# V-Sekai/godot-whisper

Measured on AMD Instinct MI355X. Metric: realtime-factor (audio-sec/wall-sec), base.en 30 s chunk, PCM->tokens, higher is better.
Workload: dtype f16; 1 GPU; base.en, single 30 s chunk per step per GPU (1x MI355X), greedy decode, host params (max_tokens=16, single_segment, token_timestamps), whisper_full with host PCM (H2D inside the timed region); weights=synthetic seed 1234 (f16 ggml, base.en shape)

## Files before the change

godot-whisper_amd/csrc/device.cpp:

```cpp

#include "wmi.h"
#include <atomic>
#include <thread>
#include <map>
#include <mutex>
#include "kernels.h"

#include <algorithm>
#include <cmath>
#include <cstdlib>
#include <cstring>

namespace wmi {

namespace {

template <typename T> bool dalloc(T *& p, size_t n_elems) {
    p = nullptr;
    return HIP_OK(hipMalloc((void **) &p, std::max<size_t>(n_elems, 1) * sizeof(T)));
}
template <typename T> void dfree(T *& p) { if (p) (void) hipFree(p); p = nullptr; }

}

static bool make_own_queue_stream(int device, hipStream_t * out) {
    uint32_t mask[16]; for (uint32_t & m : mask) m = 0xFFFFFFFFu;
    hipDeviceProp_t prop{};
    const int ncu = hipGetDeviceProperties(&prop, device) == hipSuccess ? prop.multiProcessorCount : 256;
    const uint32_t words = (uint32_t) std::min(16, (ncu + 31) / 32);
    if (hipExtStreamCreateWithCUMask(out, words, mask) == hipSuccess) return true;
    (void) hipGetLastError();
    return false;
}

static std::mutex g_oq_mu;
static std::map<int, std::vector<hipStream_t>> g_oq_pool;
static std::map<int, int> g_oq_made;
hipStream_t own_queue_stream_get(int device) {
    static const int cap = getenv("WMI_OWN_QUEUE_CAP") ? std::max(0, atoi(getenv("WMI_OWN_QUEUE_CAP"))) : 16;
    {
        std::lock_guard<std::mutex> lk(g_oq_mu);
        auto & v = g_oq_pool[device];
        if (!v.empty()) { hipStream_t s = v.back(); v.pop_back(); return s; }
        if (g_oq_made[device] >= cap) return nullptr;
        g_oq_made[device] += 1;
    }
    hipStream_t s = nullptr;
    if (make_own_queue_stream(device, &s)) return s;
    std::lock_guard<std::mutex> lk(g_oq_mu);
    g_oq_made[device] -= 1;
    return nullptr;
}
void own_queue_stream_put(int device, hipStream_t s) {
    if (!s) return;
    (void) hipStreamSynchronize(s);
    std::lock_guard<std::mutex> lk(g_oq_mu);
    g_oq_pool[device].push_back(s);
}

static thread_local StateInstall * t_state_install = nullptr;
State * StateSlot::get() const {
    for (const StateInstall * p = t_state_install; p; p = p->prev) if (p->slot == this) return p->st;
    return own;
}
StateInstall::StateInstall(const StateSlot & sl, State * s) : slot(&sl), st(s), prev(t_state_install) { t_state_install = this; }
StateInstall::~StateInstall() { t_state_install = prev; }
StateInstall * state_installs_top() { return t_state_install; }
void state_installs_set(StateInstall * top) { t_state_install = top; }

static bool init_state_into(whisper_context & ctx, State * st, bool replica_state, hipStream_t adopt);
bool init_state(whisper_context & ctx, bool replica_state, hipStream_t adopt) {
    State * st = new State();
    ctx.state = st;
    return init_state_into(ctx, st, replica_state, adopt);
}
static bool init_state_into(whisper_context & ctx, State * st, bool replica_state, hipStream_t adopt) {
    const HParams & hp = ctx.model.hp;
    st->device = ctx.device;
    DeviceState & d = st->dev;
    if (!HIP_OK(hipSetDevice(ctx.device))) return false;
    static const bool pooled = getenv("WMI_POOLED_MAIN_STREAM") != nullptr;
    if (adopt) { d.stream = adopt; d.stream_own_queue = true; }
    else if (!pooled && (d.stream = own_queue_stream_get(ctx.device))) d.stream_own_queue = true;
    else HIP_TRY(hipStreamCreateWithFlags(&d.stream, hipStreamNonBlocking));
    if (!replica_state) {
        static const int spares = getenv("WMI_SPARE_QUEUES") ? atoi(getenv("WMI_SPARE_QUEUES"))
                                : getenv("WMI_BATCH_REPLICAS") ? std::max(0, std::min(15, atoi(getenv("WMI_BATCH_REPLICAS")))) : 3;
        for (int i = 0; i < spares; ++i) { hipStream_t sp = own_queue_stream_get(ctx.device); if (sp) ctx.spare_streams.push_back(sp); }
    }

    const size_t S = hp.n_audio_state, T = hp.n_audio_ctx, Lt = hp.n_text_layer, H = hp.n_audio_head;
    const size_t n_self = 3 * (size_t) hp.n_text_ctx;
    st->kv_self.size = (uint32_t) n_self; st->kv_self.cells.assign(n_self, KVCell());
    bool ok = true;
    ok = ok && dalloc(st->kv_self.k, Lt * n_self * S) && dalloc(st->kv_self.v, Lt * n_self * S);
    ok = ok && dalloc(d.kvc_k, Lt * T * S) && dalloc(d.kvc_v, Lt * T * S);
    d.Tpad = (int) ((T + 63) / 64 * 64);
    const size_t mel_rows = 2 * T + 8;
    ok = ok && dalloc(d.mel_t, mel_rows * hp.n_mels + 1024) && dalloc(d.conv1, (2 * T + 4) * S)
            && dalloc(d.x, T * S) && dalloc(d.embd_conv, T * S) && dalloc(d.xn, T * S)
            && dalloc(d.q, T * S) && dalloc(d.k, T * S) && dalloc(d.vt, S * d.Tpad) && dalloc(d.att, T * S)
            && dalloc(d.h, T * 4 * S) && dalloc(d.rowmax, H * T) && dalloc(d.enc_out, T * S) && dalloc(d.enc_out_h, T * S)
            && dalloc(d.mel_max, 4);
    const size_t n = hp.n_text_ctx;
    if (ctx.model.quantised) {
        const size_t rows = std::max<size_t>(T, n);
        d.aq_rows = (int) rows;
        ok = ok && dalloc(d.aq, rows * 4 * S) && dalloc(d.ads, 2 * rows * (4 * S / 32)) && dalloc(d.att32, T * S) && dalloc(d.datt32, n * S);
        d.wq16_elems = 8 * S * S;
        ok = ok && dalloc(d.aq16, rows * 4 * S) && dalloc(d.wq16, d.wq16_elems);
    }
    d.logits_rows_cap = 8;
    ok = ok && dalloc(d.d_tokens, 3 * n + n * n_self);
    if (ok) { d.d_pos = d.d_tokens + n; d.d_rows = d.d_pos + n; d.d_mask = (float *) (d.d_rows + n); }
    ok = ok
            && dalloc(d.dx, n * S) && dalloc(d.dxn, n * S) && dalloc(d.dq, n * S) && dalloc(d.datt, n * S)
            && dalloc(d.dh, n * 4 * S) && dalloc(d.logits, (size_t) d.logits_rows_cap * hp.n_vocab)
            && dalloc(d.xattn, k::attn_cross_scratch_floats((int) n, (int) H, (int) T));
    d.pinned_bytes = std::max<size_t>((size_t) d.logits_rows_cap * hp.n_vocab * 4, n * n_self * 4 + 3 * n * 4 + 4096);
    ok = ok && HIP_OK(hipHostMalloc(&d.pinned, d.pinned_bytes, hipHostMallocDefault));
    {
        unsigned char * hand = nullptr;
        ok = ok && dalloc(hand, (size_t) 32 * S + 64 + 40960);
        if (ok) { d.mlp_hand = hand; d.mlp_arrive = (unsigned long long *) (hand + (size_t) 16 * S); k::fill_zero(hand, (size_t) 32 * S + 64 + 40960, d.stream); }
    }
    if (!ok) { WMI_ERR("%s: device allocation failed\n", __func__); return false; }
    k::fill_zero(d.vt, S * d.Tpad * sizeof(__half), d.stream);
    k::fill_zero(d.conv1, (2 * T + 4) * S * sizeof(__half), d.stream);
    k::fill_zero(d.mel_t, (mel_rows * hp.n_mels + 1024) * sizeof(__half), d.stream);
    k::fill_zero(st->kv_self.k, Lt * n_self * S * sizeof(__half), d.stream);
    k::fill_zero(st->kv_self.v, Lt * n_self * S * sizeof(__half), d.stream);
    k::fill_zero(d.kvc_k, Lt * T * S * sizeof(__half), d.stream);
    k::fill_zero(d.kvc_v, Lt * T * S * sizeof(__half), d.stream);
    HIP_TRY(hipStreamSynchronize(d.stream));

    st->batch.token.resize(n); st->batch.pos.resize(n); st->batch.seq_id.resize(n); st->batch.logits.resize(n);
    st->logits.reserve((size_t) hp.n_vocab * 8);
    for (auto & dec : st->decoders) dec.rng = std::mt19937(0);
    WMI_INFO("%s: kv self size = %.2f MB, kv cross size = %.2f MB\n", __func__,
             2.0 * Lt * n_self * S * 2 / 1e6, 2.0 * Lt * T * S * 2 / 1e6);
    return true;
}

State * create_state(whisper_context & ctx) {
    State * st = new State();
    if (init_state_into(ctx, st, true, nullptr)) return st;
    destroy_state(st);
    return nullptr;
}

void free_state(whisper_context & ctx) {
    destroy_state(ctx.state);
    ctx.state = nullptr;
}

void destroy_state(State * st) {
    if (!st) return;
    (void) hipSetDevice(st->device);
    DeviceState & d = st->dev;
    if (d.stream) (void) hipStreamSynchronize(d.stream);
    dfree(st->kv_self.k); dfree(st->kv_self.v); dfree(d.kvc_k); dfree(d.kvc_v);
    if (d.copy_stream) { (void) hipStreamSynchronize(d.copy_stream); (void) hipStreamDestroy(d.copy_stream); }
    if (d.energy_ev) (void) hipEventDestroy(d.energy_ev);
    for (hipEvent_t & e : d.ph_ev) { if (e) (void) hipEventDestroy(e); e = nullptr; }
    if (d.mel_ev) { (void) hipEventDestroy(d.mel_ev); d.mel_ev = nullptr; }
    dfree(d.energy); if (d.energy_host) (void) hipHostFree(d.energy_host);
    if (d.ts_host) (void) hipHostFree(d.ts_host);
    dfree(d.pcm); dfree(d.mel); dfree(d.mel_max); dfree(d.mel_t); dfree(d.conv1); dfree(d.x); dfree(d.embd_conv);
    dfree(d.xn); dfree(d.q); dfree(d.k); dfree(d.vt); dfree(d.att); dfree(d.h); dfree(d.rowmax); dfree(d.enc_out);
    dfree(d.enc_out_h); dfree(d.d_tokens); d.d_pos = nullptr; d.d_mask = nullptr; d.d_rows = nullptr; dfree(d.dx); dfree(d.dxn);
    dfree(d.dq); dfree(d.datt); dfree(d.dh); dfree(d.logits); dfree(d.xattn); dfree(d.ban_dev);
    if (d.mlp_hand) { (void) hipFree(d.mlp_hand); d.mlp_hand = nullptr; d.mlp_arrive = nullptr; }
    dfree(d.aq); dfree(d.ads); dfree(d.aq16); dfree(d.wq16); dfree(d.att32); dfree(d.datt32);
    for (auto & sg : d.step_graphs) { if (sg.exec) (void) hipGraphExecDestroy(sg.exec); if (sg.graph) (void) hipGraphDestroy(sg.graph); sg = DeviceState::StepGraph{}; }
    if (d.step_dev) (void) hipFree(d.step_dev);
    if (d.sample_dev) (void) hipFree(d.sample_dev);
    if (d.filter_scratch) (void) hipFree(d.filter_scratch);
    if (d.draw_scratch) (void) hipFree(d.draw_scratch);
    if (d.draw_host) (void) hipHostFree(d.draw_host);
    if (d.step_host) (void) hipHostFree(d.step_host);
    if (d.sample_host) (void) hipHostFree(d.sample_host);
    if (d.pinned) (void) hipHostFree(d.pinned);
    if (d.stream && d.stream_own_queue) own_queue_stream_put(st->device, d.stream);
    else if (d.stream) (void) hipStreamDestroy(d.stream);
    delete st;
}

static bool ensure_mel_capacity(DeviceState & d, size_t n_pad, size_t n_mel_elems) {
    if (n_pad > d.pcm_cap) { dfree(d.pcm); if (!dalloc(d.pcm, n_pad + 1024)) return false; d.pcm_cap = n_pad + 1024; }
    if (n_mel_elems > d.mel_cap) { dfree(d.mel); if (!dalloc(d.mel, n_mel_elems)) return false; d.mel_cap = n_mel_elems; }
    return true;
}

static bool phase_events(DeviceState & d) {
    for (hipEvent_t & e : d.ph_ev) if (!e && !HIP_OK(hipEventCreate(&e))) return false;
    return true;
}
int64_t phase_settle(State & st, bool wait) {
    DeviceState & d = st.dev;
    if (!d.ph_mel && !d.ph_enc) return 0;
    if (wait) (void) hipStreamSynchronize(d.stream);
    float ms = 0.0f; double gpu_us = 0.0;
    if (d.ph_mel) { if (hipEventSynchronize(d.ph_ev[1]) == hipSuccess && hipEventElapsedTime(&ms, d.ph_ev[0], d.ph_ev[1]) == hipSuccess) { st.t_mel_us += (int64_t) (ms * 1e3); gpu_us += ms * 1e3; } d.ph_mel = false; }
    if (d.ph_enc) { if (hipEventSynchronize(d.ph_ev[3]) == hipSuccess && hipEventElapsedTime(&ms, d.ph_ev[2], d.ph_ev[3]) == hipSuccess) { st.t_encode_us += (int64_t) (ms * 1e3); gpu_us += ms * 1e3; } d.ph_enc = false; }
    return d.ph_host0 + (int64_t) gpu_us;
}

bool pcm_to_mel(whisper_context & ctx, const float * samples, int n_samples, bool samples_on_device, bool sync, bool defer) {
    if (!compute_ready(ctx, __func__)) return false;
    State & st = *ctx.state; DeviceState & d = st.dev;
    const int64_t t0 = time_us();
    const int n_mel = ctx.model.n_filt_mel;
    hipStream_t ms = d.mel_stream ? d.mel_stream : d.stream;
    const int64_t n_pad = (int64_t) n_samples + 480000 + 400;
    const int n_len = (int) ((n_pad - 400) / 160);
    const int n_len_org = 1 + (n_samples + 200 - 400) / 160;
    const int n_valid = n_samples + 200;
    const int n_fft_frames = std::min(n_valid / 160 + 1, n_len);
    if (!ensure_mel_capacity(d, (size_t) n_pad + (size_t) n_samples, (size_t) n_mel * n_len)) return false;
    defer = defer && ms == d.stream && phase_events(d);
    if (defer) { (void) phase_settle(st, true); HIP_TRY(hipEventRecord(d.ph_ev[0], ms)); }
    const float * src = samples;
    if (!samples_on_device) {
        float * stage = d.pcm + n_pad;
        HIP_TRY(hipMemcpyAsync(stage, samples, (size_t) n_samples * 4, hipMemcpyHostToDevice, ms));
        src = stage;
    }
    d.last_pcm = src; d.last_pcm_n = n_samples;
    k::mel_pad(src, n_samples, d.pcm, (int) n_pad, ms, (int *) d.mel_max);
    k::mel_frames(d.pcm, n_valid, n_fft_frames, n_len, n_mel, ctx.w.mel_filters, ctx.w.mel_ranges, ctx.w.mel_taps, d.mel, (int *) d.mel_max, ms);
    k::mel_normalize(d.mel, n_mel * n_len, (const int *) d.mel_max, ms);
    st.mel.n_len = n_len; st.mel.n_len_org = n_len_org; st.mel.n_mel = n_mel;
    if (defer) { HIP_TRY(hipEventRecord(d.ph_ev[1], ms)); d.ph_mel = true; d.ph_host0 = t0; return true; }
    if (sync) HIP_TRY(hipStreamSynchronize(ms));
    st.t_mel_us += time_us() - t0;
    return true;
}

static bool ensure_copy_stream(DeviceState & d) {
    if (d.copy_stream) return true;
    int prio_lo = 0, prio_hi = 0;
    (void) hipDeviceGetStreamPriorityRange(&prio_lo, &prio_hi);
    if (!HIP_OK(hipStreamCreateWithPriority(&d.copy_stream, hipStreamNonBlocking, prio_lo))) HIP_TRY(hipStreamCreateWithFlags(&d.copy_stream, hipStreamNonBlocking));
    HIP_TRY(hipEventCreateWithFlags(&d.energy_ev, hipEventDisableTiming));
    return true;
}
static hipStream_t envelope_stream(const DeviceState & d) { return d.energy_wait_stream ? d.energy_wait_stream : d.copy_stream; }

bool pcm_to_mel_batch(whisper_context & ctx, const std::vector<State *> & states, const float * const * pcm, const int * n_samples,
                      bool samples_on_device, bool envelopes) {
    if (!compute_ready(ctx, __func__)) return false;
    DeviceState & pd = ctx.state->dev;
    hipStream_t s = pd.stream;
    const int n_mel = ctx.model.n_filt_mel;
    const int64_t t0 = time_us();
    k::MelBatch mb{}; int nb = 0; std::vector<State *> in;
    if (envelopes && !ensure_copy_stream(pd)) return false;
    for (size_t r = 0; r < states.size(); ++r) {
        const int n = n_samples[r];
        if (n <= 0) continue;
        if (nb >= 16) return false;
        State & st = *states[r]; DeviceState & d = st.dev;
        const int64_t n_pad = (int64_t) n + 480000 + 400;
        const int n_len = (int) ((n_pad - 400) / 160);
        if (!ensure_mel_capacity(d, (size_t) n_pad + (size_t) n, (size_t) n_mel * n_len)) return false;
        const float * src = pcm[r];
        if (!samples_on_device) {
            float * stage = d.pcm + n_pad;
            HIP_TRY(hipMemcpyAsync(stage, pcm[r], (size_t) n * 4, hipMemcpyHostToDevice, s));
            src = stage;
        }
        d.last_pcm = src; d.last_pcm_n = n;
        st.mel.n_len = n_len; st.mel.n_len_org = 1 + (n + 200 - 400) / 160; st.mel.n_mel = n_mel;
        mb.pcm[nb] = src; mb.pad[nb] = d.pcm; mb.mel[nb] = d.mel; mb.gmax[nb] = (int *) d.mel_max; mb.n[nb] = n;
        if (envelopes) {
            if (d.energy_pending && envelope_stream(d)) { HIP_TRY(hipStreamSynchronize(envelope_stream(d))); d.energy_pending = false; }
            const size_t nblk = (size_t) n / 256 + 2;
            if ((size_t) n > d.energy_cap) {
                st.energy = nullptr; st.energy_n = 0; st.energy_bmin = st.energy_bmax = nullptr;
                if (d.energy_host) (void) hipHostFree(d.energy_host);
                d.energy_host = nullptr; d.energy_cap = 0;
                if (!HIP_OK(hipHostMalloc((void **) &d.energy_host, ((size_t) n + 2 * ((size_t) n / 256 + 2)) * 4, hipHostMallocDefault))) return false;
                d.energy_cap = (size_t) n;
            }
            const size_t need = d.energy_cap + 2 * nblk;
            if (d.energy_dev_cap < need) { dfree(d.energy); d.energy_dev_cap = 0; if (!dalloc(d.energy, need)) return false; d.energy_dev_cap = need; }
            mb.energy[nb] = d.energy; mb.bmin[nb] = d.energy + d.energy_cap; mb.bmax[nb] = d.energy + d.energy_cap + nblk;
        }
        in.push_back(&st); ++nb;
    }
    if (nb == 0) return true;
    if (envelopes) {
        if (!pd.mel_ev) HIP_TRY(hipEventCreateWithFlags(&pd.mel_ev, hipEventDisableTiming));
        HIP_TRY(hipEventRecord(pd.energy_ev, s));
        HIP_TRY(hipStreamWaitEvent(pd.copy_stream, pd.energy_ev, 0));
        k::signal_energy_batch(mb, nb, 32, pd.copy_stream);
        HIP_TRY(hipEventRecord(pd.mel_ev, pd.copy_stream));
        for (State * st : in) {
            DeviceState & d = st->dev;
            d.energy_device_only = true; d.energy_pending = true; d.energy_wait_stream = pd.copy_stream;
        }
    }
    k::mel_batch(mb, nb, n_mel, ctx.w.mel_filters, ctx.w.mel_ranges, ctx.w.mel_taps, s);
    if (envelopes) HIP_TRY(hipStreamWaitEvent(s, pd.mel_ev, 0));
    ctx.state->t_mel_us += time_us() - t0;
    return hipGetLastError() == hipSuccess;
}

bool signal_energy_device(whisper_context & ctx, int hw, bool sync, int via_dma) {
    State & st = *ctx.state; DeviceState & d = st.dev;
    const int n = d.last_pcm_n;
    if (!d.last_pcm || n <= 0) return false;
    if (!ensure_copy_stream(d)) return false;
    if (d.energy_pending) { HIP_TRY(hipStreamSynchronize(envelope_stream(d))); d.energy_pending = false; }
    d.energy_wait_stream = nullptr;
    d.energy_device_only = false;
    if ((size_t) n > d.energy_cap) {
        st.energy = nullptr; st.energy_n = 0; st.energy_bmin = st.energy_bmax = nullptr;
        if (d.energy_host) (void) hipHostFree(d.energy_host);
        d.energy_host = nullptr; d.energy_cap = 0;
        if (!HIP_OK(hipHostMalloc((void **) &d.energy_host, ((size_t) n + 2 * ((size_t) n / 256 + 2)) * 4, hipHostMallocDefault))) return false;
        d.energy_cap = (size_t) n;
    }
    HIP_TRY(hipEventRecord(d.energy_ev, d.mel_stream ? d.mel_stream : d.stream));
    HIP_TRY(hipStreamWaitEvent(d.copy_stream, d.energy_ev, 0));
    {
        const size_t nb = (size_t) n / 256 + 2;
        const size_t need = d.energy_cap + 2 * nb;
        if (via_dma && d.energy_dev_cap < need) { dfree(d.energy); d.energy_dev_cap = 0; if (dalloc(d.energy, need)) d.energy_dev_cap = need; else via_dma = 0; }
        if (via_dma == 3) {
            k::signal_energy(d.last_pcm, n, hw, d.energy, d.energy + d.energy_cap, d.energy + d.energy_cap + nb, d.copy_stream);
            d.energy_device_only = true;
        } else
        k::signal_energy(d.last_pcm, n, hw, d.energy_host, d.energy_host + d.energy_cap, d.energy_host + d.energy_cap + nb, d.copy_stream);
    }
    d.energy_pending = true;
    return sync ? signal_energy_wait(st) : true;
}

bool ts_refine_device(State & st, const k::TsTok * in, int n, k::TsOut * out) {
    DeviceState & d = st.dev;
    constexpr int CAP = 448;
    if (n <= 0) return true;
    hipStream_t es = envelope_stream(d);
    if (n > CAP || !d.energy || !es) return false;
    if (!d.ts_host && !HIP_OK(hipHostMalloc(&d.ts_host, CAP * (sizeof(k::TsTok) + sizeof(k::TsOut)), hipHostMallocDefault))) return false;
    k::TsTok * hin = (k::TsTok *) d.ts_host; k::TsOut * hout = (k::TsOut *) (hin + CAP);
    memcpy(hin, in, (size_t) n * sizeof(k::TsTok));
    const size_t nb = (size_t) d.last_pcm_n / 256 + 2;
    k::ts_refine(d.energy, d.energy + d.energy_cap, d.energy + d.energy_cap + nb, d.last_pcm_n, hin, hout, n, es);
    HIP_TRY(hipStreamSynchronize(es));
    memcpy(out, hout, (size_t) n * sizeof(k::TsOut));
    return true;
}

bool signal_energy_wait(State & st) {
    DeviceState & d = st.dev;
    if (!d.energy_pending) return true;
    if (d.energy_device_only) {
        HIP_TRY(hipStreamSynchronize(envelope_stream(d)));
        st.energy = nullptr; st.energy_bmin = st.energy_bmax = nullptr; st.energy_n = d.last_pcm_n; st.energy_on_device = true;
        d.energy_pending = false;
        return true;
    }
    st.energy_on_device = false;
    HIP_TRY(hipStreamSynchronize(d.copy_stream));
    st.energy = d.energy_host; st.energy_n = d.last_pcm_n;
    st.energy_bmin = d.energy_host + d.energy_cap; st.energy_bmax = st.energy_bmin + ((size_t) d.last_pcm_n / 256 + 2);
    d.energy_pending = false;
    return true;
}

bool set_mel(whisper_context & ctx, const float * data, int n_len, int n_mel) {
    if (!compute_ready(ctx, __func__)) return false;
    State & st = *ctx.state; DeviceState & d = st.dev;
    if (!ensure_mel_capacity(d, 0, (size_t) n_len * n_mel)) return false;
    HIP_TRY(hipMemcpyAsync(d.mel, data, (size_t) n_len * n_mel * 4, hipMemcpyHostToDevice, d.stream));
    HIP_TRY(hipStreamSynchronize(d.stream));
    st.mel.n_len = n_len; st.mel.n_len_org = n_len; st.mel.n_mel = n_mel;
    return true;
}

bool encode(whisper_context & ctx, int mel_offset, bool defer) {
    if (!compute_ready(ctx, __func__)) return false;
    State & st = *ctx.state; DeviceState & d = st.dev; const Weights & w = ctx.w; const HParams & hp = ctx.model.hp;
    const int64_t t0 = time_us();
    d.chain_valid = false;
    defer = defer && !ctx.model.quantised && phase_events(d);
    if (defer) {
        if (d.ph_enc) (void) phase_settle(st, true);
        HIP_TRY(hipEventRecord(d.ph_ev[2], d.stream));
        if (!d.ph_mel) d.ph_host0 = t0;
    }
    const int T = st.exp_n_audio_ctx > 0 ? st.exp_n_audio_ctx : hp.n_audio_ctx;
    const int S = hp.n_audio_state, H = hp.n_audio_head, La = hp.n_audio_layer, Lt = hp.n_text_layer, nm = hp.n_mels;
    hipStream_t s = d.stream;
    if (st.mel.n_mel != nm || d.mel == nullptr) { WMI_ERR("%s: no mel spectrogram (n_mel %d, expected %d)\n", __func__, st.mel.n_mel, nm); return false; }

    const int rows_mel = 2 * T + 6;
    k::mel_slice(d.mel, st.mel.n_len, nm, mel_offset, 2 * T, d.mel_t, nm, rows_mel, s);
    {
        k::GemmArgs a{};
        a.A = d.mel_t; a.lda = nm; a.W = w.conv1_w; a.ldw = w.conv1_k; a.M = 2 * T; a.N = S; a.K = w.conv1_k;
        a.bias = w.conv1_b; a.C = d.conv1 + S; a.ldc = S;
        k::gemm(k::EPI_F16_BIAS_GELU, a, s);
    }
    if (d.conv1_max_T > T) k::fill_zero(d.conv1 + (size_t) (2 * T + 1) * S, (size_t) S * sizeof(__half), s);
    d.conv1_max_T = std::max(d.conv1_max_T, T);
    {
        k::GemmArgs a{};
        a.A = d.conv1; a.lda = 2 * S; a.W = w.conv2_w; a.ldw = w.conv2_k; a.M = T; a.N = S; a.K = w.conv2_k;
        a.bias = w.conv2_b; a.C = d.x; a.ldc = S; a.resid = w.e_pe; a.ldr = S; a.aux = d.embd_conv; a.ldaux = S;
        k::gemm(k::EPI_CONV2, a, s);
    }
    const float kq_scale = 1.0f / sqrtf((float) S / H);
    if (ctx.model.quantised) { if (!encode_layers_q(ctx, T)) return false; }
    else {
    for (int il = 0; il < La; ++il) {
        const EncLayerW & l = w.enc[il];
        k::layernorm(d.x, T, S, l.ln1_g, l.ln1_b, hp.eps, d.xn, nullptr, s);
        {
            k::GemmArgs a{};
            a.A = d.xn; a.lda = S; a.W = l.w_qkv; a.ldw = S; a.M = T; a.N = 3 * S; a.K = S; a.bias = l.b_qkv;
            a.C = d.q; a.ldc = S; a.aux = d.k; a.ldaux = S; a.aux2 = d.vt; a.ldaux2 = d.Tpad; a.S = S;
            k::gemm(k::EPI_QKV_ENC, a, s);
        }
        k::attn_encoder(d.q, d.k, d.vt, T, d.Tpad, S, H, kq_scale, d.att, s);
        {
            k::GemmArgs a{};
            a.A = d.att; a.lda = S; a.W = l.w_o; a.ldw = S; a.M = T; a.N = S; a.K = S; a.bias = l.b_o;
            a.C = d.x; a.ldc = S; a.resid = d.x; a.ldr = S;
            k::gemm(k::EPI_F32_BIAS_RESID, a, s);
        }
        k::layernorm(d.x, T, S, l.ln2_g, l.ln2_b, hp.eps, d.xn, nullptr, s);
        {
            k::GemmArgs a{};
            a.A = d.xn; a.lda = S; a.W = l.w_fc1; a.ldw = S; a.M = T; a.N = 4 * S; a.K = S; a.bias = l.b_fc1;
            a.C = d.h; a.ldc = 4 * S;
            k::gemm(k::EPI_F16_BIAS_GELU, a, s);
        }
        {
            k::GemmArgs a{};
            a.A = d.h; a.lda = 4 * S; a.W = l.w_fc2; a.ldw = 4 * S; a.M = T; a.N = S; a.K = 4 * S; a.bias = l.b_fc2;
            a.C = d.x; a.ldc = S; a.resid = d.x; a.ldr = S;
            k::gemm(k::EPI_F32_BIAS_RESID, a, s);
        }
    }
    k::layernorm(d.x, T, S, w.e_ln_g, w.e_ln_b, hp.eps, d.enc_out_h, d.enc_out, s);
    {
        k::GemmArgs a{};
        a.A = d.enc_out_h; a.lda = S; a.W = w.w_ckv; a.ldw = S; a.M = T; a.N = Lt * 2 * S; a.K = S; a.bias = w.b_ckv;
        a.C = d.kvc_k; a.ldc = S; a.aux = d.kvc_v; a.ldaux = S; a.S = S; a.layer_stride = (int64_t) T * S;
        a.scale = powf((float) S / H, -0.25f);
        k::gemm(k::EPI_CROSS_KV, a, s);
    }
    }
    st.enc_n_ctx = T;
    st.n_encode++;
    if (defer) {
        HIP_TRY(hipEventRecord(d.ph_ev[3], s)); d.ph_enc = true;
        return HIP_OK(hipGetLastError());
    }
    HIP_TRY(hipStreamSynchronize(s));
    if (!HIP_OK(hipGetLastError())) return false;
    {
        int64_t dt = time_us() - t0;
        const int64_t done = phase_settle(st, false);
        if (done > t0) dt = std::max<int64_t>(0, dt - (done - t0));
        st.t_encode_us += dt;
    }
    return true;
}

bool decode(whisper_context & ctx, const Batch & batch) {
    if (!compute_ready(ctx, __func__)) return false;
    State & st = *ctx.state; DeviceState & d = st.dev; const Weights & w = ctx.w; const HParams & hp = ctx.model.hp;
    const int64_t t0 = time_us();
    d.chain_valid = false;
    KVCache & kv = st.kv_self;
    const int n = batch.n_tokens;
    if (n <= 0) return false;
    if (n > hp.n_text_ctx) { WMI_ERR("%s: %d tokens in one batch, the model's text context is %d\n", __func__, n, hp.n_text_ctx); return false; }
    if (!kv_find_slot(kv, batch)) return false;
    kv.n = (uint32_t) kv_cell_max(kv);
    const int n_kv = (int) kv.n, kv_head = (int) kv.head, n_ctx = (int) kv.size;
    const int S = hp.n_text_state, H = hp.n_text_head, Lt = hp.n_text_layer, NV = hp.n_vocab;
    const int Tc = st.enc_n_ctx > 0 ? st.enc_n_ctx : (st.exp_n_audio_ctx > 0 ? st.exp_n_audio_ctx : hp.n_audio_ctx);
    hipStream_t s = d.stream;

    int32_t * p_tok = (int32_t *) d.pinned, * p_pos = p_tok + n, * p_rows = p_pos + n;
    float * p_mask = (float *) (p_rows + n);
    std::vector<int> rows;
    for (int i = 0; i < n; ++i) { p_tok[i] = batch.token[i]; p_pos[i] = batch.pos[i]; if (batch.logits[i]) rows.push_back(i); }
    for (size_t i = 0; i < rows.size(); ++i) p_rows[i] = rows[i];
    for (int j = 0; j < n; ++j) {
        const int32_t pos = batch.pos[j], seq = batch.seq_id[j];
        for (int i = 0; i < n_kv; ++i)
            p_mask[(size_t) j * n_kv + i] = (!kv.cells[i].has(seq) || kv.cells[i].pos > pos) ? -INFINITY : 0.0f;
    }
    d.d_pos = d.d_tokens + n; d.d_rows = d.d_pos + n; d.d_mask = (float *) (d.d_rows + n);
    HIP_TRY(hipMemcpyAsync(d.d_tokens, p_tok, ((size_t) 3 * n + (size_t) n * n_kv) * 4, hipMemcpyHostToDevice, s));

    if (ctx.model.quantised) {
        if (!decode_layers_q(ctx, n, n_kv, kv_head, Tc, rows)) return false;
        HIP_TRY(hipStreamSynchronize(s));
        if (!HIP_OK(hipGetLastError())) return false;
        int64_t dtq = time_us() - t0;
        { const int64_t done = phase_settle(st, false); if (done > t0) dtq = std::max<int64_t>(0, dtq - (done - t0)); }
        if (n == 1)      { st.t_decode_us += dtq; st.n_decode++; }
        else if (n < 16) { st.t_batchd_us += dtq; st.n_batchd += n; }
        else             { st.t_prompt_us += dtq; st.n_prompt += n; }
        return true;
    }
    k::dec_embed(d.d_tokens, d.d_pos, n, S, w.d_te, w.d_pe, d.dx, s);
    const float kq_scale = powf((float) S / H, -0.25f);

    auto proj = [&](int epi, const float * ln_g, const float * ln_b, const __half * a16, int K, int N, const __half * W,
                    const float * bias, void * C, int ldc, const float * resid, void * aux, int ldaux, void * aux2,
                    int ldaux2, float scale) {
        if (n <= 8) {
            k::GemvArgs g{};
            g.x32 = d.dx; g.ln_g = ln_g; g.ln_b = ln_b; g.eps = hp.eps; g.a16 = a16; g.n = n; g.K = K; g.N = N; g.W = W;
            g.bias = bias; g.epi = epi; g.C = C; g.ldc = ldc; g.resid = resid; g.ldr = S; g.aux = aux; g.ldaux = ldaux;
            g.aux2 = aux2; g.ldaux2 = ldaux2; g.scale = scale; g.S = S; g.rows = nullptr;
            k::gemv(g, s);
        } else {
            const __half * A = a16;
            if (ln_g) { k::layernorm(d.dx, n, S, ln_g, ln_b, hp.eps, d.dxn, nullptr, s); A = d.dxn; }
            k::GemmArgs a{};
            a.A = A; a.lda = K; a.W = W; a.ldw = K; a.M = n; a.N = N; a.K = K; a.bias = bias; a.C = C; a.ldc = ldc;
            a.resid = resid; a.ldr = S; a.aux = aux; a.ldaux = ldaux; a.aux2 = aux2; a.ldaux2 = ldaux2; a.scale = scale; a.S = S;
            k::gemm(epi, a, s);
        }
    };

    for (int il = 0; il < Lt; ++il) {
        const DecLayerW & l = w.dec[il];
        __half * ck = kv.k + ((size_t) il * n_ctx) * S, * cv = kv.v + ((size_t) il * n_ctx) * S;
        proj(k::EPI_QKV_DEC, l.ln1_g, l.ln1_b, nullptr, S, 3 * S, l.w_qkv, l.b_qkv, d.dq, S, nullptr,
             ck + (size_t) kv_head * S, S, cv + (size_t) kv_head * S, S, kq_scale);
        k::attn_decoder(d.dq, n, S, H, ck, cv, n_kv, d.d_mask, n_kv, d.datt, s);
        proj(k::EPI_F32_BIAS_RESID, nullptr, nullptr, d.datt, S, S, l.w_o, l.b_o, d.dx, S, d.dx, nullptr, 0, nullptr, 0, 0.f);
        proj(k::EPI_Q_SCALED, l.ln2_g, l.ln2_b, nullptr, S, S, l.w_cq, l.b_cq, d.dq, S, nullptr, nullptr, 0, nullptr, 0, kq_scale);
        k::attn_cross_split(d.dq, n, S, H, d.kvc_k + (size_t) il * Tc * S, d.kvc_v + (size_t) il * Tc * S, Tc, d.xattn, d.datt, s);
        proj(k::EPI_F32_BIAS_RESID, nullptr, nullptr, d.datt, S, S, l.w_co, l.b_co, d.dx, S, d.dx, nullptr, 0, nullptr, 0, 0.f);
        proj(k::EPI_F16_BIAS_GELU, l.ln3_g, l.ln3_b, nullptr, S, 4 * S, l.w_fc1, l.b_fc1, d.dh, 4 * S, nullptr, nullptr, 0, nullptr, 0, 0.f);
        proj(k::EPI_F32_BIAS_RESID, nullptr, nullptr, d.dh, 4 * S, S, l.w_fc2, l.b_fc2, d.dx, S, d.dx, nullptr, 0, nullptr, 0, 0.f);
    }

    st.logits.resize((size_t) n * NV);
    for (size_t r0 = 0; r0 < rows.size(); r0 += 8) {
        const int nr = (int) std::min<size_t>(8, rows.size() - r0);
        k::GemvArgs g{};
        g.x32 = d.dx; g.ln_g = w.d_ln_g; g.ln_b = w.d_ln_b; g.eps = hp.eps; g.n = nr; g.K = S; g.N = NV; g.W = w.d_te;
        g.epi = k::EPI_LOGITS; g.C = d.logits; g.ldc = NV; g.rows = d.d_rows + r0;
        k::gemv(g, s);
        if (d.keep_logits_on_device && rows.size() <= 8) continue;
        HIP_TRY(hipMemcpyAsync(d.pinned, d.logits, (size_t) nr * NV * 4, hipMemcpyDeviceToHost, s));
        HIP_TRY(hipStreamSynchronize(s));
        for (int r = 0; r < nr; ++r)
            memcpy(st.logits.data() + (size_t) rows[r0 + r] * NV, (const float *) d.pinned + (size_t) r * NV, (size_t) NV * 4);
    }
    HIP_TRY(hipStreamSynchronize(s));
    if (!HIP_OK(hipGetLastError())) return false;

    int64_t dt = time_us() - t0;
    { const int64_t done = phase_settle(st, false); if (done > t0) dt = std::max<int64_t>(0, dt - (done - t0)); }
    if (n == 1)      { st.t_decode_us += dt; st.n_decode++; }
    else if (n < 16) { st.t_batchd_us += dt; st.n_batchd += n; }
    else             { st.t_prompt_us += dt; st.n_prompt += n; }
    return true;
}

}

namespace wmi {

bool upload_static_ban(whisper_context & ctx, const whisper_full_params & params) {
    State & st = *ctx.state; DeviceState & d = st.dev; const Vocab & v = ctx.model.vocab;
    const uint64_t sig = (params.suppress_non_speech_tokens ? 1u : 0u) | (params.no_timestamps ? 2u : 0u) | (params.tdrz_enable ? 4u : 0u) | 8u;
    if (d.ban_dev && d.ban_sig == sig) return true;
    const int n = v.n_vocab;
    std::vector<uint8_t> ban(n, 0);
    auto B = [&](int id) { if (id >= 0 && id < n) ban[id] = 1; };
    B(v.not_); B(v.sot); B(v.nosp); if (!params.tdrz_enable) B(v.solm);
    B(v.translate); B(v.transcribe); B(v.prev);
    for (int i = 0; i < lang_count(); ++i) B(v.sot + 1 + i);
    if (params.no_timestamps) for (int i = v.beg; i < n; ++i) ban[i] = 1;
    if (params.suppress_non_speech_tokens) {
        Decoder tmp; tmp.i_batch = 0;
        std::vector<float> saved; saved.swap(st.logits);
        st.logits.assign(n, 0.0f);
        for (int i = v.beg; i < n; ++i) st.logits[i] = -1e30f;
        whisper_full_params p2 = params; p2.suppress_blank = false; p2.max_initial_ts = 0.0f; p2.logits_filter_callback = nullptr;
        tmp.sequence.tokens.push_back(whisper_token_data{0, 0, 0.f, 0.f, 0.f, 0.f, -1, -1, 0.f});
        process_logits(ctx, tmp, p2, 0.0f);
        for (int i = 0; i < v.beg; ++i) if (tmp.logits[i] == -INFINITY) ban[i] = 1;
        st.logits.swap(saved);
    }
    if (!d.ban_dev && !dalloc(d.ban_dev, (size_t) n)) return false;
    HIP_TRY(hipMemcpyAsync(d.ban_dev, ban.data(), (size_t) n, hipMemcpyHostToDevice, d.stream));
// ... 442 lines not shown
```

godot-whisper_amd/csrc/gemm_epi.h:

```cpp
#pragma once
#include "kernels.h"
#include "wave_ops.h"

namespace wmi { namespace k { namespace gemm_detail {

typedef _Float16 half8 __attribute__((ext_vector_type(8)));
typedef _Float16 half4 __attribute__((ext_vector_type(4)));
typedef float    floatx4 __attribute__((ext_vector_type(4)));


__device__ __forceinline__ float round_f16(float x) { return __half2float(f2h(x)); }

__device__ __forceinline__ float gelu16(float x) {
    const float xh = round_f16(x);
    const float g  = 0.5f * xh * (1.0f + tanhf(0.79788456080286535587989211986876f * xh * (1.0f + 0.044715f * xh * xh)));
    return round_f16(g);
}

__device__ __forceinline__ float gelu16_fast(float x) {
    const float xh = round_f16(x);
    const float u  = 0.79788456080286535587989211986876f * xh * (1.0f + 0.044715f * xh * xh);
    const float t  = 1.0f - 2.0f * __builtin_amdgcn_rcpf(__expf(2.0f * u) + 1.0f);
    return round_f16(0.5f * xh * (1.0f + t));
}

typedef float    float2v __attribute__((ext_vector_type(2)));
typedef _Float16 half2v  __attribute__((ext_vector_type(2)));
__device__ __forceinline__ half2v gelu16_pair(float2v x) {
    const half2v xh = __builtin_convertvector(x, half2v);
    const float2v xf = {(float) xh[0], (float) xh[1]};
    constexpr float C0 = -2.0f * 0.79788456080286535587989211986876f * 1.44269504088896340736f;
    constexpr float C1 = C0 * 0.044715f;
    const float2v c0 = {C0, C0}, c1 = {C1, C1}, one = {1.0f, 1.0f};
    const float2v w = __builtin_elementwise_fma(xf * xf, c1, c0) * xf;
    const float2v e = {__builtin_amdgcn_exp2f(w[0]), __builtin_amdgcn_exp2f(w[1])};
    const float2v d = one + e;
    const float2v r = {__builtin_amdgcn_rcpf(d[0]), __builtin_amdgcn_rcpf(d[1])};
    const float2v g = xf * r;
    return __builtin_convertvector(g, half2v);
}

struct Conv2Row { int out, pe; bool valid; };
__device__ __forceinline__ Conv2Row conv2_row(const GemmArgs & a, int m) {
    if (a.rows_per_chunk <= 0) return Conv2Row{m, m, true};
    const int P = a.rows_per_chunk, c = m / P, t = m - c * P;
    return Conv2Row{c * (P - 4) + t, t < P - 4 ? t : 0, t < P - 4};
}

template <int FM, int FN, bool GUARD>
__device__ __forceinline__ void epilogue_vt_wide(const GemmArgs & a, floatx4 (&acc)[FM][FN], const int mb, const int nb, const int lane);
__device__ __forceinline__ bool vt_wide_ok(const GemmArgs & a);
template <int EPI, int FM, int FN, bool GUARD>
__device__ __forceinline__ void epilogue_rows(const GemmArgs & a, floatx4 (&acc)[FM][FN], const int mb, const int nb, const int lane) {
    if constexpr (EPI == EPI_QKV_ENC) {
        if (__builtin_amdgcn_readfirstlane(nb) >= 2 * a.S && vt_wide_ok(a)) { epilogue_vt_wide<FM, FN, GUARD>(a, acc, mb, nb, lane); return; }
    }
    const int frow = lane & 15, fq = lane >> 4;
    float biasv[FN];
#pragma unroll
    for (int j = 0; j < FN; ++j) {
        const int n = nb + j * 16 + frow;
        biasv[j] = (a.bias && (!GUARD || n < a.N)) ? a.bias[n] : 0.0f;
    }
#pragma unroll
    for (int j = 0; j < FN; ++j) {
        const int n = nb + j * 16 + frow;
        if (GUARD && n >= a.N) continue;
        const float bias = biasv[j];
        float rpre[FM][4];
        if constexpr (EPI == EPI_F32_BIAS_RESID || EPI == EPI_CONV2) {
#pragma unroll
            for (int i = 0; i < FM; ++i)
#pragma unroll
                for (int r = 0; r < 4; ++r) {
                    const int m = mb + i * 16 + fq * 4 + r;
                    const int mc = (GUARD && m >= a.M) ? a.M - 1 : m;
                    rpre[i][r] = a.resid[(size_t) (EPI == EPI_CONV2 ? conv2_row(a, mc).pe : mc) * a.ldr + n];
                }
        }
#pragma unroll
        for (int i = 0; i < FM; ++i) {
            const int mrow = mb + i * 16 + fq * 4;
            if constexpr (EPI == EPI_QKV_ENC) {
                const int seg = n / a.S, c = n - seg * a.S;
                if (seg == 2) {
                    const int rpc = a.rows_per_chunk > 0 ? a.rows_per_chunk : a.M;
                    const int cb = mrow / rpc, t0 = mrow - cb * rpc;
                    __half * vt = (__half *) a.aux2 + (size_t) cb * a.chunk_stride_aux2 + (size_t) c * a.ldaux2;
                    if ((!GUARD || mrow + 3 < a.M) && t0 + 3 < rpc && ((t0 & 3) == 0)) {
                        half4 v;
#pragma unroll
                        for (int r = 0; r < 4; ++r) v[r] = (_Float16) pin_f32(acc[i][j][r] + bias);
                        *(half4 *) (vt + vt_pos(t0)) = v;
                    } else {
                        for (int r = 0; r < 4; ++r) {
                            const int m = mrow + r;
                            if (m >= a.M) continue;
                            const int cb2 = m / rpc, t = m - cb2 * rpc;
                            ((__half *) a.aux2)[(size_t) cb2 * a.chunk_stride_aux2 + (size_t) c * a.ldaux2 + vt_pos(t)] = f2h(acc[i][j][r] + bias);
                        }
                    }
                    continue;
                }
#pragma unroll
                for (int r = 0; r < 4; ++r) {
                    const int m = mrow + r;
                    if (GUARD && m >= a.M) continue;
                    const float v = acc[i][j][r] + bias;
                    if (seg == 0) ((__half *) a.C)[(size_t) m * a.ldc + c] = f2h(v);
                    else          ((__half *) a.aux)[(size_t) m * a.ldaux + c] = f2h(v);
                }
                continue;
            }
#pragma unroll
            for (int r = 0; r < 4; ++r) {
                const int m = mrow + r;
                if (GUARD && m >= a.M) continue;
                const float v = acc[i][j][r];
                if constexpr (EPI == EPI_F16_BIAS) {
                    ((__half *) a.C)[(size_t) m * a.ldc + n] = f2h(v + bias);
                } else if constexpr (EPI == EPI_F16_BIAS_GELU) {
                    ((__half *) a.C)[(size_t) m * a.ldc + n] = f2h(gelu16_fast(v + bias));
                } else if constexpr (EPI == EPI_F32_BIAS_RESID) {
                    ((float *) a.C)[(size_t) m * a.ldc + n] = (v + bias) + rpre[i][r];
                } else if constexpr (EPI == EPI_CONV2) {
                    const float g = gelu16_fast(v + bias);
                    const Conv2Row cr = conv2_row(a, m);
                    if (cr.valid) {
                        if (a.aux) ((float *) a.aux)[(size_t) cr.out * a.ldaux + n] = g;
                        ((float *) a.C)[(size_t) cr.out * a.ldc + n] = rpre[i][r] + g;
                    }
                } else if constexpr (EPI == EPI_QKV_DEC) {
                    const int seg = __builtin_amdgcn_readfirstlane((nb + j * 16) / a.S);
                    const int c = n - seg * a.S;
                    __half * dst; float val;
                    if (seg == 0)      { dst = (__half *) a.C    + (size_t) m * a.ldc;    val = (v + bias) * a.scale; }
                    else if (seg == 1) { dst = (__half *) a.aux  + (size_t) m * a.ldaux;  val = v * a.scale; }
                    else               { dst = (__half *) a.aux2 + (size_t) m * a.ldaux2; val = v + bias; }
                    dst[c] = f2h(val);
                } else if constexpr (EPI == EPI_CROSS_KV) {
                    const int il = n / (2 * a.S), c = n - il * 2 * a.S;
                    if (c < a.S) ((__half *) a.C)[il * a.layer_stride + (size_t) m * a.ldc + c] = f2h(v * a.scale);
                    else         ((__half *) a.aux)[il * a.layer_stride + (size_t) m * a.ldaux + (c - a.S)] = f2h(v + bias);
                } else if constexpr (EPI == EPI_Q_SCALED) {
                    ((__half *) a.C)[(size_t) m * a.ldc + n] = f2h((v + bias) * a.scale);
                }
            }
        }
    }
}

template <int EPI, int FM, int FN, bool GUARD>
__device__ __forceinline__ void epilogue_cols(const GemmArgs & a, floatx4 (&acc)[FM][FN], const int mb, const int nb, const int n0, const int lane) {
    const int frow = lane & 15, fq = lane >> 4;
#pragma unroll
    for (int j = 0; j < FN; ++j) {
        const int n = nb + j * 16 + fq * 4;
        if (GUARD && n >= a.N) continue;
        float4 b4 = make_float4(0.f, 0.f, 0.f, 0.f);
        if (a.bias) b4 = *(const float4 *) (a.bias + n);
        const float bias[4] = {b4.x, b4.y, b4.z, b4.w};
        float4 rpre[FM];
        if constexpr (EPI == EPI_F32_BIAS_RESID || EPI == EPI_CONV2) {
#pragma unroll
            for (int i = 0; i < FM; ++i) {
                const int m = mb + i * 16 + frow;
                const int mc = (GUARD && m >= a.M) ? a.M - 1 : m;
                rpre[i] = *(const float4 *) (a.resid + (size_t) (EPI == EPI_CONV2 ? conv2_row(a, mc).pe : mc) * a.ldr + n);
            }
        }
#pragma unroll
        for (int i = 0; i < FM; ++i) {
            const int m = mb + i * 16 + frow;
            if (GUARD && m >= a.M) continue;
            float v[4];
#pragma unroll
            for (int r = 0; r < 4; ++r) v[r] = acc[i][j][r];
            auto put16 = [&](__half * dst, const float (&x)[4]) {
                half4 h;
#pragma unroll
                for (int r = 0; r < 4; ++r) h[r] = (_Float16) pin_f32(x[r]);
                *(half4 *) dst = h;
            };
            if constexpr (EPI == EPI_F16_BIAS) {
                const float x[4] = {v[0] + bias[0], v[1] + bias[1], v[2] + bias[2], v[3] + bias[3]};
                put16((__half *) a.C + (size_t) m * a.ldc + n, x);
            } else if constexpr (EPI == EPI_F16_BIAS_GELU) {
                const float2v x0 = {v[0] + bias[0], v[1] + bias[1]}, x1 = {v[2] + bias[2], v[3] + bias[3]};
                const half2v g0 = gelu16_pair(x0), g1 = gelu16_pair(x1);
                half4 h; h[0] = g0[0]; h[1] = g0[1]; h[2] = g1[0]; h[3] = g1[1];
                *(half4 *) ((__half *) a.C + (size_t) m * a.ldc + n) = h;
            } else if constexpr (EPI == EPI_Q_SCALED) {
                const float x[4] = {(v[0] + bias[0]) * a.scale, (v[1] + bias[1]) * a.scale, (v[2] + bias[2]) * a.scale, (v[3] + bias[3]) * a.scale};
                put16((__half *) a.C + (size_t) m * a.ldc + n, x);
            } else if constexpr (EPI == EPI_F32_BIAS_RESID) {
                float4 o;
                o.x = (v[0] + bias[0]) + rpre[i].x; o.y = (v[1] + bias[1]) + rpre[i].y; o.z = (v[2] + bias[2]) + rpre[i].z; o.w = (v[3] + bias[3]) + rpre[i].w;
                *(float4 *) ((float *) a.C + (size_t) m * a.ldc + n) = o;
            } else if constexpr (EPI == EPI_CONV2) {
                float4 g, o;
                const float2v x0 = {v[0] + bias[0], v[1] + bias[1]}, x1 = {v[2] + bias[2], v[3] + bias[3]};
                const half2v g0 = gelu16_pair(x0), g1 = gelu16_pair(x1);
                g.x = (float) g0[0]; g.y = (float) g0[1]; g.z = (float) g1[0]; g.w = (float) g1[1];
                const Conv2Row cr = conv2_row(a, m);
                if (cr.valid) {
                    if (a.aux) *(float4 *) ((float *) a.aux + (size_t) cr.out * a.ldaux + n) = g;
                    o.x = rpre[i].x + g.x; o.y = rpre[i].y + g.y; o.z = rpre[i].z + g.z; o.w = rpre[i].w + g.w;
                    *(float4 *) ((float *) a.C + (size_t) cr.out * a.ldc + n) = o;
                }
            } else if constexpr (EPI == EPI_QKV_ENC) {
                const int seg = __builtin_amdgcn_readfirstlane(n0 / a.S);
                const int c = n - seg * a.S;
                const float x[4] = {v[0] + bias[0], v[1] + bias[1], v[2] + bias[2], v[3] + bias[3]};
                if (seg == 0) put16((__half *) a.C + (size_t) m * a.ldc + c, x);
                else          put16((__half *) a.aux + (size_t) m * a.ldaux + c, x);
            } else if constexpr (EPI == EPI_CROSS_KV) {
                const int il = n / (2 * a.S), c = n - il * 2 * a.S;
                if (c < a.S) {
                    const float x[4] = {v[0] * a.scale, v[1] * a.scale, v[2] * a.scale, v[3] * a.scale};
                    put16((__half *) a.C + il * a.layer_stride + (size_t) m * a.ldc + c, x);
                } else {
                    const float x[4] = {v[0] + bias[0], v[1] + bias[1], v[2] + bias[2], v[3] + bias[3]};
                    put16((__half *) a.aux + il * a.layer_stride + (size_t) m * a.ldaux + (c - a.S), x);
                }
            }
        }
    }
}

__device__ __forceinline__ uint4 ror8_u4(uint4 t) {
    t.x = (uint32_t) xor_lane<8>((int) t.x); t.y = (uint32_t) xor_lane<8>((int) t.y);
    t.z = (uint32_t) xor_lane<8>((int) t.z); t.w = (uint32_t) xor_lane<8>((int) t.w);
    return t;
}
__device__ __forceinline__ void trade_rows8(uint4 & P, uint4 & Q, const bool lo) {
    uint4 t = lo ? Q : P;
    t = ror8_u4(t);
    if (lo) Q = t; else P = t;
}

struct VtDest { __half * p; bool ok; };
template <bool GUARD>
__device__ __forceinline__ VtDest vt_block_dest(const GemmArgs & a, const int m_blk, const int c, const int pos8) {
    const int rpc = a.rows_per_chunk > 0 ? a.rows_per_chunk : a.M;
    const int cb = m_blk / rpc, tb = m_blk - cb * rpc;
    VtDest d;
    d.ok = (!GUARD || m_blk < a.M) && tb + 16 <= a.ldaux2;
    d.p = (__half *) a.aux2 + (size_t) cb * a.chunk_stride_aux2 + (size_t) c * a.ldaux2 + tb + pos8;
    return d;
}
template <int FM, int FN, bool GUARD>
__device__ __forceinline__ void epilogue_vt_wide(const GemmArgs & a, floatx4 (&acc)[FM][FN], const int mb, const int nb, const int lane) {
    const int frow = lane & 15, fq = lane >> 4;
    const bool lo = frow < 8;
    const int pos8 = (fq & 1) << 3, up = fq >> 1;
    auto pack = [&](const floatx4 & v, const float bias, uint32_t (&w)[2]) {
        half4 h;
#pragma unroll
        for (int r = 0; r < 4; ++r) h[r] = (_Float16) pin_f32(v[r] + bias);
        const uint2 u = *(const uint2 *) &h;
        w[0] = u.x; w[1] = u.y;
    };
    auto pair16 = [&](const floatx4 & v0, const floatx4 & v1, const float bias) -> uint4 {
        uint32_t w0[2], w1[2];
        pack(v0, bias, w0); pack(v1, bias, w1);
        const auto s0 = __builtin_amdgcn_permlane32_swap(w0[0], w1[0], false, false);
        const auto s1 = __builtin_amdgcn_permlane32_swap(w0[1], w1[1], false, false);
        return make_uint4(s0[0], s1[0], s0[1], s1[1]);
    };
#pragma unroll
    for (int j = 0; j < FN; ++j) {
        const int n = nb + j * 16 + frow;
        const int c = n - 2 * a.S;
        const float bias = a.bias ? a.bias[n] : 0.0f;
        int i = 0;
#pragma unroll
        for (; i + 3 < FM; i += 4) {
            uint4 P = pair16(acc[i][j], acc[i + 1][j], bias), Q = pair16(acc[i + 2][j], acc[i + 3][j], bias);
            trade_rows8(P, Q, lo);
            const int blk = mb + (i + (lo ? 0 : 2) + up) * 16, cc = c - frow + (frow & 7);
            const VtDest d0 = vt_block_dest<GUARD>(a, blk, cc, pos8), d1 = vt_block_dest<GUARD>(a, blk, cc + 8, pos8);
            if (d0.ok) *(uint4 *) d0.p = P;
            if (d1.ok) *(uint4 *) d1.p = Q;
        }
#pragma unroll
        for (; i + 1 < FM; i += 2) {
            const uint4 P = pair16(acc[i][j], acc[i + 1][j], bias);
            const VtDest d = vt_block_dest<GUARD>(a, mb + (i + up) * 16, c, pos8);
            if (d.ok) *(uint4 *) d.p = P;
        }
#pragma unroll
        for (; i < FM; ++i) {
            uint32_t w[2];
            pack(acc[i][j], bias, w);
            const VtDest d = vt_block_dest<GUARD>(a, mb + i * 16, c, 0);
            if (d.ok) *(uint2 *) (d.p + ((fq & 1) << 3) + ((fq >> 1) << 2)) = make_uint2(w[0], w[1]);
        }
    }
}
__device__ __forceinline__ bool vt_wide_ok(const GemmArgs & a) {
    const int rpc = a.rows_per_chunk > 0 ? a.rows_per_chunk : a.M;
    return !(a.no_glds & 16) && (rpc >= a.M || (rpc & 15) == 0) && (a.ldaux2 & 7) == 0 && (a.chunk_stride_aux2 & 7) == 0;
}

template <int EPI, int FM, int FN, bool GUARD>
__device__ __forceinline__ void epilogue_cols_wide(const GemmArgs & a, floatx4 (&acc)[FM][FN], const int mb, const int nb, const int n0, const int lane) {
    static_assert(FN % 2 == 0, "wide stores pair fragment columns");
    static_assert(EPI == EPI_F16_BIAS || EPI == EPI_F16_BIAS_GELU || EPI == EPI_Q_SCALED || EPI == EPI_F32_BIAS_RESID || EPI == EPI_CROSS_KV || EPI == EPI_QKV_ENC, "epilogue");
    if constexpr (GUARD) {
        if (nb + 16 * FN > a.N) { epilogue_cols<EPI, FM, FN, true>(a, acc, mb, nb, n0, lane); return; }
    }
    const int frow = lane & 15, fq = lane >> 4;
    const bool lo = frow < 8;
    const int r8 = frow & 7, hb = frow >> 3;
    float bias[FN][4];
#pragma unroll
    for (int j = 0; j < FN; ++j) {
        float4 b4 = make_float4(0.f, 0.f, 0.f, 0.f);
        if (a.bias) b4 = *(const float4 *) (a.bias + nb + j * 16 + fq * 4);
        bias[j][0] = b4.x; bias[j][1] = b4.y; bias[j][2] = b4.z; bias[j][3] = b4.w;
    }
    if constexpr (EPI == EPI_F32_BIAS_RESID) {
#pragma unroll
        for (int i = 0; i < FM; ++i) {
            const int m = mb + i * 16 + frow;
            float4 rp[FN];
#pragma unroll
            for (int j = 0; j < FN; ++j) rp[j] = *(const float4 *) (a.resid + (size_t) ((GUARD && m >= a.M) ? a.M - 1 : m) * a.ldr + nb + j * 16 + fq * 4);
#pragma unroll
            for (int j = 0; j < FN; j += 2) {
                uint4 P, Q;
                {
                    float4 o;
                    o.x = (acc[i][j][0] + bias[j][0]) + rp[j].x; o.y = (acc[i][j][1] + bias[j][1]) + rp[j].y;
                    o.z = (acc[i][j][2] + bias[j][2]) + rp[j].z; o.w = (acc[i][j][3] + bias[j][3]) + rp[j].w;
                    P = make_uint4(__float_as_uint(o.x), __float_as_uint(o.y), __float_as_uint(o.z), __float_as_uint(o.w));
                    o.x = (acc[i][j + 1][0] + bias[j + 1][0]) + rp[j + 1].x; o.y = (acc[i][j + 1][1] + bias[j + 1][1]) + rp[j + 1].y;
                    o.z = (acc[i][j + 1][2] + bias[j + 1][2]) + rp[j + 1].z; o.w = (acc[i][j + 1][3] + bias[j + 1][3]) + rp[j + 1].w;
                    Q = make_uint4(__float_as_uint(o.x), __float_as_uint(o.y), __float_as_uint(o.z), __float_as_uint(o.w));
                }
                trade_rows8(P, Q, lo);
                const int mr = mb + i * 16 + r8, n = nb + (j + hb) * 16 + fq * 4;
                if (!GUARD || mr < a.M)     *(uint4 *) ((float *) a.C + (size_t) mr * a.ldc + n) = P;
                if (!GUARD || mr + 8 < a.M) *(uint4 *) ((float *) a.C + (size_t) (mr + 8) * a.ldc + n) = Q;
            }
        }
        return;
    } else {
    __half * dst; int ldd; int c0; float scale = 1.0f; bool use_bias = true;
    if constexpr (EPI == EPI_QKV_ENC) {
        const int seg = __builtin_amdgcn_readfirstlane(nb / a.S);
        c0 = nb - seg * a.S;
        dst = seg == 0 ? (__half *) a.C : (__half *) a.aux; ldd = seg == 0 ? a.ldc : a.ldaux;
    } else if constexpr (EPI == EPI_CROSS_KV) {
        const int il = __builtin_amdgcn_readfirstlane(nb / (2 * a.S)), c = nb - il * 2 * a.S;
        const bool isk = c < a.S;
        dst = (isk ? (__half *) a.C : (__half *) a.aux) + il * a.layer_stride; ldd = isk ? a.ldc : a.ldaux; c0 = isk ? c : c - a.S;
        scale = isk ? a.scale : 1.0f; use_bias = !isk;
    } else {
        dst = (__half *) a.C; ldd = a.ldc; c0 = nb;
        if constexpr (EPI == EPI_Q_SCALED) scale = a.scale;
    }
    const int cb = ((fq & 1) << 4) | ((fq >> 1) << 3);
#pragma unroll
    for (int i = 0; i < FM; ++i) {
        uint4 blk[FN / 2];
#pragma unroll
        for (int j = 0; j < FN; j += 2) {
            uint32_t w[2][2];
#pragma unroll
            for (int jj = 0; jj < 2; ++jj) {
                const floatx4 v = acc[i][j + jj];
                half4 h;
                if constexpr (EPI == EPI_F16_BIAS_GELU) {
                    const float2v x0 = {v[0] + bias[j + jj][0], v[1] + bias[j + jj][1]}, x1 = {v[2] + bias[j + jj][2], v[3] + bias[j + jj][3]};
                    const half2v g0 = gelu16_pair(x0), g1 = gelu16_pair(x1);
                    h[0] = g0[0]; h[1] = g0[1]; h[2] = g1[0]; h[3] = g1[1];
                } else if constexpr (EPI == EPI_CROSS_KV) {
#pragma unroll
                    for (int r = 0; r < 4; ++r) h[r] = (_Float16) pin_f32(use_bias ? v[r] + bias[j + jj][r] : v[r] * scale);
                } else if constexpr (EPI == EPI_Q_SCALED) {
#pragma unroll
                    for (int r = 0; r < 4; ++r) h[r] = (_Float16) pin_f32((v[r] + bias[j + jj][r]) * scale);
                } else {
#pragma unroll
                    for (int r = 0; r < 4; ++r) h[r] = (_Float16) pin_f32(v[r] + bias[j + jj][r]);
                }
                const uint2 u = *(const uint2 *) &h;
                w[jj][0] = u.x; w[jj][1] = u.y;
            }
            const auto s0 = __builtin_amdgcn_permlane16_swap(w[0][0], w[1][0], false, false);
            const auto s1 = __builtin_amdgcn_permlane16_swap(w[0][1], w[1][1], false, false);
            blk[j / 2] = make_uint4(s0[0], s1[0], s0[1], s1[1]);
        }
#pragma unroll
        for (int b = 0; b < FN / 2; b += 2) {
            if constexpr (FN / 2 >= 2) {
                uint4 P = blk[b], Q = blk[b + 1];
                trade_rows8(P, Q, lo);
                const int mr = mb + i * 16 + r8, c = c0 + (b + hb) * 32 + cb;
                if (!GUARD || mr < a.M)     *(uint4 *) (dst + (size_t) mr * ldd + c) = P;
                if (!GUARD || mr + 8 < a.M) *(uint4 *) (dst + (size_t) (mr + 8) * ldd + c) = Q;
            } else {
                const int m = mb + i * 16 + frow, c = c0 + b * 32 + cb;
                if (!GUARD || m < a.M) *(uint4 *) (dst + (size_t) m * ldd + c) = blk[b];
            }
        }
    }
    }
}

template <int EPI, int FM, int FN>
__device__ __forceinline__ void pack_cols_wide(const GemmArgs & a, floatx4 (&acc)[FM][FN], const int mb, const int nb, const int n0, const int lane,
                                               uint4 (&out)[FM][2], __half * & ptr, int & ldd_out) {
    static_assert(FN == 4, "pack_cols_wide: wave tiles of four fragment columns");
    static_assert(EPI == EPI_F16_BIAS || EPI == EPI_F16_BIAS_GELU || EPI == EPI_Q_SCALED || EPI == EPI_CROSS_KV || EPI == EPI_QKV_ENC, "epilogue");
    const int frow = lane & 15, fq = lane >> 4;
    const bool lo = frow < 8;
    const int r8 = frow & 7, hb = frow >> 3;
    float bias[FN][4];
#pragma unroll
    for (int j = 0; j < FN; ++j) {
        float4 b4 = make_float4(0.f, 0.f, 0.f, 0.f);
        if (a.bias) b4 = *(const float4 *) (a.bias + nb + j * 16 + fq * 4);
        bias[j][0] = b4.x; bias[j][1] = b4.y; bias[j][2] = b4.z; bias[j][3] = b4.w;
    }
    __half * dst; int ldd; int c0; float scale = 1.0f; bool use_bias = true;
    if constexpr (EPI == EPI_QKV_ENC) {
        const int seg = __builtin_amdgcn_readfirstlane(nb / a.S);
        c0 = nb - seg * a.S;
        dst = seg == 0 ? (__half *) a.C : (__half *) a.aux; ldd = seg == 0 ? a.ldc : a.ldaux;
    } else if constexpr (EPI == EPI_CROSS_KV) {
        const int il = __builtin_amdgcn_readfirstlane(nb / (2 * a.S)), c = nb - il * 2 * a.S;
        const bool isk = c < a.S;
        dst = (isk ? (__half *) a.C : (__half *) a.aux) + il * a.layer_stride; ldd = isk ? a.ldc : a.ldaux; c0 = isk ? c : c - a.S;
        scale = isk ? a.scale : 1.0f; use_bias = !isk;
    } else {
        dst = (__half *) a.C; ldd = a.ldc; c0 = nb;
        if constexpr (EPI == EPI_Q_SCALED) scale = a.scale;
    }
    const int cb = ((fq & 1) << 4) | ((fq >> 1) << 3);
#pragma unroll
    for (int i = 0; i < FM; ++i) {
        uint4 blk[2];
#pragma unroll
        for (int j = 0; j < FN; j += 2) {
            uint32_t w[2][2];
#pragma unroll
            for (int jj = 0; jj < 2; ++jj) {
                const floatx4 v = acc[i][j + jj];
                half4 h;
                if constexpr (EPI == EPI_F16_BIAS_GELU) {
                    const float2v x0 = {v[0] + bias[j + jj][0], v[1] + bias[j + jj][1]}, x1 = {v[2] + bias[j + jj][2], v[3] + bias[j + jj][3]};
                    const half2v g0 = gelu16_pair(x0), g1 = gelu16_pair(x1);
                    h[0] = g0[0]; h[1] = g0[1]; h[2] = g1[0]; h[3] = g1[1];
                } else if constexpr (EPI == EPI_CROSS_KV) {
#pragma unroll
                    for (int r = 0; r < 4; ++r) h[r] = (_Float16) pin_f32(use_bias ? v[r] + bias[j + jj][r] : v[r] * scale);
                } else if constexpr (EPI == EPI_Q_SCALED) {
#pragma unroll
                    for (int r = 0; r < 4; ++r) h[r] = (_Float16) pin_f32((v[r] + bias[j + jj][r]) * scale);
                } else {
#pragma unroll
                    for (int r = 0; r < 4; ++r) h[r] = (_Float16) pin_f32(v[r] + bias[j + jj][r]);
                }
                const uint2 u = *(const uint2 *) &h;
                w[jj][0] = u.x; w[jj][1] = u.y;
            }
            const auto s0 = __builtin_amdgcn_permlane16_swap(w[0][0], w[1][0], false, false);
            const auto s1 = __builtin_amdgcn_permlane16_swap(w[0][1], w[1][1], false, false);
            blk[j / 2] = make_uint4(s0[0], s1[0], s0[1], s1[1]);
        }
        uint4 P = blk[0], Q = blk[1];
        trade_rows8(P, Q, lo);
        out[i][0] = P; out[i][1] = Q;
    }
    ptr = dst + (size_t) (mb + r8) * ldd + (c0 + hb * 32 + cb);
    ldd_out = ldd;
}

}}}
```

godot-whisper_amd/csrc/k_dec.hip:

```cpp

#include <atomic>
#include "kernels.h"
#include "wave_ops.h"
#include <type_traits>

#include <cstdlib>
#include <algorithm>

namespace wmi { namespace k {

namespace {

__device__ __forceinline__ float round_f16(float x) { return __half2float(f2h(x)); }
__host__ __device__ __forceinline__ size_t sa_score_floats(int K, int cap) { const size_t n = (size_t) (K / 64) * cap; return n < 1280 ? 1280 : n; }
__device__ __forceinline__ float gelu16(float x) {
    const float xh = round_f16(x);
    const float g  = 0.5f * xh * (1.0f + tanhf(0.79788456080286535587989211986876f * xh * (1.0f + 0.044715f * xh * xh)));
    return round_f16(g);
}

__global__ void k_dec_embed(const int32_t * __restrict__ tokens, const int32_t * __restrict__ pos, int S,
                            const __half * __restrict__ te, const float * __restrict__ pe, float * __restrict__ x) {
    const int i = blockIdx.x;
    const __half * t = te + (size_t) tokens[i] * S;
// ... 1837 lines not shown
        if (lane == 0) red[wave] = m;
        __syncthreads();
        m = fmaxf(fmaxf(red[0], red[1]), fmaxf(red[2], red[3]));
        __syncthreads();
        float l = 0.0f;
        for (int j = tid; j < n_kv; j += 256) { const float e = round_f16(expf(round_f16(row[j] - m))); row[j] = e; l += e; }
        _Pragma("unroll") for (int o = 32; o > 0; o >>= 1) l += WMI_SHX(l, o);
        if (lane == 0) red[wave] = l;
        __syncthreads();
        const float inv = (float) (1.0 / (double) ((red[0] + red[1]) + (red[2] + red[3])));
        for (int j = tid; j < n_kv; j += 256) row[j] = round_f16(row[j] * inv);
        __syncthreads();
        {
            const __half vnew = hq[128 + lane];
            float acc = 0.0f;
            for (int j = j0; j < j1; j += VB) {
                const bool more = j + VB < j1;
                __half vn[VB];
                if (more) {
#pragma unroll
                    for (int t = 0; t < VB; ++t) vn[t] = vp[(size_t) (j + VB + t < j1 ? j + VB + t : j1 - 1) * K];
                }
#pragma unroll
                for (int t = 0; t < VB; ++t) if (j + t < j1) acc = fmaf(row[j + t], __half2float(j + t == slot ? vnew : vh[t]), acc);
                if (more) {
#pragma unroll
                    for (int t = 0; t < VB; ++t) vh[t] = vn[t];
                }
            }
            part[wave * 64 + lane] = acc;
        }
        __syncthreads();
        if (wave == 0) {
            const float acc = (part[lane] + part[64 + lane]) + (part[128 + lane] + part[192 + lane]);
            const uint32_t mine = (uint32_t) __half_as_ushort(f2h(acc));
            const uint32_t other = (uint32_t) WMI_SHX((int) mine, 1);
            if (!(lane & 1)) {
                const unsigned long long gr = ((unsigned long long) tag << 32) | (unsigned long long) (mine | (other << 16));
                __hip_atomic_store(a.ga + (h * 32 + (lane >> 1)), gr, __ATOMIC_RELAXED, __HIP_MEMORY_SCOPE_AGENT);
            }
        }
        tm2 = stamp_t0(sp.base);
      }
    } else
    if (head_wave) {
        const int h = wg;
        const int part = lane >> 4;
        const unsigned long long * src = a.gq + (lane < 48 ? part * (S >> 1) + 32 * h + (lane & 15) * 2 : 32 * h);
        uint32_t spins = 0; bool landed = false; u32x4 q;
        for (; spins < spin_cap; ++spins) {
            asm volatile("global_load_dwordx4 %0, %1, off sc0 sc1\n\ts_waitcnt vmcnt(0)" : "=&v"(q) : "v"(src) : "memory");
            const bool ok = lane >= 48 || (q[1] == tag && q[3] == tag);
            if (__all(ok)) { landed = true; break; }
        }
        if (lane == 0 && (!landed || spins > PAIR_SLOW_POLLS))
            __hip_atomic_fetch_or(a.fault, landed ? PAIR_SLOW : PAIR_FAULT_TIMEOUT, __ATOMIC_RELAXED, __HIP_MEMORY_SCOPE_AGENT);
        if (lane < 48) *(uint2 *) (hq + part * 64 + (lane & 15) * 4) = make_uint2(q[0], q[2]);
        const int n_kv = __builtin_amdgcn_readfirstlane(nkv_pre), slot = __builtin_amdgcn_readfirstlane(ro_pre);
        uint4 qv[1];
        qv[0] = *(const uint4 *) (hq + o8 * 8);
        const uint4 knew = *(const uint4 *) (hq + 64 + o8 * 8), vnew = *(const uint4 *) (hq + 128 + o8 * 8);
        const int hs[1] = { h };
        if (n_kv > 32) {
#pragma unroll
            for (int t = 4; t < 8; ++t) {
                const int j = 8 * t + g, jc = j < n_kv ? j : 0;
                kv[0][t] = *(const uint4 *) (a.ck + (size_t) jc * K + h * 64 + o8 * 8);
                vv[0][t] = *(const uint4 *) (a.cv + (size_t) jc * K + h * 64 + o8 * 8);
            }
#pragma unroll
            for (int t = 0; t < 8; ++t) if (8 * t + g == slot) { kv[0][t] = knew; vv[0][t] = vnew; }
            self_attn_body<1, 8>(qv, kv, vv, n_kv, hs, H, lane, hatt - h * 64, nullptr, wscr);
        } else {
#pragma unroll
            for (int t = 0; t < 4; ++t) if (8 * t + g == slot) { kv[0][t] = knew; vv[0][t] = vnew; }
#pragma unroll
            for (int t = 4; t < 8; ++t) { kv[0][t] = make_uint4(0u, 0u, 0u, 0u); vv[0][t] = kv[0][t]; }
            self_attn_body<1, 4>(qv, kv, vv, n_kv, hs, H, lane, hatt - h * 64, nullptr, wscr);
        }
        if (lane < 32) {
            const uint32_t pr = *(const uint32_t *) (hatt + 2 * lane);
            const unsigned long long gr = ((unsigned long long) tag << 32) | (unsigned long long) pr;
            __hip_atomic_store(a.ga + (h * 32 + lane), gr, __ATOMIC_RELAXED, __HIP_MEMORY_SCOPE_AGENT);
        }
        tm2 = stamp_t0(sp.base);
    }
    if (p3) {
        const uint32_t slow_polls = LONG ? PAIR_SLOW_POLLS * (1u + (uint32_t) (__builtin_amdgcn_readfirstlane(nkv_pre) >> 6)) : PAIR_SLOW_POLLS;
        if (tid < (S >> 2)) {
            const unsigned long long * src = a.ga + tid * 2;
            uint32_t spins = 0; bool landed = false; u32x4 q;
            for (; spins < spin_cap; ++spins) {
                asm volatile("global_load_dwordx4 %0, %1, off sc0 sc1\n\ts_waitcnt vmcnt(0)" : "=&v"(q) : "v"(src) : "memory");
                const bool ok = q[1] == tag && q[3] == tag;
                if (__all(ok)) { landed = true; break; }
            }
            if (lane == 0 && (!landed || spins > slow_polls))
                __hip_atomic_fetch_or(a.fault, landed ? PAIR_SLOW : PAIR_FAULT_TIMEOUT, __ATOMIC_RELAXED, __HIP_MEMORY_SCOPE_AGENT);
            *(uint2 *) (act + tid * 4) = make_uint2(q[0], q[2]);
        }
        __syncthreads();
        float a3[NCH][8];
#pragma unroll
        for (int t = 0; t < NCH; ++t) {
            const int c = lane * 8 + 512 * t;
            uint4 u4 = *(const uint4 *) (act + (c < K ? c : 0));
            if (c >= K) u4 = make_uint4(0u, 0u, 0u, 0u);
            const __half2 * h = (const __half2 *) &u4;
#pragma unroll
            for (int e = 0; e < 4; ++e) { const float2 f = __half22float2(h[e]); a3[t][2 * e] = f.x; a3[t][2 * e + 1] = f.y; }
        }
        float acc[R3];
#pragma unroll
        for (int u = 0; u < R3; ++u) acc[u] = 0.0f;
#pragma unroll
        for (int t = 0; t < NCH; ++t)
#pragma unroll
            for (int u = 0; u < R3; ++u) {
                const __half2 * h = (const __half2 *) &w3[t][u];
#pragma unroll
                for (int e = 0; e < 4; ++e) {
                    const float2 f = __half22float2(h[e]);
                    acc[u] = fmaf(f.x, a3[t][2 * e], acc[u]);
                    acc[u] = fmaf(f.y, a3[t][2 * e + 1], acc[u]);
                }
            }
        float v;
        if constexpr (R3 == 2) {
            { const bool hi = lane & 32; const float keep = hi ? acc[1] : acc[0], send = hi ? acc[0] : acc[1]; v = keep + WMI_SHX(send, 32); }
            v += WMI_SHX(v, 16); v += WMI_SHX(v, 8); v += WMI_SHX(v, 4); v += WMI_SHX(v, 2); v += WMI_SHX(v, 1);
        } else {
#pragma unroll
            for (int u = 0; u < 2; ++u) { const bool hi = lane & 32; const float keep = hi ? acc[u + 2] : acc[u], send = hi ? acc[u] : acc[u + 2]; acc[u] = keep + WMI_SHX(send, 32); }
            { const bool hi = lane & 16; const float keep = hi ? acc[1] : acc[0], send = hi ? acc[0] : acc[1]; v = keep + WMI_SHX(send, 16); }
            v += WMI_SHX(v, 8); v += WMI_SHX(v, 4); v += WMI_SHX(v, 2); v += WMI_SHX(v, 1);
        }
        if ((lane % LPR3) == 0) {
            const float bias = a.bo ? bias3 : 0.0f;
            a.xout[orow + wrow3] = (v + bias) + resid3;
        }
    }
    stamp_end(sp.base, sp.slot, (int) blockIdx.y * (int) gridDim.x * WPB + gw, ts0, tm1, tm2);
}

static Knobs read_knobs() {
    Knobs kn{};
    kn.no_mlp_pair = getenv("WMI_NO_MLP_PAIR") != nullptr;
    kn.sa_wpb = getenv("WMI_SA_WPB") ? atoi(getenv("WMI_SA_WPB")) : 8;
    kn.gemv1_wide_generic = getenv("WMI_GEMV1_WIDE_GENERIC") != nullptr;
    kn.host_draws = getenv("WMI_HOST_DRAWS") != nullptr;
    kn.debug_sync = getenv("WMI_DEBUG_SYNC") != nullptr;
    kn.pair_withhold = getenv("WMI_PAIR_WITHHOLD") ? atoi(getenv("WMI_PAIR_WITHHOLD")) : 0;
    kn.pair_spin_cap = getenv("WMI_PAIR_SPIN_CAP") ? (uint32_t) strtoul(getenv("WMI_PAIR_SPIN_CAP"), nullptr, 0) : 0u;
    kn.no_front = getenv("WMI_NO_FRONT") != nullptr;
    kn.front_withhold = getenv("WMI_FRONT_WITHHOLD") ? atoi(getenv("WMI_FRONT_WITHHOLD")) : 0;
    kn.front_wpb = getenv("WMI_FRONT_WPB") ? atoi(getenv("WMI_FRONT_WPB")) : 4;
    kn.no_xback = getenv("WMI_NO_XBACK") != nullptr;
    kn.xback_withhold = getenv("WMI_XBACK_WITHHOLD") ? atoi(getenv("WMI_XBACK_WITHHOLD")) : 0;
    return kn;
}
static std::atomic<const Knobs *> g_knobs{nullptr};
const Knobs & knobs() {
    const Knobs * kn = g_knobs.load(std::memory_order_acquire);
    if (kn) return *kn;
    const Knobs * fresh = new Knobs(read_knobs());
    const Knobs * expect = nullptr;
    if (g_knobs.compare_exchange_strong(expect, fresh, std::memory_order_acq_rel)) return *fresh;
    delete fresh;
    return *expect;
}
void reload_knobs() { g_knobs.store(new Knobs(read_knobs()), std::memory_order_release); }

#define WMI_PAIR_TABLE(S, nch2, X) do { \
        if ((S) <= 512)      { if ((nch2) <= 3) X(1, 3, 4); else X(1, 4, 4); } \
        else if ((S) <= 768) X(2, 6, 4); \
        else                X(2, 8, 4); } while (0)

template <int N1, int N2, int W>
static int pair_fit() {
    static std::atomic<int> cache[64];
    int dev = 0;
    (void) hipGetDevice(&dev);
    std::atomic<int> & c = cache[dev & 63];
    int fit = c.load(std::memory_order_relaxed);
    if (fit > 0) return fit;
    int nb = 0, ncu = 0;
    if (hipOccupancyMaxActiveBlocksPerMultiprocessor(&nb, (const void *) k_mlp_pair<N1, N2, W>, 64 * W, 0) != hipSuccess) return 0;
    (void) hipDeviceGetAttribute(&ncu, hipDeviceAttributeMultiprocessorCount, dev);
    fit = nb > 1 ? (nb - 1) * ncu : nb * ncu;
    c.store(fit, std::memory_order_relaxed);
    return fit;
}

bool mlp_pair_usable(int S, bool with_mirror) {
    if (S > 1024 || (S % 64) != 0) return false;
    const int blocks = S / 4 + (with_mirror ? 1 : 0);
    const int nch2 = (4 * S + 511) / 512;
    int fit = 0;
#define WMI_PAIR_FIT(N1, N2, W) fit = pair_fit<N1, N2, W>()
    WMI_PAIR_TABLE(S, nch2, WMI_PAIR_FIT);
#undef WMI_PAIR_FIT
    return blocks <= fit;
}

void mlp_pair(const MlpPairArgs & a, float * x_inout, hipStream_t st) {
    const int S = a.S;
    const int G = S / 4;
    const int blocks = G + (a.step_copy_src ? 1 : 0);
    const int nch2 = (4 * S + 511) / 512;
    const Stamp sp = stamp_next();
#define WMI_PAIR_GO(N1, N2, W) hipLaunchKernelGGL((k_mlp_pair<N1, N2, W>), dim3(blocks), dim3(64 * W), 0, st, a, x_inout, G, sp)
    WMI_PAIR_TABLE(S, nch2, WMI_PAIR_GO);
#undef WMI_PAIR_GO
}
#undef WMI_PAIR_TABLE

static int front_wpb(int rows) { return rows > 1 ? 8 : (knobs().front_wpb == 8 ? 8 : 4); }
static size_t front_long_lds(int cap) { return sizeof(float) * (size_t) (((cap + 3) & ~3) + 256 + 4); }
bool front_usable(int S, int rows, int long_cap) {
    if (S > 1024 || (S % 64) != 0 || S < 128) return false;
    int dev = 0; (void) hipGetDevice(&dev);
    const int wide = S > 512 ? 1 : 0, wpb = front_wpb(rows), w8 = wpb == 8 ? 1 : 0;
    auto resident = [&](const void * fn, size_t lds) {
        int cus = 0, nb = 0;
        (void) hipDeviceGetAttribute(&cus, hipDeviceAttributeMultiprocessorCount, dev);
        if (hipOccupancyMaxActiveBlocksPerMultiprocessor(&nb, fn, 64 * wpb, lds) != hipSuccess) nb = 0;
        return 1 + std::max(0, (cus - 1) * std::min(nb, 2));
    };
    int v;
    if (long_cap > 0) {
        if (rows > 1 || wpb != 4 || front_long_lds(long_cap) > 48 * 1024) return false;
        static std::atomic<long long> lcache[64][2][4];
        v = 0;
        for (auto & e : lcache[dev & 63][wide]) {
            long long c = e.load(std::memory_order_acquire);
            if (c == 0) {
                const long long mine = ((long long) long_cap << 32) | resident(wide ? (const void *) k_front<2, 4, true> : (const void *) k_front<1, 4, true>, front_long_lds(long_cap));
                if (e.compare_exchange_strong(c, mine, std::memory_order_acq_rel)) c = mine;
            }
            if ((int) (c >> 32) == long_cap) { v = (int) (c & 0xffffffffll); break; }
        }
        if (v == 0) v = resident(wide ? (const void *) k_front<2, 4, true> : (const void *) k_front<1, 4, true>, front_long_lds(long_cap));
    } else {
        static std::atomic<int> cache[64][2][2];
        v = cache[dev & 63][wide][w8].load(std::memory_order_relaxed);
        if (v == 0) {
            v = resident(wpb == 4 ? (wide ? (const void *) k_front<2, 4> : (const void *) k_front<1, 4>) : (wide ? (const void *) k_front<2, 8> : (const void *) k_front<1, 8>), 0);
            cache[dev & 63][wide][w8].store(v, std::memory_order_relaxed);
        }
    }
    return (3 * S / (wpb == 4 ? 16 : 32)) * std::max(rows, 1) <= v - 1;
}
void front(const FrontArgs & a, hipStream_t st, bool long_kv) {
    const int rows = a.rows > 1 ? a.rows : 1;
    if (long_kv) {
        const dim3 grid(3 * a.S / 16, 1);
        const size_t lds = front_long_lds(a.cap);
        if (a.S <= 512) hipLaunchKernelGGL((k_front<1, 4, true>), grid, dim3(256), lds, st, a, stamp_next());
        else            hipLaunchKernelGGL((k_front<2, 4, true>), grid, dim3(256), lds, st, a, stamp_next());
    } else
    if (front_wpb(rows) == 4) {
        const dim3 grid(3 * a.S / 16, rows);
        if (a.S <= 512) hipLaunchKernelGGL((k_front<1, 4>), grid, dim3(256), 0, st, a, stamp_next());
        else            hipLaunchKernelGGL((k_front<2, 4>), grid, dim3(256), 0, st, a, stamp_next());
    } else {
        const dim3 grid(3 * a.S / 32, rows);
        if (a.S <= 512) hipLaunchKernelGGL((k_front<1, 8>), grid, dim3(512), 0, st, a, stamp_next());
        else            hipLaunchKernelGGL((k_front<2, 8>), grid, dim3(512), 0, st, a, stamp_next());
    }
}

void gemv(const GemvArgs & a, hipStream_t st) {
    const Stamp sp = stamp_next();
    if (sp.base) { GemvArgs b = a; b.stamps = sp.base; b.stamp_slot = sp.slot; gemv_(b, st); return; }
    gemv_(a, st);
}
static bool rows_on_mfma(const GemvArgs & a) {
    return a.lanes && a.n >= 2 && a.n <= 16 && !a.sa_q && (!a.comb_o || a.N < 8192) && (a.K % 128) == 0 &&
           (a.epi != EPI_QKV_DEC || (a.S % 16) == 0) && (!g_rows_valu || a.n > 8);
}
bool gemv_rows_carries_mirror(const GemvArgs & a) { return rows_on_mfma(a) && a.N >= 8192; }
bool gemv_rows_take_self_attention(const GemvArgs & a) {
    const int nch = (a.K + 511) / 512, hpw = (a.K / 64 + 3) / 4;
    const bool inst = (nch == 1 && (hpw == 1 || hpw == 2)) || (nch == 2 && (hpw == 3 || hpw == 4)) || (nch == 3 && (hpw == 5 || hpw == 4));
    return a.lanes && a.n >= 2 && a.n <= 16 && a.N < 8192 && a.K <= 2048 && (a.K % 64) == 0 && a.epi == EPI_F32_BIAS_RESID && inst;
}
static void gemv_(const GemvArgs & a, hipStream_t st) {
    if (a.lanes && a.n >= 2 && a.n <= 16 && a.N < 8192 && !a.rows && a.K <= 2048 && (a.K % 8) == 0 && (!a.ln_g || a.K <= 1536) && !a.step_copy_src) {
        if (launch_gemv1_special(a, (a.K + 511) / 512, st)) return;
    }
    const bool mfma_ok = rows_on_mfma(a) && !a.sa_q;
    if (mfma_ok) {
        const bool vec = (a.N % 16) == 0 && (a.ldc % 4) == 0 && (!a.resid || (a.ldr % 4) == 0) &&
                         (a.epi != EPI_QKV_DEC || ((a.ldaux % 4) == 0 && (a.ldaux2 % 4) == 0));
        if (a.N >= 8192) { if (a.epi == EPI_LOGITS && (a.ldc % 4) == 0 && !a.bias) launch_rows_mfma<false, EPI_LOGITS>(a, st); else launch_rows_mfma<false>(a, st); }
        else if (vec && a.epi == EPI_QKV_DEC)        launch_rows_mfma<true, EPI_QKV_DEC>(a, st);
        else if (vec && a.epi == EPI_F32_BIAS_RESID) launch_rows_mfma<true, EPI_F32_BIAS_RESID>(a, st);
        else if (vec && a.epi == EPI_F16_BIAS_GELU)  launch_rows_mfma<true, EPI_F16_BIAS_GELU>(a, st);
        else launch_rows_mfma<true>(a, st);
        return;
    }
    const bool plain = !a.ln_g && !a.sa_q && !a.comb_o;
    if (a.n == 1 && !a.lanes && a.K > 2048 && a.K <= 5120 && (a.K % 8) == 0 && plain && launch_gemv1_special(a, (a.K + 511) / 512, st)) return;
    if (a.n == 1 && !a.lanes && a.K <= 2048 && (a.K % 8) == 0 && (!a.ln_g || a.K <= 1536)) {
        const int nch = (a.K + 511) / 512;
        if (launch_gemv1_special(a, nch, st)) return;
// ... 23 lines not shown
```

godot-whisper_amd/csrc/k_gemm.hip:

```cpp

#include "kernels.h"
#include "wave_ops.h"
#include "gemm_epi.h"

#include <cstdlib>
#include <type_traits>

namespace wmi { namespace k {

namespace {

using namespace gemm_detail;

constexpr int BK = 64;

__device__ __forceinline__ uint32_t lds_off(int row, int chunk) {
    return (uint32_t) (row * 128 + ((chunk ^ (row & 7)) << 4));
}

template <int BM, int BN, int EPI, int NST = 2, int NW = 4>
__global__ __launch_bounds__(NW * 64) void k_gemm(const GemmArgs a) {
    constexpr int WN_ = NW / 2;
    constexpr int FM = BM / 32, FN = BN / (WN_ * 16);
    constexpr int LA = BM / (NW * 8), LB = BN / (NW * 8);
    extern __shared__ __attribute__((aligned(16))) unsigned char smem[];
    auto sA = [&](int buf) -> unsigned char * { return smem + buf * ((BM + BN) * 128); };
    auto sB = [&](int buf) -> unsigned char * { return smem + buf * ((BM + BN) * 128) + BM * 128; };

    const int tid = threadIdx.x, lane = tid & 63, wave = tid >> 6;
    const int wm = wave / WN_, wn = wave % WN_;
    const unsigned long long pt0 = a.probe ? wall_clock64() : 0ull;
    unsigned long long pt1 = 0ull, pt2 = 0ull;

    const int ntm = (a.M + BM - 1) / BM, ntn = (a.N + BN - 1) / BN, nwg = ntm * ntn;
    int wg = blockIdx.x;
    {
        const int q = nwg / 8, r = nwg % 8, xcd = wg % 8, idx = wg / 8;
        wg = (xcd < r ? xcd * (q + 1) : r * (q + 1) + (xcd - r) * q) + idx;
    }
    const int tm = wg / ntn, tn = wg % ntn;
    const int m0 = tm * BM, n0 = tn * BN;

    const int srow = tid >> 3, schunk = tid & 7;
    const __half * gA[LA]; const __half * gB[LB];
#pragma unroll
    for (int p = 0; p < LA; ++p) {
        int r = m0 + p * (NW * 8) + srow; if (r > a.M - 1) r = a.M - 1;
        gA[p] = a.A + (size_t) r * a.lda + schunk * 8;
    }
#pragma unroll
    for (int p = 0; p < LB; ++p) {
        int r = n0 + p * (NW * 8) + srow; if (r > a.N - 1) r = a.N - 1;
        gB[p] = a.W + (size_t) r * a.ldw + schunk * 8;
    }

    floatx4 acc[FM][FN];
#pragma unroll
    for (int i = 0; i < FM; ++i)
#pragma unroll
        for (int j = 0; j < FN; ++j) acc[i][j] = floatx4{0.f, 0.f, 0.f, 0.f};

    const int nk = (a.K + BK - 1) / BK;
    const int ktail = a.K - (nk - 1) * BK;
    uint4 ra[LA], rb[LB];

    auto load_tile = [&](int kt) {
        const bool half_only = (kt == nk - 1) && (ktail < BK) && (schunk >= 4);
#pragma unroll
        for (int p = 0; p < LA; ++p) ra[p] = half_only ? uint4{0, 0, 0, 0} : *(const uint4 *) (gA[p] + kt * BK);
#pragma unroll
        for (int p = 0; p < LB; ++p) rb[p] = half_only ? uint4{0, 0, 0, 0} : *(const uint4 *) (gB[p] + kt * BK);
    };
    auto store_tile = [&](int buf) {
#pragma unroll
        for (int p = 0; p < LA; ++p) *(uint4 *) (sA(buf) + lds_off(p * (NW * 8) + srow, schunk)) = ra[p];
#pragma unroll
        for (int p = 0; p < LB; ++p) *(uint4 *) (sB(buf) + lds_off(p * (NW * 8) + srow, schunk)) = rb[p];
    };

    const int frow = lane & 15, fq = lane >> 4;
#ifdef WMI_GEMM_NO_SWAP
    constexpr bool SWAP = false;
#else
    constexpr bool SWAP = EPI != EPI_QKV_DEC;
#endif
    const bool big = a.M >= 4096;
    const bool swap = SWAP && !(EPI == EPI_QKV_ENC && (n0 >= 2 * a.S || (big && !(a.no_glds & 8)))) && !(EPI == EPI_F32_BIAS_RESID && big && !(a.no_glds & 32));
    auto compute = [&](int buf, auto sw_tag) {
        constexpr bool SWF = decltype(sw_tag)::value;
#pragma unroll
        for (int kk = 0; kk < 2; ++kk) {
            half8 fa[FM], fb[FN];
#pragma unroll
            for (int i = 0; i < FM; ++i)
                fa[i] = *(const half8 *) (sA(buf) + lds_off(wm * (BM / 2) + i * 16 + frow, kk * 4 + fq));
#pragma unroll
            for (int j = 0; j < FN; ++j)
                fb[j] = *(const half8 *) (sB(buf) + lds_off(wn * (BN / WN_) + j * 16 + frow, kk * 4 + fq));
#pragma unroll
            for (int i = 0; i < FM; ++i)
#pragma unroll
                for (int j = 0; j < FN; ++j) {
                    if constexpr (SWF) acc[i][j] = __builtin_amdgcn_mfma_f32_16x16x32_f16(fb[j], fa[i], acc[i][j], 0, 0, 0);
                    else               acc[i][j] = __builtin_amdgcn_mfma_f32_16x16x32_f16(fa[i], fb[j], acc[i][j], 0, 0, 0);
                }
        }
    };

    auto k_loops = [&](auto sw_tag) {
    if ((BM >= 96 || nwg <= 1024) && (a.K % BK) == 0 && !(a.no_glds & 1)) {
        constexpr int PA = BM / (NW * 8), PB = BN / (NW * 8);
        const int prow = lane >> 3;
        const __half * qA[PA]; const __half * qB[PB];
#pragma unroll
        for (int p = 0; p < PA; ++p) {
            const int lrow = (wave * PA + p) * 8 + prow, pch = (lane & 7) ^ (lrow & 7);
            int r = m0 + lrow; if (r > a.M - 1) r = a.M - 1;
            qA[p] = a.A + (size_t) r * a.lda + pch * 8;
        }
#pragma unroll
        for (int p = 0; p < PB; ++p) {
            const int lrow = (wave * PB + p) * 8 + prow, pch = (lane & 7) ^ (lrow & 7);
            int r = n0 + lrow; if (r > a.N - 1) r = a.N - 1;
            qB[p] = a.W + (size_t) r * a.ldw + pch * 8;
        }
        const uint32_t lds0 = lds_addr(smem);
        auto issue = [&](int kt, int buf) {
#pragma unroll
            for (int p = 0; p < PA; ++p)
                glds_asm<16>(qA[p] + kt * BK, lds0 + buf * ((BM + BN) * 128) + (wave * PA + p) * 1024);
#pragma unroll
            for (int p = 0; p < PB; ++p)
                glds_asm<16>(qB[p] + kt * BK, lds0 + buf * ((BM + BN) * 128) + BM * 128 + (wave * PB + p) * 1024);
        };
        constexpr int LPT = PA + PB;
#pragma unroll
        for (int s0 = 0; s0 < NST - 1; ++s0) if (s0 < nk) issue(s0, s0);
        for (int kt = 0; kt < nk; ++kt) {
            if (nk - 1 - kt >= NST - 2) asm volatile("s_waitcnt vmcnt(%0)" :: "n"((NST - 2) * LPT) : "memory");
            else                        asm volatile("s_waitcnt vmcnt(0)" ::: "memory");
            __builtin_amdgcn_s_barrier();
            asm volatile("" ::: "memory");
            if (a.probe && kt == 0) pt1 = wall_clock64();
            if (kt + NST - 1 < nk) issue(kt + NST - 1, (kt + NST - 1) % NST);
            compute(kt % NST, sw_tag);
        }
        if (a.probe) { asm volatile("s_nop 0" ::: "memory"); pt2 = wall_clock64(); }
    } else {
        load_tile(0);
        store_tile(0);
        __syncthreads();
        for (int kt = 0; kt < nk; ++kt) {
            const int buf = kt & 1;
            if (kt + 1 < nk) load_tile(kt + 1);
            compute(buf, sw_tag);
            if (kt + 1 < nk) store_tile(buf ^ 1);
            __syncthreads();
        }
    }
    };
    constexpr bool RT_ORIENT = SWAP && (EPI == EPI_QKV_ENC || EPI == EPI_F32_BIAS_RESID);
    if constexpr (!SWAP) k_loops(std::false_type{});
    else if constexpr (!RT_ORIENT) k_loops(std::true_type{});
    else { if (swap) k_loops(std::true_type{}); else k_loops(std::false_type{}); }

    const int mb = m0 + wm * (BM / 2), nb = n0 + wn * (BN / WN_);
    const bool interior = m0 + BM <= a.M && n0 + BN <= a.N && !(a.no_glds & 2);
    constexpr bool WIDE_OK = FN % 2 == 0 && (EPI == EPI_F16_BIAS || EPI == EPI_F16_BIAS_GELU || EPI == EPI_Q_SCALED || EPI == EPI_F32_BIAS_RESID ||
                                             EPI == EPI_CROSS_KV || EPI == EPI_QKV_ENC);
    if (SWAP && swap) {
        if constexpr (WIDE_OK) {
            if (!(a.no_glds & 4)) {
                if (interior) epilogue_cols_wide<EPI, FM, FN, false>(a, acc, mb, nb, n0, lane); else epilogue_cols_wide<EPI, FM, FN, true>(a, acc, mb, nb, n0, lane);
            } else {
                if (interior) epilogue_cols<EPI, FM, FN, false>(a, acc, mb, nb, n0, lane); else epilogue_cols<EPI, FM, FN, true>(a, acc, mb, nb, n0, lane);
            }
        } else {
            if (interior) epilogue_cols<EPI, FM, FN, false>(a, acc, mb, nb, n0, lane); else epilogue_cols<EPI, FM, FN, true>(a, acc, mb, nb, n0, lane);
        }
    }
    else              { if (interior) epilogue_rows<EPI, FM, FN, false>(a, acc, mb, nb, lane);     else epilogue_rows<EPI, FM, FN, true>(a, acc, mb, nb, lane); }
    if (a.probe && tid == 0) {
        asm volatile("s_waitcnt vmcnt(0)" ::: "memory");
        unsigned hwid; asm volatile("s_getreg_b32 %0, hwreg(HW_REG_HW_ID)" : "=s"(hwid));
        unsigned long long * o = a.probe + (size_t) blockIdx.x * 5;
        o[0] = pt0; o[1] = pt1; o[2] = pt2; o[3] = wall_clock64(); o[4] = hwid;
    }
}

template <int BM, int BN, int EPI, int NST, int NW = 4>
void launch_n(const GemmArgs & a, hipStream_t st) {
    const int ntm = (a.M + BM - 1) / BM, ntn = (a.N + BN - 1) / BN;
    const size_t smem = NST * (size_t) (BM + BN) * 128;
    static std::atomic<uint64_t> lds_ok{0};
    allow_full_lds((const void *) k_gemm<BM, BN, EPI, NST, NW>, lds_ok);
    hipLaunchKernelGGL((k_gemm<BM, BN, EPI, NST, NW>), dim3(ntm * ntn), dim3(NW * 64), smem, st, a);
}
template <int BM, int BN, int EPI>
void launch(const GemmArgs & a, hipStream_t st) {
    const long nwg = (long) ((a.M + BM - 1) / BM) * ((a.N + BN - 1) / BN);
    if (BM < 128 && nwg <= 400) launch_n<BM, BN, EPI, 4>(a, st);
    else                        launch_n<BM, BN, EPI, 2>(a, st);
}

template <int EPI>
void dispatch(const GemmArgs & a, hipStream_t st) {
    const long t128 = (long) ((a.M + 127) / 128) * ((a.N + 127) / 128);
    const long t64 = (long) ((a.M + 63) / 64) * ((a.N + 63) / 64);
    static const int wide = getenv("WMI_GEMM_WIDE") ? atoi(getenv("WMI_GEMM_WIDE")) : 0;
    const long t256 = (long) ((a.M + 127) / 128) * (a.N / 256);
    if constexpr (EPI == EPI_F16_BIAS_GELU || EPI == EPI_QKV_ENC || EPI == EPI_CROSS_KV || EPI == EPI_F16_BIAS) {
        if (wide && (a.N % 256) == 0 && t256 >= 384 && (a.K % BK) == 0 && !(a.no_glds & 1)) { launch_n<128, 256, EPI, 3, 8>(a, st); return; }
    }
    if constexpr (EPI == EPI_F32_BIAS_RESID) {
        const long t192 = (long) ((a.M + 191) / 192) * (a.N / 128);
        if (a.M >= 4096 && a.N <= 1024 && (a.N % 128) == 0 && (a.K % BK) == 0 && !(a.no_glds & 1) && (a.K >= 1024 || t192 >= 200)) {
            launch_n<192, 128, EPI, 4, 8>(a, st); return;
        }
    }
    if (t128 >= 320 || (t128 >= 256 && a.K >= 1024)) {
        if constexpr (EPI == EPI_QKV_ENC || EPI == EPI_F32_BIAS_RESID || EPI == EPI_CONV2 || EPI == EPI_F16_BIAS_GELU) {
            const long t96 = (long) ((a.M + 95) / 96) * ((a.N + 127) / 128);
            auto fill = [](long t) { return (double) t / (double) (((t + 511) / 512) * 512); };
            if (a.M >= 4096 && (a.K % BK) == 0 && fill(t96) > fill(t128) + 0.08) { launch_n<96, 128, EPI, 2>(a, st); return; }
        }
        launch<128, 128, EPI>(a, st);
    }
    else if constexpr (EPI == EPI_F32_BIAS_RESID) {
        if (a.K >= 1024 && (a.N % 128) == 0 && (a.K % BK) == 0 && t64 >= 400 && !(a.no_glds & 1)) { launch_n<64, 128, EPI, 4>(a, st); return; }
        if (t64 < 256) launch<64, 32, EPI>(a, st); else launch<64, 64, EPI>(a, st);
    }
    else             launch<64, 64, EPI>(a, st);
}

}

static thread_local GemmLog * tl_gemm_log = nullptr;
void gemm_log_install(GemmLog * log) { tl_gemm_log = log; }

void gemm(int epi, const GemmArgs & a_in, hipStream_t st) {
    static const bool no_glds = getenv("WMI_GEMM_NO_GLDS") != nullptr;
    static const bool guard_all = getenv("WMI_GEMM_GUARD_ALL") != nullptr;
    static const bool narrow = getenv("WMI_GEMM_NARROW_STORES") != nullptr;
    static const bool qkv_swap = getenv("WMI_GEMM_QKV_SWAP") != nullptr;
    static const bool resid_swap = getenv("WMI_GEMM_RESID_SWAP") != nullptr;
    static const bool vt_narrow = getenv("WMI_GEMM_VT_NARROW") != nullptr;
    GemmArgs a = a_in; a.no_glds = (no_glds ? 1 : 0) | (guard_all ? 2 : 0) | (narrow ? 4 : 0) | (qkv_swap ? 8 : 0) | (vt_narrow ? 16 : 0) | (resid_swap ? 32 : 0);
    if (GemmLog * lg = tl_gemm_log) {
        const size_t wgs = (size_t) ((a.M + 63) / 64) * (size_t) ((a.N + 31) / 32);
        if (!a.probe && lg->used + wgs * 5 <= lg->cap_words) {
            a.probe = lg->buf + lg->used;
            lg->entries.push_back(GemmLogEntry{epi, a.M, a.N, a.K, lg->used, (int) wgs});
            lg->used += wgs * 5;
        }
    }
    if (!no_glds && (epi == EPI_F16_BIAS_GELU || epi == EPI_CROSS_KV) && a.M >= 4096 && a.N >= 1024 && (a.N % 256) == 0 && (a.K % 64) == 0 &&
        (epi != EPI_CROSS_KV || (a.S % 64) == 0)) {
        const long t192 = (long) ((a.M + 191) / 192) * (a.N / 256);
        if (t192 >= 384) { GemmArgs b = a; b.no_glds = a.no_glds & 16; if (gemm8(epi, 192, true, b, st)) return; }
    }
    if (!no_glds && epi == EPI_QKV_ENC && a.M >= 4096 && (a.N % 256) == 0 && (a.K % 64) == 0 && a.S > 0 && (a.S % 128) == 0 && a.N == 3 * a.S) {
        const long t288 = (long) ((a.M + 287) / 288) * (a.N / 256);
        const long n_cu = cu_count_x8(), rounds = (t288 + n_cu - 1) / n_cu;
        if (t288 * 5 >= rounds * n_cu * 4) { GemmArgs b = a; b.no_glds = a.no_glds & 16; if (gemm8(epi, 288, true, b, st, 32)) return; }
    }
    switch (epi) {
        case EPI_F16_BIAS:       dispatch<EPI_F16_BIAS>(a, st); break;
        case EPI_F16_BIAS_GELU:  dispatch<EPI_F16_BIAS_GELU>(a, st); break;
        case EPI_F32_BIAS_RESID: dispatch<EPI_F32_BIAS_RESID>(a, st); break;
        case EPI_CONV2:          dispatch<EPI_CONV2>(a, st); break;
        case EPI_QKV_ENC:        dispatch<EPI_QKV_ENC>(a, st); break;
        case EPI_QKV_DEC:        dispatch<EPI_QKV_DEC>(a, st); break;
        case EPI_CROSS_KV:       dispatch<EPI_CROSS_KV>(a, st); break;
        case EPI_Q_SCALED:       dispatch<EPI_Q_SCALED>(a, st); break;
        default: break;
    }
}

}}
```

godot-whisper_amd/csrc/k_mel.hip:

```cpp

#include "kernels.h"
#include <type_traits>
#include "wave_ops.h"
#include <climits>
#include <cmath>
#include <mutex>

namespace wmi { namespace k {

namespace {

struct MelTables { float hann[400]; float sinv[400]; float cosv[400]; };
__constant__ MelTables c_mel;

std::atomic<uint64_t> g_tables_mask{0};

void upload_tables() {
    MelTables t;
    for (int i = 0; i < 400; ++i) {
        t.hann[i] = 0.5 * (1.0 - cosf((2.0 * M_PI * i) / 400));
        double theta = (2 * M_PI * i) / 400;
        t.sinv[i] = sinf(theta);
        t.cosv[i] = cosf(theta);
    }
    (void) hipMemcpyToSymbol(HIP_SYMBOL(c_mel), &t, sizeof(t));
}

__device__ inline int enc_ordered(float f) { int i = __float_as_int(f); return i >= 0 ? i : i ^ 0x7FFFFFFF; }
__device__ inline float dec_ordered(int i) { return __int_as_float(i >= 0 ? i : i ^ 0x7FFFFFFF); }

__device__ __forceinline__ void mel_pad_body(const float * __restrict__ pcm, int n, float * __restrict__ out, int total, int * __restrict__ gmax) {
    int i = blockIdx.x * blockDim.x + threadIdx.x;
    if (i == 0 && gmax) *gmax = INT_MIN;
    if (i >= total) return;
    float v = 0.0f;
    if (i < 200) {
        int j = 200 - i; if (j > n - 1) j = n - 1; if (j < 0) j = 0;
        v = n > 0 ? pcm[j] : 0.0f;
    } else if (i < 200 + n) {
        v = pcm[i - 200];
    }
    out[i] = v;
}
__global__ void k_mel_pad(const float * __restrict__ pcm, int n, float * __restrict__ out, int total, int * __restrict__ gmax) { mel_pad_body(pcm, n, out, total, gmax); }
__global__ void k_mel_pad_b(const MelBatch b) { const int c = blockIdx.y; mel_pad_body(b.pcm[c], b.n[c], b.pad[c], b.n[c] + 480400, b.gmax[c]); }

__device__ inline void butterfly_stage(const float * src, float * dst, int ngroups, int N, int tid, int nthreads,
                                       bool last, const float2 * tw) {
    const int half = N / 2;
    const int total = ngroups * half;
    for (int t = tid; t < total; t += nthreads) {
        const int g = t / half, kk = t % half;
        const float2 * E = (const float2 *) src + (g * half);
        const float2 * O = (const float2 *) src + ((g + ngroups) * half);
        const float2 w = tw[kk];
        const float re =  w.x;
        const float im = -w.y;
        const float2 e = E[kk], o = O[kk];
        float2 * D = (float2 *) dst + (g * N);
        D[kk] = make_float2(fmaf(-im, o.y, fmaf(re, o.x, e.x)), fmaf(im, o.x, fmaf(re, o.y, e.y)));
        if (!last || kk == 0)
            D[kk + half] = make_float2(fmaf(im, o.y, fmaf(-re, o.x, e.x)), fmaf(-im, o.x, fmaf(-re, o.y, e.y)));
    }
}

__device__ __forceinline__ void mel_tail_body(float * __restrict__ mel, int n_len, int n_mel, int n_fft_frames, int * __restrict__ gmax) {
    const int w = n_len - n_fft_frames;
    const int i = blockIdx.x * blockDim.x + threadIdx.x;
    if (i < w * n_mel) { const int j = i / w, f = n_fft_frames + (i - j * w); mel[(size_t) j * n_len + f] = -10.0f; }
    if (i == 0 && w > 0) atomicMax(gmax, enc_ordered(-10.0f));
}
__global__ void k_mel_tail(float * __restrict__ mel, int n_len, int n_mel, int n_fft_frames, int * __restrict__ gmax) { mel_tail_body(mel, n_len, n_mel, n_fft_frames, gmax); }

constexpr int MEL_NT = 256;
__device__ __forceinline__ void mel_frames_body(const float * __restrict__ pad, int n_valid, int n_fft_frames,
                                                    int n_len, int n_mel, const float * __restrict__ filters,
                                                    const int32_t * __restrict__ ranges, const float * __restrict__ taps,
                                                    float * __restrict__ mel, int * __restrict__ gmax) {
    __shared__ float xin[400];
    __shared__ __attribute__((aligned(8))) float bufA[800];
    __shared__ __attribute__((aligned(8))) float bufB[800];
    __shared__ float pw[204];
    __shared__ __attribute__((aligned(8))) float2 tw25[25], tw50[25], tw100[50], tw200[100], tw400[200];
    const int frame = blockIdx.x;
    const int tid = threadIdx.x;
    if (frame >= n_fft_frames) return;

    const int offset = frame * 160;
    int nin = n_valid - offset; if (nin > 400) nin = 400;
    {
        static_assert(MEL_NT == 256, "two samples per thread");
        const int j0 = tid, j1 = tid + 256;
        const int j1c = j1 < 400 ? j1 : 0, jt = tid < 200 ? tid : 0, j25 = tid < 25 ? tid : 0, j50 = tid < 50 ? tid : 0, j100 = tid < 100 ? tid : 0;
        const float h0 = c_mel.hann[j0], h1 = c_mel.hann[j1c];
        const float p0 = pad[offset + (j0 < nin ? j0 : 0)], p1 = pad[offset + (j1c < nin ? j1c : 0)];
        const float2 w25 = make_float2(c_mel.cosv[16 * j25], c_mel.sinv[16 * j25]), w50 = make_float2(c_mel.cosv[8 * j25], c_mel.sinv[8 * j25]);
        const float2 w100 = make_float2(c_mel.cosv[4 * j50], c_mel.sinv[4 * j50]);
        const float2 w200 = make_float2(c_mel.cosv[2 * j100], c_mel.sinv[2 * j100]);
        const float2 w400 = make_float2(c_mel.cosv[jt], c_mel.sinv[jt]);
        xin[j0] = j0 < nin ? h0 * p0 : 0.0f;
        if (j1 < 400) xin[j1] = j1 < nin ? h1 * p1 : 0.0f;
        if (tid < 25)  { tw25[tid] = w25; tw50[tid] = w50; }
        if (tid < 50)  tw100[tid] = w100;
        if (tid < 100) tw200[tid] = w200;
        if (tid < 200) tw400[tid] = w400;
    }
    int fr0 = 0, fr1 = 0;
    if (tid < n_mel) { fr0 = ranges[2 * tid]; fr1 = ranges[2 * tid + 1]; }
    constexpr int FW = 12;
    float fw[FW][4], f200 = 0.0f;
    {
        const float4 * tp = (const float4 *) taps + (size_t) (tid < n_mel ? tid : 0) * 13;
        float4 tv[FW + 1];
#pragma unroll
        for (int q = 0; q <= FW; ++q) tv[q] = tp[q];
#pragma unroll
        for (int q = 0; q < FW; ++q) { fw[q][0] = tv[q].x; fw[q][1] = tv[q].y; fw[q][2] = tv[q].z; fw[q][3] = tv[q].w; }
        f200 = tv[FW].x;
    }
    __syncthreads();

    for (int t = tid; t < 400; t += MEL_NT) {
        const int r = t / 25, kk = t % 25;
        float re = 0.0f, im = 0.0f;
        int idx = 0;
#pragma unroll 5
        for (int m = 0; m < 25; ++m) {
            const float v = xin[r + 16 * m];
            const float2 w = tw25[idx];
            re = fmaf(v, w.x, re);
            im = fmaf(-v, w.y, im);
            idx += kk; if (idx >= 25) idx -= 25;
        }
        bufA[2 * (r * 25 + kk)]     = re;
        bufA[2 * (r * 25 + kk) + 1] = im;
    }
    __syncthreads();
    butterfly_stage(bufA, bufB, 8, 50, tid, MEL_NT, false, tw50);   __syncthreads();
    butterfly_stage(bufB, bufA, 4, 100, tid, MEL_NT, false, tw100); __syncthreads();
    butterfly_stage(bufA, bufB, 2, 200, tid, MEL_NT, false, tw200); __syncthreads();
    butterfly_stage(bufB, bufA, 1, 400, tid, MEL_NT, true, tw400);  __syncthreads();

    for (int j = tid; j < 201; j += MEL_NT) {
        const float re = bufA[2 * j], im = bufA[2 * j + 1];
        pw[j] = fmaf(re, re, im * im);
    }
    __syncthreads();

    float vmax = -INFINITY;
    for (int j = tid; j < n_mel; j += MEL_NT) {
        if (j != tid) { fr0 = ranges[2 * j]; fr1 = ranges[2 * j + 1]; }
        const float * f = filters + (size_t) j * 201;
        double sum = 0.0;
        if (j == tid) {
#pragma unroll
            for (int q = 0; q < FW; ++q) {
                if (fr0 + q < fr1) {
                    const int kk = 4 * (fr0 + q);
                    float g = pw[kk] * fw[q][0];
                    g = fmaf(pw[kk + 1], fw[q][1], g);
                    g = fmaf(pw[kk + 2], fw[q][2], g);
                    g = fmaf(pw[kk + 3], fw[q][3], g);
                    sum += (double) g;
                }
            }
        }
        for (int g4 = (j == tid ? fr0 + FW : fr0); g4 < fr1; ++g4) {
            const int kk = 4 * g4;
            float g = pw[kk] * f[kk];
            g = fmaf(pw[kk + 1], f[kk + 1], g);
            g = fmaf(pw[kk + 2], f[kk + 2], g);
            g = fmaf(pw[kk + 3], f[kk + 3], g);
            sum += (double) g;
        }
        sum += (double) (pw[200] * (j == tid ? f200 : f[200]));
        sum = log10(sum > 1e-10 ? sum : 1e-10);
        const float v = (float) sum;
        mel[(size_t) j * n_len + frame] = v;
        vmax = fmaxf(vmax, v);
    }
    _Pragma("unroll") for (int o = 32; o > 0; o >>= 1) vmax = fmaxf(vmax, WMI_SHX(vmax, o));
    __shared__ float s_vmax[MEL_NT / 64];
    if ((tid & 63) == 0) s_vmax[tid >> 6] = vmax;
    __syncthreads();
    if (tid == 0) {
        float v = s_vmax[0];
        for (int w = 1; w < MEL_NT / 64; ++w) v = fmaxf(v, s_vmax[w]);
        if (v > -INFINITY) {
            const int e = enc_ordered(v);
            if (e > __hip_atomic_load(gmax, __ATOMIC_RELAXED, __HIP_MEMORY_SCOPE_AGENT)) atomicMax(gmax, e);
        }
    }
}
__global__ __launch_bounds__(MEL_NT) void k_mel_frames(const float * __restrict__ pad, int n_valid, int n_fft_frames,
                                                    int n_len, int n_mel, const float * __restrict__ filters,
                                                    const int32_t * __restrict__ ranges, const float * __restrict__ taps,
                                                    float * __restrict__ mel, int * __restrict__ gmax) {
    mel_frames_body(pad, n_valid, n_fft_frames, n_len, n_mel, filters, ranges, taps, mel, gmax);
}
__device__ __forceinline__ int mel_n_len(int n) { return (int) (((long long) n + 480000) / 160); }
__device__ __forceinline__ int mel_n_fft(int n) { const int a = (n + 200) / 160 + 1, l = mel_n_len(n); return a < l ? a : l; }
__global__ __launch_bounds__(MEL_NT) void k_mel_frames_b(const MelBatch b, int n_mel, const float * __restrict__ filters,
                                                      const int32_t * __restrict__ ranges, const float * __restrict__ taps) {
    const int c = blockIdx.y, n = b.n[c];
    mel_frames_body(b.pad[c], n + 200, mel_n_fft(n), mel_n_len(n), n_mel, filters, ranges, taps, b.mel[c], b.gmax[c]);
}
__global__ void k_mel_tail_b(const MelBatch b, int n_mel) {
    const int c = blockIdx.y, n = b.n[c];
    mel_tail_body(b.mel[c], mel_n_len(n), n_mel, mel_n_fft(n), b.gmax[c]);
}

__device__ __forceinline__ void mel_normalize_body(float * __restrict__ mel, int n, const int * __restrict__ gmax) {
    int i = blockIdx.x * blockDim.x + threadIdx.x;
    if (i >= n) return;
    const double mmax = (double) dec_ordered(*gmax) - 8.0;
    float v = mel[i];
    if ((double) v < mmax) v = (float) mmax;
    mel[i] = (float) (((double) v + 4.0) / 4.0);
}
__global__ void k_mel_normalize(float * __restrict__ mel, int n, const int * __restrict__ gmax) { mel_normalize_body(mel, n, gmax); }
__global__ void k_mel_normalize_b(const MelBatch b, int n_mel) { const int c = blockIdx.y; mel_normalize_body(b.mel[c], n_mel * mel_n_len(b.n[c]), b.gmax[c]); }

__global__ void k_mel_slice(const float * __restrict__ mel, int n_len, int n_mel, int offset, int n_frames,
                            __half * __restrict__ out, int ld, int rows_total) {
    __shared__ float tile[32][33];
    const int r0 = blockIdx.x * 32, c0 = blockIdx.y * 32;
    const int tx = threadIdx.x & 31, ty = threadIdx.x >> 5;
    for (int j = ty; j < 32; j += 8) {
        const int c = c0 + j, r = r0 + tx;
        const int fr = offset + r - 1;
        float v = 0.0f;
        if (c < n_mel && r >= 1 && r <= n_frames && fr < n_len && fr >= 0) v = mel[(size_t) c * n_len + fr];
        tile[j][tx] = v;
    }
    __syncthreads();
    for (int j = ty; j < 32; j += 8) {
        const int r = r0 + j, c = c0 + tx;
        if (r < rows_total && c < ld) out[(size_t) r * ld + c] = f2h(c < n_mel ? tile[tx][j] : 0.0f);
    }
}

__global__ void k_mel_slice_batch(const MelSliceBatch mb, int n_mel, int n_frames, __half * __restrict__ out, int ld, int rows_total) {
    __shared__ float tile[32][33];
    const int ch = blockIdx.z;
    const float * __restrict__ mel = mb.mel[ch]; const int n_len = mb.n_len[ch], offset = mb.offset[ch];
    out += (size_t) ch * rows_total * ld;
    const int r0 = blockIdx.x * 32, c0 = blockIdx.y * 32;
    const int tx = threadIdx.x & 31, ty = threadIdx.x >> 5;
    for (int j = ty; j < 32; j += 8) {
        const int c = c0 + j, r = r0 + tx;
        const int fr = offset + r - 1;
        float v = 0.0f;
        if (c < n_mel && r >= 1 && r <= n_frames && fr < n_len && fr >= 0) v = mel[(size_t) c * n_len + fr];
        tile[j][tx] = v;
    }
    __syncthreads();
    for (int j = ty; j < 32; j += 8) {
        const int r = r0 + j, c = c0 + tx;
        if (r < rows_total && c < ld) out[(size_t) r * ld + c] = f2h(c < n_mel ? tile[tx][j] : 0.0f);
    }
}
__global__ void k_fill_zero_strided(uint32_t * p, size_t words, size_t stride_words, int count) {
    const size_t i = (size_t) blockIdx.x * blockDim.x + threadIdx.x;
    if (i < words && (int) blockIdx.y < count) p[(size_t) blockIdx.y * stride_words + i] = 0u;
}

__device__ __forceinline__ void signal_energy_body(const float * __restrict__ x, int n, int hw, float * __restrict__ out,
                                                       float * __restrict__ bmin, float * __restrict__ bmax) {
    __shared__ float s_min[4], s_max[4];
    for (int blk = blockIdx.x; blk * 256 < n; blk += gridDim.x) {
    if (blk != (int) blockIdx.x) __syncthreads();
    const int i = blk * blockDim.x + threadIdx.x;
    float v = 0.0f;
    if (hw <= 64) {
        __shared__ float tile[256 + 128];
        const int base = blk * 256 - hw;
        for (int t = threadIdx.x; t < 256 + 2 * hw; t += 256) { const int k = base + t; tile[t] = (k >= 0 && k < n) ? fabsf(x[k]) : 0.0f; }
        __syncthreads();
        if (i < n) {
            float sum = 0.0f;
            for (int j = 0; j <= 2 * hw; ++j) sum = sum + tile[threadIdx.x + j];
            v = sum / (float) (2 * hw + 1);
            out[i] = v;
        }
        __syncthreads();
    } else
    if (i < n) {
        float sum = 0.0f;
        for (int j = -hw; j <= hw; ++j) {
            const int k = i + j;
            if (k >= 0 && k < n) sum = (float) ((double) sum + fabs((double) x[k]));
        }
        v = sum / (float) (2 * hw + 1);
        out[i] = v;
    }
    float lo = i < n ? v : INFINITY, hi = i < n ? v : -INFINITY;
    _Pragma("unroll") for (int o = 32; o > 0; o >>= 1) { lo = fminf(lo, WMI_SHX(lo, o)); hi = fmaxf(hi, WMI_SHX(hi, o)); }
    if ((threadIdx.x & 63) == 0) { s_min[threadIdx.x >> 6] = lo; s_max[threadIdx.x >> 6] = hi; }
    __syncthreads();
    if (threadIdx.x == 0) {
        bmin[blk] = fminf(fminf(s_min[0], s_min[1]), fminf(s_min[2], s_min[3]));
        bmax[blk] = fmaxf(fmaxf(s_max[0], s_max[1]), fmaxf(s_max[2], s_max[3]));
    }
    }
}
__global__ __launch_bounds__(256) void k_signal_energy(const float * __restrict__ x, int n, int hw, float * __restrict__ out,
                                                       float * __restrict__ bmin, float * __restrict__ bmax) { signal_energy_body(x, n, hw, out, bmin, bmax); }
__global__ __launch_bounds__(256) void k_signal_energy_b(const MelBatch b, int hw) {
    const int c = blockIdx.y;
    signal_energy_body(b.pcm[c], b.n[c], hw, b.energy[c], b.bmin[c], b.bmax[c]);
}

__global__ void k_downmix(const float2 * __restrict__ frames, int n, float * __restrict__ out) {
    const int i = blockIdx.x * blockDim.x + threadIdx.x;
    if (i < n) { const float2 f = frames[i]; out[i] = (float) ((double) (f.x + f.y) / 2.0); }
}

__global__ __launch_bounds__(256) void k_vad(const float * __restrict__ x, int n, int n_last, float alpha, int filter, float vad_thold,
                                             float * __restrict__ res) {
    constexpr int CHUNK = 8192;
    __shared__ __attribute__((aligned(16))) float buf[CHUNK];
    float y = 0.0f, e_all = 0.0f, e_last = 0.0f;
    const int first_last = n - n_last;
    for (int c0 = 0; c0 < n; c0 += CHUNK) {
        const int m = min(CHUNK, n - c0);
        for (int i = threadIdx.x; i < m; i += 256) buf[i] = x[c0 + i];
        __syncthreads();
        if (threadIdx.x == 0) {
            auto run = [&](int i0, int i1, auto tail_tag) {
                constexpr bool TAIL = decltype(tail_tag)::value;
                int i = i0;
                for (; i < i1 && (i & 3); ++i) {
                    float v = buf[i];
                    if (filter) { y = __fmul_rn(alpha, __fsub_rn(__fadd_rn(y, v), y)); v = y; }
                    e_all = __fadd_rn(e_all, fabsf(v));
                    if (TAIL) e_last = __fadd_rn(e_last, fabsf(v));
                }
                for (; i + 8 <= i1; i += 8) {
                    const float4 a4 = *(const float4 *) (buf + i), b4 = *(const float4 *) (buf + i + 4);
                    const float v8[8] = {a4.x, a4.y, a4.z, a4.w, b4.x, b4.y, b4.z, b4.w};
#pragma unroll
                    for (int u = 0; u < 8; ++u) {
                        float v = v8[u];
                        if (filter) { y = __fmul_rn(alpha, __fsub_rn(__fadd_rn(y, v), y)); v = y; }
                        e_all = __fadd_rn(e_all, fabsf(v));
                        if (TAIL) e_last = __fadd_rn(e_last, fabsf(v));
                    }
                }
                for (; i < i1; ++i) {
                    float v = buf[i];
                    if (filter) { y = __fmul_rn(alpha, __fsub_rn(__fadd_rn(y, v), y)); v = y; }
                    e_all = __fadd_rn(e_all, fabsf(v));
                    if (TAIL) e_last = __fadd_rn(e_last, fabsf(v));
                }
            };
            int i0 = 0;
            if (c0 == 0) {
                const float v = buf[0];
                if (filter) y = v;
                e_all = __fadd_rn(e_all, fabsf(v));
                if (first_last <= 0) e_last = __fadd_rn(e_last, fabsf(v));
                i0 = 1;
            }
            const int split = min(max(first_last - c0, i0), m);
            run(i0, split, std::false_type{});
            run(split, m, std::true_type{});
        }
        __syncthreads();
    }
    if (threadIdx.x == 0) {
        e_all /= (float) n;
        if (n_last != 0) e_last /= (float) n_last;
        const bool quiet = !(!(e_all < 0.0001f && e_last < 0.0001f) || e_last > vad_thold * e_all);
        res[0] = quiet ? 1.0f : 0.0f; res[1] = e_all; res[2] = e_last;
    }
}

__global__ void k_fill_zero(uint32_t * p, size_t n) {
    size_t i = (size_t) blockIdx.x * blockDim.x + threadIdx.x;
    const size_t stride = (size_t) gridDim.x * blockDim.x;
    for (; i < n; i += stride) p[i] = 0u;
}

__global__ void k_set_int(int * p, int v) { *p = v; }

}

void mel_pad(const float * pcm, int n_samples, float * pcm_pad, int n_pad_total, hipStream_t st, int * gmax_reset) {
    hipLaunchKernelGGL(k_mel_pad, dim3((n_pad_total + 255) / 256), dim3(256), 0, st, pcm, n_samples, pcm_pad, n_pad_total, gmax_reset);
}

void mel_frames(const float * pcm_pad, int n_valid, int n_fft_frames, int n_len, int n_mel, const float * filters,
                const int32_t * ranges, const float * taps, float * mel, int * gmax, hipStream_t st) {
    {
        int dev = 0; (void) hipGetDevice(&dev);
        const uint64_t bit = 1ull << (dev & 63);
        if (!(g_tables_mask.load(std::memory_order_acquire) & bit)) { upload_tables(); g_tables_mask.fetch_or(bit, std::memory_order_release); }
    }
    if (n_fft_frames > 0)
        hipLaunchKernelGGL(k_mel_frames, dim3(n_fft_frames), dim3(MEL_NT), 0, st, pcm_pad, n_valid, n_fft_frames, n_len, n_mel,
                           filters, ranges, taps, mel, gmax);
    const int tail = (n_len - n_fft_frames) * n_mel;
    if (tail > 0) hipLaunchKernelGGL(k_mel_tail, dim3((tail + 255) / 256), dim3(256), 0, st, mel, n_len, n_mel, n_fft_frames, gmax);
}

void mel_batch(const MelBatch & b, int nb, int n_mel, const float * filters, const int32_t * ranges, const float * taps, hipStream_t st) {
    {
        int dev = 0; (void) hipGetDevice(&dev);
        const uint64_t bit = 1ull << (dev & 63);
        if (!(g_tables_mask.load(std::memory_order_acquire) & bit)) { upload_tables(); g_tables_mask.fetch_or(bit, std::memory_order_release); }
    }
    int n_max = 0, n_min = INT_MAX;
    for (int c = 0; c < nb; ++c) { n_max = std::max(n_max, b.n[c]); n_min = std::min(n_min, b.n[c]); }
    auto n_len = [](int n) { return (int) (((long long) n + 480000) / 160); };
    auto n_fft = [&](int n) { return std::min((n + 200) / 160 + 1, n_len(n)); };
    hipLaunchKernelGGL(k_mel_pad_b, dim3((n_max + 480400 + 255) / 256, nb), dim3(256), 0, st, b);
    hipLaunchKernelGGL(k_mel_frames_b, dim3(n_fft(n_max), nb), dim3(MEL_NT), 0, st, b, n_mel, filters, ranges, taps);
    int tail_max = 0;
    for (int c = 0; c < nb; ++c) tail_max = std::max(tail_max, (n_len(b.n[c]) - n_fft(b.n[c])) * n_mel);
    if (tail_max > 0) hipLaunchKernelGGL(k_mel_tail_b, dim3((tail_max + 255) / 256, nb), dim3(256), 0, st, b, n_mel);
    hipLaunchKernelGGL(k_mel_normalize_b, dim3((n_mel * n_len(n_max) + 255) / 256, nb), dim3(256), 0, st, b, n_mel);
}
void signal_energy_batch(const MelBatch & b, int nb, int hw, hipStream_t st) {
    int n_max = 0;
    for (int c = 0; c < nb; ++c) n_max = std::max(n_max, b.n[c]);
    if (n_max > 0) hipLaunchKernelGGL(k_signal_energy_b, dim3((n_max + 255) / 256, nb), dim3(256), 0, st, b, hw);
}

void mel_normalize(float * mel, int n, const int * gmax, hipStream_t st) {
    hipLaunchKernelGGL(k_mel_normalize, dim3((n + 255) / 256), dim3(256), 0, st, mel, n, gmax);
}

void mel_slice(const float * mel, int n_len, int n_mel, int offset, int n_frames, __half * out, int ld, int rows_total,
               hipStream_t st) {
    dim3 grid((rows_total + 31) / 32, (ld + 31) / 32);
    hipLaunchKernelGGL(k_mel_slice, grid, dim3(256), 0, st, mel, n_len, n_mel, offset, n_frames, out, ld, rows_total);
}

void mel_slice_batch(const MelSliceBatch & mb, int nb, int n_mel, int n_frames, __half * out, int ld, int rows_total, hipStream_t st) {
    dim3 grid((rows_total + 31) / 32, (ld + 31) / 32, nb);
    hipLaunchKernelGGL(k_mel_slice_batch, grid, dim3(256), 0, st, mb, n_mel, n_frames, out, ld, rows_total);
}
void fill_zero_strided(void * p, size_t bytes, size_t stride_bytes, int count, hipStream_t st) {
    if (count <= 0 || bytes == 0) return;
    hipLaunchKernelGGL(k_fill_zero_strided, dim3((unsigned) ((bytes / 4 + 255) / 256), count), dim3(256), 0, st, (uint32_t *) p, bytes / 4, stride_bytes / 4, count);
}

void signal_energy(const float * pcm, int n, int hw, float * out, float * bmin, float * bmax, hipStream_t st) {
    const int nblk = (n + 255) / 256;
    hipLaunchKernelGGL(k_signal_energy, dim3(nblk), dim3(256), 0, st, pcm, n, hw, out, bmin, bmax);
}

__device__ __forceinline__ int ts_walk(const float * __restrict__ en, const float * __restrict__ bext, int k, int bound, float th, int dir, bool above, int lane) {
    for (;;) {
        const int dist = dir > 0 ? bound - k : k - bound;
        if (dist <= 0) return k;
        const bool edge = dir > 0 ? (k & 255) == 0 : (k & 255) == 255;
        if (edge) {
            const int b = (k >> 8) + dir * lane;
            const bool inside = dir > 0 ? ((b + 1) << 8) <= bound : (b >= 0 && (b << 8) > bound);
            bool cont = false;
            if (inside) { const float e = bext[b]; cont = above ? e > th : e < th; }
            const unsigned long long m = __ballot(cont);
            const int nskip = m == ~0ull ? 64 : __builtin_ctzll(~m);
            if (nskip > 0) { k += dir * 256 * nskip; continue; }
        }
        const int to_edge = dir > 0 ? 256 - (k & 255) : (k & 255) + 1;
        int cnt = dist + 1; if (cnt > 64) cnt = 64; if (cnt > to_edge) cnt = to_edge;
        const int p = k + dir * lane;
        bool stop = false;
        if (lane < cnt) { const float x = en[p]; stop = p == bound || !(above ? x > th : x < th); }
        const unsigned long long m = __ballot(stop);
        if (m) return k + dir * __builtin_ctzll(m);
        k += dir * cnt;
    }
}

__device__ __forceinline__ float ts_trip_exact(float acc, const float (&x)[16], int n_left, int lane) {
#pragma unroll
    for (int sub = 0; sub < 4; ++sub) {
        const int b0 = sub * 256;
        if (b0 >= n_left) break;
        const uint32_t bits = __float_as_uint(acc);
        const int E = (int) ((bits >> 23) & 0xFF) - 127;
        bool done = false;
        if (b0 + 256 <= n_left && (bits >> 31) == 0 && E >= -100 && E <= 100) {
            const uint32_t units = (bits & 0x7FFFFFu) | 0x800000u;
            const float scale = __uint_as_float((uint32_t) (127 + 23 - E) << 23);
            bool bad = false; uint32_t isum = 0;
#pragma unroll
            for (int k = 0; k < 4; ++k) {
                const float tt = x[sub * 4 + k] * scale;
                const int q = __float2int_rn(tt);
                const float d = fabsf(tt - (float) q);
                bad = bad || d == 0.5f || !(tt < 8388608.0f) || tt < 0.0f;
                isum += (uint32_t) q;
            }
            if (__ballot(bad) == 0) {
                _Pragma("unroll") for (int o = 32; o > 0; o >>= 1) isum += (uint32_t) __shfl_xor((int) isum, o);
                const unsigned long long total = (unsigned long long) units + isum;
                if (total < 0x1000000ull) { acc = __uint_as_float(((uint32_t) (E + 127) << 23) | ((uint32_t) total & 0x7FFFFFu)); done = true; }
            }
        }
        if (!done) {
#pragma unroll
            for (int k = 0; k < 4; ++k) {
                const int c0 = b0 + k * 64;
                const int cnt = n_left - c0 < 64 ? n_left - c0 : 64;
                const float v = x[sub * 4 + k];
                if (cnt >= 64) {
#pragma unroll
                    for (int l = 0; l < 64; ++l) acc = acc + __builtin_bit_cast(float, __builtin_amdgcn_readlane(__builtin_bit_cast(int, v), l));
                } else {
                    for (int l = 0; l < cnt; ++l) acc = acc + __shfl(v, l);
                }
            }
        }
    }
    return acc;
}

constexpr int TS_W = 8;
__global__ __launch_bounds__(TS_W * 64) void k_ts_refine(const float * __restrict__ en_, const float * __restrict__ bmin_, const float * __restrict__ bmax_,
                                                         int n_samples_, const TsTok * __restrict__ in, TsOut * __restrict__ out) {
    __shared__ uint32_t s_sum[TS_W]; __shared__ int s_bad[TS_W]; __shared__ float s_acc;
    const int tid = threadIdx.x, lane = tid & 63, wave = tid >> 6;
    const TsTok t = in[blockIdx.x];
    const float * __restrict__ en = t.en ? t.en : en_;
    const int n_samples = t.en ? t.n_samples : n_samples_;
    const float * __restrict__ bmin = t.en ? t.en + t.ext_off : bmin_;
    const float * __restrict__ bmax = t.en ? bmin + ((size_t) t.n_samples / 256 + 2) : bmax_;
    float acc = 0.0f;
    {
        const float * p = en + t.a0;
        const int n = t.a1 - t.a0;
        auto fetch = [&](float (&dst)[16], int base) {
#pragma unroll
            for (int r = 0; r < 16; ++r) { const int e = base + r * 64 + lane; dst[r] = (e >= 0 && e < n) ? p[e] : 0.0f; }
        };
        float x[16], nx[16]; int nx_base = -1;
        int i = 0;
        while (i < n) {
            const int base = i + wave * 1024;
            if (nx_base == base) {
#pragma unroll
                for (int r = 0; r < 16; ++r) x[r] = nx[r];
            } else fetch(x, base);
            nx_base = base + TS_W * 1024;
            if (nx_base < n) fetch(nx, nx_base); else nx_base = -1;
            const uint32_t bits = __float_as_uint(acc);
            const int E = (int) ((bits >> 23) & 0xFF) - 127;
            const bool fast = (bits >> 31) == 0 && E >= -100 && E <= 100;
            bool bad = !fast || base + 1024 > n;
            uint32_t isum = 0;
            if (!bad) {
                const float scale = __uint_as_float((uint32_t) (127 + 23 - E) << 23);
#pragma unroll
                for (int r = 0; r < 16; ++r) {
                    const float tt = x[r] * scale;
                    const int q = __float2int_rn(tt);
                    const float d = fabsf(tt - (float) q);
                    bad = bad || d == 0.5f || !(tt < 8388608.0f) || tt < 0.0f;
                    isum += (uint32_t) q;
                }
                bad = bad || isum >= 0x1000000u;
                bad = __ballot(bad) != 0;
                if (!bad) { _Pragma("unroll") for (int o = 32; o > 0; o >>= 1) isum += (uint32_t) __shfl_xor((int) isum, o); }
            }
            if (lane == 0) { s_sum[wave] = isum; s_bad[wave] = bad ? 1 : 0; }
            __syncthreads();
            int k = 0;
            if (fast) {
                uint32_t running = (bits & 0x7FFFFFu) | 0x800000u;
                for (; k < TS_W; ++k) {
                    if (s_bad[k] || (unsigned long long) running + s_sum[k] >= 0x1000000ull) break;
                    running += s_sum[k];
                }
                if (k > 0) acc = __uint_as_float(((uint32_t) (E + 127) << 23) | (running & 0x7FFFFFu));
            }
            i += k * 1024;
            const bool slow = k < TS_W && i < n;
            if (slow) {
                if (wave == 0) {
// ... 54 lines not shown
```

godot-whisper_amd/csrc/k_norm.hip:

```cpp

#include "kernels.h"
#include "wave_ops.h"

namespace wmi { namespace k {

namespace {

template <int MAXV>
__global__ __launch_bounds__(256) void k_layernorm(const float * __restrict__ x, int rows, int S,
                                                   const float * __restrict__ g, const float * __restrict__ b, float eps,
                                                   __half * __restrict__ out16, float * __restrict__ out32, int rpc_in, int rpc_out) {
    const int lane = threadIdx.x & 63;
    const int row = blockIdx.x * 4 + (threadIdx.x >> 6);
    if (row >= rows) return;
    const float * xr = x + (size_t) row * S;
    const int orow = rpc_in > 0 ? (row / rpc_in) * rpc_out + row % rpc_in : row;
    float4 v[MAXV], gg[MAXV], bb[MAXV];
#pragma unroll
    for (int i = 0; i < MAXV; ++i) {
        const int c = (i * 64 + lane) * 4, cc = c < S ? c : 0;
        v[i] = *(const float4 *) (xr + cc); gg[i] = *(const float4 *) (g + cc); bb[i] = *(const float4 *) (b + cc);
    }
    float sum = 0.0f;
#pragma unroll
    for (int i = 0; i < MAXV; ++i) {
        const int c = (i * 64 + lane) * 4;
        if (c < S) sum += (v[i].x + v[i].y) + (v[i].z + v[i].w);
        else v[i] = make_float4(0.f, 0.f, 0.f, 0.f);
    }
    _Pragma("unroll") for (int o = 32; o > 0; o >>= 1) sum += WMI_SHX(sum, o);
    const float mean = sum / (float) S;
    float sq = 0.0f;
#pragma unroll
    for (int i = 0; i < MAXV; ++i) {
        const int c = (i * 64 + lane) * 4;
        if (c < S) {
            v[i].x -= mean; v[i].y -= mean; v[i].z -= mean; v[i].w -= mean;
            sq += (v[i].x * v[i].x + v[i].y * v[i].y) + (v[i].z * v[i].z + v[i].w * v[i].w);
        }
    }
    _Pragma("unroll") for (int o = 32; o > 0; o >>= 1) sq += WMI_SHX(sq, o);
    const float scale = 1.0f / sqrtf(sq / (float) S + eps);
#pragma unroll
    for (int i = 0; i < MAXV; ++i) {
        const int c = (i * 64 + lane) * 4;
        if (c < S) {
            float4 y;
            y.x = __fadd_rn(__fmul_rn(v[i].x * scale, gg[i].x), bb[i].x);
            y.y = __fadd_rn(__fmul_rn(v[i].y * scale, gg[i].y), bb[i].y);
            y.z = __fadd_rn(__fmul_rn(v[i].z * scale, gg[i].z), bb[i].z);
            y.w = __fadd_rn(__fmul_rn(v[i].w * scale, gg[i].w), bb[i].w);
            if (out32) *(float4 *) (out32 + (size_t) orow * S + c) = y;
            if (out16) {
                __half2 h01 = __floats2half2_rn(pin_f32(y.x), pin_f32(y.y)), h23 = __floats2half2_rn(pin_f32(y.z), pin_f32(y.w));
                uint2 pk; pk.x = *(uint32_t *) &h01; pk.y = *(uint32_t *) &h23;
                *(uint2 *) (out16 + (size_t) orow * S + c) = pk;
            }
        }
    }
}

}

void layernorm(const float * x, int rows, int S, const float * g, const float * b, float eps,
               __half * out16, float * out32, hipStream_t st, int rows_per_chunk_in, int rows_per_chunk_out) {
    if (rows <= 0) return;
    const dim3 grid((rows + 3) / 4), block(256);
    const int nv = (S + 255) / 256;
    if (nv <= 2)      hipLaunchKernelGGL((k_layernorm<2>), grid, block, 0, st, x, rows, S, g, b, eps, out16, out32, rows_per_chunk_in, rows_per_chunk_out);
    else if (nv <= 4) hipLaunchKernelGGL((k_layernorm<4>), grid, block, 0, st, x, rows, S, g, b, eps, out16, out32, rows_per_chunk_in, rows_per_chunk_out);
    else              hipLaunchKernelGGL((k_layernorm<8>), grid, block, 0, st, x, rows, S, g, b, eps, out16, out32, rows_per_chunk_in, rows_per_chunk_out);
}

}}
```

godot-whisper_amd/csrc/kernels.h:

```cpp
#pragma once
#include <memory>
#include <vector>
#include <hip/hip_runtime.h>
#include <hip/hip_fp16.h>
#include <atomic>
#include <cstdint>

namespace wmi { namespace k {

inline void allow_full_lds(const void * kernel, std::atomic<uint64_t> & mask) {
    int dev = 0;
    (void) hipGetDevice(&dev);
    const uint64_t bit = 1ull << (dev & 63);
    if (mask.load(std::memory_order_acquire) & bit) return;
    (void) hipFuncSetAttribute(kernel, hipFuncAttributeMaxDynamicSharedMemorySize, 160 * 1024);
    mask.fetch_or(bit, std::memory_order_release);
}

#if defined(__HIPCC__)
__device__ __forceinline__ float pin_f32(float x) { asm volatile("" : "+v"(x)); return x; }
__device__ __forceinline__ __half f2h(float x) { return __float2half_rn(pin_f32(x)); }
__host__ __device__ __forceinline__ int vt_pos(int t) { return (t & ~12) | ((t & 4) << 1) | ((t & 8) >> 1); }
#endif

inline int cu_count_x8() {
    static std::atomic<int> cache[64];
    int dev = 0;
    (void) hipGetDevice(&dev);
    std::atomic<int> & c = cache[dev & 63];
    int n = c.load(std::memory_order_relaxed);
    if (n > 0) return n;
    n = 256;
    (void) hipDeviceGetAttribute(&n, hipDeviceAttributeMultiprocessorCount, dev);
    n = n > 8 ? n & ~7 : 8;
    c.store(n, std::memory_order_relaxed);
    return n;
}

#if defined(__HIPCC__)
#define WMI_ARG_NOW(x) asm volatile("" :: "s"(x))
#endif

constexpr int STAMP_WAVES = 4096;
struct Stamp { unsigned long long * base; int slot; };
void  stamp_enable(unsigned long long * base);
Stamp stamp_next();
int   stamp_count();
#if defined(__HIPCC__)
__device__ __forceinline__ unsigned long long stamp_t0(const unsigned long long * base) { return base ? wall_clock64() : 0ull; }
__device__ __forceinline__ void stamp_end(unsigned long long * base, int slot, int widx, unsigned long long t0,
                                          unsigned long long tm1 = 0, unsigned long long tm2 = 0) {
    if (base && (threadIdx.x & 63) == 0 && widx < STAMP_WAVES) {
        unsigned long long * s = base + ((size_t) slot * STAMP_WAVES + widx) * 4;
        s[0] = t0; s[1] = wall_clock64(); s[2] = tm1; s[3] = tm2;
    }
}
#endif

void mel_pad(const float * pcm, int n_samples, float * pcm_pad, int n_pad_total, hipStream_t st, int * gmax_reset);
void mel_frames(const float * pcm_pad, int n_valid, int n_fft_frames, int n_len, int n_mel,
                const float * filters, const int32_t * ranges, const float * taps, float * mel, int * gmax, hipStream_t st);
void mel_normalize(float * mel, int n, const int * gmax, hipStream_t st);
struct MelBatch { const float * pcm[16]; float * pad[16]; float * mel[16]; int * gmax[16]; float * energy[16]; float * bmin[16]; float * bmax[16]; int n[16]; };
void mel_batch(const MelBatch & b, int nb, int n_mel, const float * filters, const int32_t * ranges, const float * taps, hipStream_t st);
void signal_energy_batch(const MelBatch & b, int nb, int hw, hipStream_t st);
struct MelSliceBatch { const float * mel[16]; int n_len[16]; int offset[16]; };
void mel_slice_batch(const MelSliceBatch & mb, int nb, int n_mel, int n_frames, __half * out, int ld, int rows_total, hipStream_t st);
void fill_zero_strided(void * p, size_t bytes, size_t stride_bytes, int count, hipStream_t st);
void mel_slice(const float * mel, int n_len, int n_mel, int offset, int n_frames, __half * out, int ld,
               int rows_total, hipStream_t st);

void signal_energy(const float * pcm, int n, int hw, float * out, float * bmin, float * bmax, hipStream_t st);
struct TsTok { int32_t s0, s1, a0, a1;
               const float * en; int32_t n_samples, ext_off; };
struct TsOut { float sum, thold; int32_t e0, e1;
               int32_t w_down_above_s0, w_up_below_s0, w_up_above_s1, w_down_below_s1; };
void ts_refine(const float * en, const float * bmin, const float * bmax, int n_samples, const TsTok * in, TsOut * out, int n_tok, hipStream_t st);

void downmix_stereo(const float * frames, int n_frames, float * out, hipStream_t st);
void vad_window(const float * x, int n, int n_last, float alpha, bool filter, float vad_thold, float * res, hipStream_t st);

struct Stepper;
struct ResamplePlan {
    int error = 0;
    int converter = 2;
    long long n_out = 0, n_used = 0;
    int half_len = 0, index_inc = 0, increment = 0;
    double float_inc = 0.0, out_scale = 0.0;
    bool need_table = false;
    std::shared_ptr<Stepper> stepper;
};
bool sinc_table(int converter, const float ** coeffs, int * count, int * increment);
ResamplePlan resample_plan(long long n_in, long long out_cap, double ratio, int converter);
void resample_table(const ResamplePlan & pl, const int ** pos, const double ** frac);
void resample_positions(const ResamplePlan & pl, long long n, long long * pos, double * frac);
void resample_launch(const ResamplePlan & pl, const float * d_in, long long n_in, float * d_out, const float * d_coeffs,
                     const int * d_pos, const double * d_frac, hipStream_t st);

enum Epi : int {
    EPI_F16_BIAS = 0,
    EPI_F16_BIAS_GELU,
    EPI_F32_BIAS_RESID,
    EPI_CONV2,
    EPI_QKV_ENC,
    EPI_QKV_DEC,
    EPI_CROSS_KV,
    EPI_Q_SCALED,
};
struct GemmArgs {
    const __half * A;  int lda;
    const __half * W;  int ldw;
    int M, N, K;
    const float * bias;
    void *  C;   int ldc;
    const float * resid; int ldr;
    void *  aux; int ldaux;
    void *  aux2; int ldaux2;
    float   scale;
    int     S;
    int64_t layer_stride;
    int     rows_per_chunk;
    int64_t chunk_stride_aux2;
    int     no_glds;
    unsigned long long * probe;
};
void gemm(int epi, const GemmArgs & a, hipStream_t st);
struct GemmLogEntry { int epi, M, N, K; size_t off; int cap; };
struct GemmLog { unsigned long long * buf = nullptr; size_t cap_words = 0, used = 0; std::vector<GemmLogEntry> entries; };
void gemm_log_install(GemmLog * log);
bool gemm8(int epi, int bm, bool swapped, const GemmArgs & a, hipStream_t st, int ks = 64);

void layernorm(const float * x, int rows, int S, const float * g, const float * b, float eps,
               __half * out16, float * out32, hipStream_t st, int rows_per_chunk_in = 0, int rows_per_chunk_out = 0);

void attn_encoder2(const __half * q, const __half * k, const __half * vt, int T, int Tpad, int S, int H, __half * out, hipStream_t st,
                   int B, float * out32, bool one_sweep, bool split, int qk_chunk_rows = 0);
void attn_encoder(const __half * q, const __half * k, const __half * vt, int T, int Tpad, int S, int H,
                  float scale, __half * out, hipStream_t st, int B = 1, float * out32 = nullptr,
                  int qk_chunk_rows = 0);
void attn_decoder(const __half * q, int n, int S, int H, const __half * kc, const __half * vc, int n_kv,
                  const float * mask, int ld_mask, __half * out, hipStream_t st,
                  const int32_t * n_kv_dev = nullptr, int n_kv_max = 0,
                  float * out32 = nullptr);

void attn_cross_split(const __half * q, int n, int S, int H, const __half * kc, const __half * vc, int T,
                      float * scratch, __half * out, hipStream_t st, int64_t kv_row_stride = 0, float * out32 = nullptr);
void attn_cross_split_partials(const __half * q, int n, int S, int H, const __half * kc, const __half * vc, int T,
                               float * scratch, const float ** part_o, const float ** part_l, const float ** part_m, int * ns, hipStream_t st,
                               int64_t kv_row_stride = 0);
struct XattnPlan { int ns, ks; float * pmax, * part_l, * part_o; bool fused, head_major; };
XattnPlan attn_cross_plan(int n, int H, int T, float * scratch);
void attn_cross_qsplit_partials(const float * x32, const float * ln_g, const float * ln_b, float eps, const __half * wq,
                                const float * bq, float qscale, int n, int S, int H, const __half * kc, const __half * vc, int T,
                                float * scratch, const float ** part_o, const float ** part_l, const float ** part_m, int * ns, hipStream_t st,
                                int64_t kv_row_stride = 0);
size_t attn_cross_scratch_floats(int n, int H, int T);

void dec_embed(const int32_t * tokens, const int32_t * pos, int n, int S, const __half * te, const float * pe,
               float * x, hipStream_t st);
struct FsMaxIdx { float v; int i; };
struct FsPartial { FsMaxIdx all, txt, ts; float sum, sum_ts; float pad[2]; };
constexpr int FS_MAX_PARTS = 768;
struct GemvArgs {
    const float * x32; const float * ln_g; const float * ln_b; float eps;
    const __half * a16;
    int n, K, N;
    const __half * W; const float * bias;
    int epi;
    void * C; int ldc;
    const float * resid; int ldr;
    void * aux; int ldaux; void * aux2; int ldaux2;
    float scale; int S;
    const int32_t * rows;
    const int32_t * row_off;
    const float * comb_o; const float * comb_l; int comb_ns;
    const float * comb_m;
    const __half * sa_q; const __half * sa_k; const __half * sa_v; const int32_t * sa_nkv; int sa_cap;
    int lanes; int step_stride; int64_t cache_row_stride;
    const void * step_copy_src; void * step_copy_dst;
    const void * rows_mirror_src; void * rows_mirror_dst;
    const void * pf_ptr; uint32_t pf_group_bytes; uint32_t pf_groups;
    unsigned long long * stamps; int stamp_slot;
    const uint8_t * fs_ban; const void * fs_step; FsPartial * fs_part;
    int ksplit; float * kpart;
    const float * pend;
};
int gemv_fused_parts(const GemvArgs & a);
bool gemv_rows_carries_mirror(const GemvArgs & a);
bool gemv_rows_take_self_attention(const GemvArgs & a);
void self_attn_rows(const __half * q, int n, int K, const __half * kc, const __half * vc, int64_t cache_row_stride,
                    const int32_t * n_kv, int step_stride, int cap, __half * out, hipStream_t st, float * out32 = nullptr,
                    bool long_cache = false,
                    const void * mirror_src = nullptr, void * mirror_dst = nullptr);
void set_xattn_probe_skip(int mask);
void attn_cross_partials_layout(int n, int H, int T, float * scratch, const float ** po, const float ** pl, const float ** pm, int * pns);
void attn_cross_combine(const float * part_o, const float * part_l, const float * part_m, int ns, int n, int S, int H, __half * out, hipStream_t st,
                        float * out32 = nullptr);
enum { EPI_LOGITS = 100 };
void gemv(const GemvArgs & a, hipStream_t st);

struct MlpPairArgs {
    const float * x; const float * ln_g, * ln_b; float eps; int S;
    const __half * W1; const float * b1; const __half * W2; const float * b2;
    uint32_t * epoch; int par; void * hand;
    uint32_t * fault; uint32_t spin_cap;
    int withhold;
    const void * step_copy_src; void * step_copy_dst;
    __half * h_out;
};
enum : uint32_t { PAIR_FAULT_TIMEOUT = 1u, PAIR_FAULT_PARITY = 2u, PAIR_SLOW = 4u };
constexpr uint32_t PAIR_SLOW_POLLS = 64;
bool mlp_pair_usable(int S, bool with_mirror);
void mlp_pair(const MlpPairArgs & a, float * x_inout, hipStream_t st);
struct FrontArgs {
    const float * x; float * xout; const float * ln_g, * ln_b; float eps; int S;
    const __half * Wqkv; const float * bqkv; float scale; __half * q16; __half * ck, * cv;
    const int32_t * kv_head, * n_kv; int cap;
    const __half * Wo; const float * bo;
    unsigned long long * gq, * ga; uint32_t * epoch; int par; uint32_t * fault; uint32_t spin_cap; int withhold;
    int64_t cache_row_stride; int step_stride; int rows;
};
struct XbackArgs {
    const float * x; float * xout; const float * ln_g, * ln_b; float eps; int S;
    const __half * wq; const float * bq; float qscale; const __half * kc, * vc; int T, ks, ns;
    float * pmax, * part_o, * part_l;
    const __half * Wo; const float * bo;
    unsigned long long * gp, * ga; uint32_t * epoch; int par; uint32_t * fault; uint32_t spin_cap; int withhold;
    int64_t kv_row_stride; int rows;
};
constexpr int XBACK_ROW_GRANULES = 8 * 8 * 66 + 256;
bool xback_usable(int S, int H, int T, int rows = 1);
void xback(XbackArgs a, int H, float * scratch, hipStream_t st);
bool front_usable(int S, int rows = 1, int long_cap = 0);
void front(const FrontArgs & a, hipStream_t st, bool long_kv = false);
struct Knobs { bool no_mlp_pair; int sa_wpb; bool gemv1_wide_generic; bool host_draws; bool debug_sync; int pair_withhold; uint32_t pair_spin_cap; bool no_front; int front_withhold; bool no_xback; int xback_withhold; int front_wpb; };
const Knobs & knobs();
void reload_knobs();
void set_attn_one_group(bool on);
bool rows_valu_enabled();
void set_rows_valu(bool on);
int  mode_epoch();
void bump_mode_epoch();

struct DecStep {
    int32_t token, pos, n_kv, kv_head;
    int32_t flags;
    int32_t space_id, eot, beg, n_vocab;
    int32_t ts_floor_end;
    int32_t ts_initial_start;
    int32_t seq;
    float   temperature;
    int32_t pad[3];
};
struct alignas(16) SampleOut { int32_t id, tid; float p; int32_t seq0; float plog, pt, ptsum; int32_t seq; };
struct ChainNext { DecStep * step_rw; const __half * te; const float * pe; float * x; int S; int n_pos;
                   const uint32_t * fault; };
constexpr int32_t SAMPLE_SEQ_MASK = 0x0FFFFFFF, SAMPLE_TAG_FAULT = 0x40000000, SAMPLE_TAG_SLOW = 0x20000000;
void filter_argmax(const float * logits, const uint8_t * static_ban, const DecStep * step, SampleOut * out, void * scratch, hipStream_t st,
                   SampleOut * out_host = nullptr, int n_rows = 1, const ChainNext * chain = nullptr, int fused_parts = 0);
size_t filter_scratch_bytes(int n_rows = 1);
void filter_draw(const float * logits, const uint8_t * static_ban, const DecStep * step, const double * u, int k, SampleOut * out,
                 void * scratch, hipStream_t st, int n_rows, int tid_default);
size_t filter_draw_scratch_bytes(int n_rows);
void dec_embed_step(const DecStep * host_step, DecStep * dev_step, int S, const __half * te, const float * pe, float * x, hipStream_t st,
                    int n_rows = 1);

enum QType : int { QT_NONE = 0, QT_Q4_0 = 2, QT_Q4_1 = 3, QT_Q5_0 = 6, QT_Q5_1 = 7, QT_Q8_0 = 8 };
struct QGeom { int qb, hb, file_bytes; bool has_m; };
QGeom  q_geom(int qtype);
inline size_t q_tile_bytes(int qtype) { const QGeom g = q_geom(qtype); return (size_t) 64 * (g.qb + g.hb); }
inline size_t q_matrix_bytes(int qtype, int64_t N, int64_t K) { return (size_t) ((N + 31) / 32) * (size_t) (K / 64) * q_tile_bytes(qtype); }
void   q_repack_host(int qtype, const uint8_t * src, int64_t N, int64_t K, uint8_t * dst);
struct QMat { const uint8_t * tiles = nullptr; int qtype = QT_NONE; };

struct Q8Rows { int8_t * qs; float * d; float * s; int ldm; __half * deq = nullptr; __half * wdeq = nullptr; size_t wdeq_elems = 0; bool wdeq_ready = false;
                const void * wdeq_of = nullptr;
                bool w_resident_ok = false; };
bool quantize_rows(const float * x32, const __half * x16, int M, int K, const float * ln_g, const float * ln_b, float eps,
                   int qtype, Q8Rows out, float * out32, __half * out16, hipStream_t st, const QMat * W_next = nullptr, int N_next = 0);

void qgemm(int epi, const GemmArgs & a, Q8Rows A, QMat W, hipStream_t st);
size_t qweights_f16_cached_bytes();
void   qweights_f16_release(const void * lo, const void * hi);
void qdequant(QMat W, int64_t row0, int64_t rows, int K, __half * out, hipStream_t st);

void qrows(const GemvArgs & a, const float * a32, QMat W, hipStream_t st);
bool qrows_ksplit_ok(const GemvArgs & a, int parts);
bool qattn_cross_qsplit_partials(const float * x32, const float * ln_g, const float * ln_b, float eps, QMat Wcq, const float * bq, float qscale,
                                 int n, int S, int H, const __half * kc, const __half * vc, int T, float * scratch,
                                 const float ** po, const float ** pl, const float ** pm, int * pns, hipStream_t st, int64_t kv_row_stride,
                                 QMat pfW, int pfN, int pfK);

void qdec_embed(const int32_t * tokens, const int32_t * pos, int n, int S, QMat te, const float * pe, float * x, hipStream_t st);
void qdec_embed_step(const DecStep * host_step, DecStep * dev_step, int S, QMat te, const float * pe, float * x, hipStream_t st, int n_rows = 1);

void touch(int * p, int blocks, hipStream_t st);
void fill_zero(void * p, size_t bytes, hipStream_t st);

}}
```

godot-whisper_amd/csrc/wmi.h:

```cpp
#pragma once

#include <hip/hip_runtime.h>
#include <hip/hip_fp16.h>

#include <cmath>
#include <cstdint>
#include <cstdio>
#include <map>
#include <functional>
#include <mutex>
#include <random>
#include <set>
#include <string>
#include <vector>

#include "../../include/whisper_mi355.h"
#include "../../include/wmi_device.h"
#include "kernels.h"

namespace wmi {

void log_msg(ggml_log_level lvl, const char * fmt, ...) __attribute__((format(printf, 2, 3)));
#define WMI_ERR(...)  ::wmi::log_msg(GGML_LOG_LEVEL_ERROR, __VA_ARGS__)
#define WMI_WARN(...) ::wmi::log_msg(GGML_LOG_LEVEL_WARN,  __VA_ARGS__)
#define WMI_INFO(...) ::wmi::log_msg(GGML_LOG_LEVEL_INFO,  __VA_ARGS__)

bool hip_ok(hipError_t e, const char * what, const char * file, int line);
#define HIP_OK(expr) ::wmi::hip_ok((expr), #expr, __FILE__, __LINE__)
#define HIP_TRY(expr) do { if (!HIP_OK(expr)) return false; } while (0)

int64_t time_us();

struct HParams {
    int32_t n_vocab = 51864, n_audio_ctx = 1500, n_audio_state = 384, n_audio_head = 6, n_audio_layer = 4;
    int32_t n_text_ctx = 448, n_text_state = 384, n_text_head = 6, n_text_layer = 4, n_mels = 80, ftype = 1;
    float   eps = 1e-5f;
};

struct Vocab {
    int n_vocab = 51864;
    std::map<std::string, int32_t> token_to_id;
    std::vector<std::string>       id_to_token;
    int32_t eot = 50256, sot = 50257, translate = 50357, transcribe = 50358, solm = 50359,
            prev = 50360, nosp = 50361, not_ = 50362, beg = 50363;
    bool is_multilingual() const { return n_vocab >= 51865; }
    int  num_languages()   const { return n_vocab - 51765 - (is_multilingual() ? 1 : 0); }
};

struct FileTensor {
    std::string name;
    int32_t     ttype = 0;
    int32_t     n_dims = 0;
    int64_t     ne[4] = {1, 1, 1, 1};
    size_t      offset = 0, nbytes = 0;
};

struct ModelFile {
    HParams hp;
    int     model_type = 0;
    int     n_filt_mel = 0, n_filt_fft = 0;
    std::vector<float> filters;
    Vocab   vocab;
    std::map<std::string, FileTensor> tensors;
    int     n_loaded = 0;
    bool    quantised = false;
    size_t  header_bytes = 0;
    bool    directory_only = false;
};

bool parse_model(const uint8_t * buf, size_t n, ModelFile & mf);
std::vector<uint8_t> export_header(const ModelFile & mf, const uint8_t * buf, size_t arena_bytes);

struct EncLayerW {
    const float *ln1_g, *ln1_b, *ln2_g, *ln2_b;
    const __half *w_qkv;  const float *b_qkv;
    const __half *w_o;    const float *b_o;
    const __half *w_fc1;  const float *b_fc1;
    const __half *w_fc2;  const float *b_fc2;
    k::QMat q_qkv, q_o, q_fc1, q_fc2;
};
struct DecLayerW {
    const float *ln1_g, *ln1_b, *ln2_g, *ln2_b, *ln3_g, *ln3_b;
    const __half *w_qkv;  const float *b_qkv;
    const __half *w_o;    const float *b_o;
    const __half *w_cq;   const float *b_cq;
    const __half *w_co;   const float *b_co;
    const __half *w_fc1;  const float *b_fc1;
    const __half *w_fc2;  const float *b_fc2;
    k::QMat q_qkv, q_o, q_cq, q_co, q_fc1, q_fc2;
};
struct Weights {
    void *  arena = nullptr;  size_t arena_bytes = 0;
    bool    arena_borrowed = false;
    const __half *conv1_w; const float *conv1_b; int conv1_k = 0;
    const __half *conv2_w; const float *conv2_b; int conv2_k = 0;
    const float  *e_pe;
    std::vector<EncLayerW> enc;
    const float  *e_ln_g, *e_ln_b;
    const __half *w_ckv;   const float *b_ckv;
    k::QMat       q_ckv;
    const float  *d_pe;
    const __half *d_te;
    k::QMat       q_te;
    int           qtype = 0;
    size_t        matrix_bytes = 0;
    std::vector<DecLayerW> dec;
    const float  *d_ln_g, *d_ln_b;
    const float  *mel_filters;
    const float   *mel_taps;
    const int32_t *mel_ranges;
};

bool upload_weights(const ModelFile & mf, const uint8_t * host_buf, Weights & w, hipStream_t st);
bool plan_weights(const ModelFile & mf, Weights & w);
void free_weights(Weights & w);

struct KVCell { int32_t pos = -1; std::set<int32_t> seq; bool has(int32_t s) const { return seq.count(s) != 0; } };
struct KVCache {
    uint32_t head = 0, size = 0, n = 0;
    std::vector<KVCell> cells;
    __half * k = nullptr;  __half * v = nullptr;
};
struct Batch {
    std::vector<int32_t> token, pos, seq_id; std::vector<int8_t> logits;
    int n_tokens = 0;
    void prep_legacy(const int32_t * tokens, int n, int n_past, int seq);
};
bool  kv_find_slot(KVCache & c, const Batch & b);
int   kv_cell_max(const KVCache & c);
void  kv_clear(KVCache & c);
void  kv_seq_rm(KVCache & c, int32_t seq, int32_t p0, int32_t p1);
void  kv_seq_cp(KVCache & c, int32_t src, int32_t dst, int32_t p0, int32_t p1);

struct Sequence {
    std::vector<whisper_token_data> tokens;
    int    result_len = 0;
    double sum_logprobs_all = 0, sum_logprobs = 0, avg_logprobs = 0, entropy = 0, score = 0;
};
struct PartialUtf8 { uint32_t value = 0; int n_remain = 0; };
struct GrammarPos  { int rule, off; };
struct Grammar {
    std::vector<std::vector<whisper_grammar_element>> rules;
    std::vector<std::vector<GrammarPos>> stacks;
    PartialUtf8 partial;
};
struct Decoder {
    Sequence sequence;
    Grammar  grammar;
    int  i_batch = 0, seek_delta = 0;
    bool failed = false, completed = false, has_ts = false;
    std::vector<float> probs, logits, logprobs;
    std::mt19937 rng{0};
};
struct Segment { int64_t t0, t1; std::string text; std::vector<whisper_token_data> tokens; bool speaker_turn_next; };

struct Mel { int n_len = 0, n_len_org = 0, n_mel = 0; };

struct DeviceState {
    hipStream_t stream = nullptr; bool stream_own_queue = false;
    float * pcm = nullptr;      size_t pcm_cap = 0;
    float * mel = nullptr;      size_t mel_cap = 0;
    float * mel_max = nullptr;
    const float * last_pcm = nullptr; int last_pcm_n = 0;
    float * energy = nullptr;   size_t energy_cap = 0;
    float * energy_host = nullptr;
    size_t  energy_dev_cap = 0;
    hipStream_t copy_stream = nullptr; hipEvent_t energy_ev = nullptr;
    hipEvent_t ph_ev[4] = {nullptr, nullptr, nullptr, nullptr}; bool ph_mel = false, ph_enc = false; int64_t ph_host0 = 0;
    hipStream_t energy_wait_stream = nullptr;
    hipStream_t mel_stream = nullptr;  hipEvent_t mel_ev = nullptr;
    bool    energy_pending = false;
    bool    energy_device_only = false;
    void *  ts_host = nullptr;
    __half * mel_t = nullptr;
    __half * conv1 = nullptr;
    float  * x     = nullptr;
    float  * embd_conv = nullptr;
    __half * xn    = nullptr;
    __half * q     = nullptr, * k = nullptr;
    __half * vt    = nullptr;
    __half * att   = nullptr;
    __half * h     = nullptr;
    float  * rowmax = nullptr;
    int8_t * aq = nullptr;  float * ads = nullptr;  int aq_rows = 0;
    __half * aq16 = nullptr, * wq16 = nullptr; size_t wq16_elems = 0;
    float  * att32 = nullptr;
    float  * datt32 = nullptr;
    float  * enc_out = nullptr;
    __half * enc_out_h = nullptr;
    __half * kvc_k = nullptr, * kvc_v = nullptr;
    int      Tpad = 0;
    int      conv1_max_T = 0;
    int32_t * d_tokens = nullptr, * d_pos = nullptr;
    float   * d_mask = nullptr;
    int32_t * d_rows = nullptr;
    float  * dx = nullptr;  __half * dxn = nullptr, * dq = nullptr, * datt = nullptr, * dh = nullptr;
    float  * xattn = nullptr;
    float  * logits = nullptr;  int logits_rows_cap = 0;
    void   * pinned = nullptr;  size_t pinned_bytes = 0;
    void   * step_dev = nullptr;   void * step_host = nullptr;
    void   * sample_dev = nullptr; void * sample_host = nullptr;
    void   * filter_scratch = nullptr;
    uint8_t * ban_dev = nullptr;   uint64_t ban_sig = ~0ull;
    void * mlp_hand = nullptr; unsigned long long * mlp_arrive = nullptr;
    bool pair_off = false; int pair_backoff = 0;
    int  pair_fallbacks = 0, pair_slow_events = 0;
    struct StepGraph { hipGraph_t graph = nullptr; hipGraphExec_t exec = nullptr; int T = -1; int seen = 0; };
    StepGraph step_graphs[8];
    bool chain_valid = false; int32_t chain_token = 0, chain_pos = 0, chain_head = 0;
    int32_t step_seq = 0;
    bool    keep_logits_on_device = false;
    void  * draw_host = nullptr;
    void  * draw_scratch = nullptr;
    bool    step_capture_failed = false;
    int     step_seen_T = -1;
};

struct State {
    std::recursive_mutex mu;
    int     device = 0;
    int64_t t_sample_us = 0, t_encode_us = 0, t_decode_us = 0, t_batchd_us = 0, t_prompt_us = 0, t_mel_us = 0;
    int32_t n_sample = 0, n_encode = 0, n_decode = 0, n_batchd = 0, n_prompt = 0, n_fail_p = 0, n_fail_h = 0;
    KVCache kv_self;
    Mel     mel;
    Batch   batch;
    Decoder decoders[8];
    std::vector<float> logits;
    std::vector<Segment> result_all;
    std::vector<int32_t> prompt_past;
    int     lang_id = 0;
    int64_t t_beg = 0, t_last = 0; int32_t tid_last = 0;
    const float * energy = nullptr; int energy_n = 0;
    const float * energy_bmin = nullptr, * energy_bmax = nullptr;
    bool energy_on_device = false;
    bool ts_failed = false;
    bool ts_hold = false;
    bool ts_defer = false; std::vector<int> ts_pending;
    int32_t exp_n_audio_ctx = 0;
    int     enc_n_ctx = 0;
    DeviceState dev;
};

struct BatchWork {
    int B = 0;
    int Tpad = 0; int qk_rows = 0;
    size_t mel_rows = 0;
    __half * mel_t = nullptr, * conv1 = nullptr;
    float  * x = nullptr;
    __half * xn = nullptr, * q = nullptr, * k = nullptr, * att = nullptr, * vt = nullptr, * h = nullptr, * enc_out_h = nullptr;
    __half * kvc_k = nullptr, * kvc_v = nullptr;
    __half * self_k = nullptr, * self_v = nullptr;
    float  * dx = nullptr; __half * dq = nullptr, * datt = nullptr, * dh = nullptr; float * logits = nullptr, * xattn = nullptr;
    int8_t * aq = nullptr; float * ads = nullptr; int aq_rows = 0; float * att32 = nullptr, * datt32 = nullptr;
    __half * aq16 = nullptr, * wq16 = nullptr; size_t wq16_elems = 0;
    void   * step_dev = nullptr, * step_host = nullptr, * sample_dev = nullptr, * sample_host = nullptr, * filter_scratch = nullptr;
    void   * front_hand = nullptr; bool front_off = false; int front_fallbacks = 0, front_backoff = 0;
    int      enc_rows = 0, enc_T = 0;
    int32_t  step_seq = 0;
    struct RowsGraph { hipGraph_t graph = nullptr; hipGraphExec_t exec = nullptr; int nb = -1, T = -1, rows = -1, epoch = -1, seen = 0; bool failed = false; } rows_graph[4];
    bool chain_valid = false; int chain_nb = 0; int32_t chain_token[16] = {}, chain_pos[16] = {}; bool chain_row_ok[16] = {};
    std::vector<State *> lanes;
    std::vector<std::vector<Segment>> results;
    std::vector<int> redo;
    std::vector<whisper_context *> replicas; int replicas_wanted = -1;
    int groups_wanted = 0, groups_last = 1;
    int64_t t_mel_us = 0, t_encode_us = 0, t_decode_us = 0, t_emit_us = 0; int n_steps = 0, n_chained = 0;
};

}

namespace wmi {
struct StateSlot {
    State * own = nullptr;
    State * get() const;
    operator State * () const { return get(); }
    State * operator->() const { return get(); }
    State & operator*() const { return *get(); }
    StateSlot & operator=(State * s) { own = s; return *this; }
};
struct StateInstall {
    const StateSlot * slot; State * st; StateInstall * prev;
    StateInstall(const StateSlot & sl, State * s);
    ~StateInstall();
    StateInstall(const StateInstall &) = delete; StateInstall & operator=(const StateInstall &) = delete;
};
StateInstall * state_installs_top();
void state_installs_set(StateInstall * top);
}

struct whisper_context {
    int64_t t_load_us = 0, t_start_us = 0;
    whisper_context_params params{};
    wmi::ModelFile model;
    wmi::Weights   w;
    wmi::StateSlot state;
    int            device = 0;
    bool           host_only = false;
    bool           weights_pending = false;
    wmi::BatchWork * batch = nullptr;
    std::vector<hipStream_t> spare_streams;
    float * d_sinc[3] = {nullptr, nullptr, nullptr};
    float * vad_res = nullptr;
    float * dsp_scratch = nullptr; size_t dsp_scratch_bytes = 0;
    std::recursive_mutex mu;
};

namespace wmi {

whisper_context * init_context(const void * buffer, size_t size, int device, bool with_state, bool allow_header = false);
bool compute_ready(const whisper_context & ctx, const char * who);
bool init_state(whisper_context & ctx, bool replica_state = false, hipStream_t adopt = nullptr);
hipStream_t own_queue_stream_get(int device);
void        own_queue_stream_put(int device, hipStream_t s);
void free_state(whisper_context & ctx);
State * create_state(whisper_context & ctx);
void destroy_state(State * st);

bool pcm_to_mel(whisper_context & ctx, const float * samples, int n_samples, bool samples_on_device, bool sync = true, bool defer = false);
int64_t phase_settle(State & st, bool wait);
bool pcm_to_mel_batch(whisper_context & ctx, const std::vector<State *> & states, const float * const * pcm, const int * n_samples,
                      bool samples_on_device, bool envelopes);
bool set_mel(whisper_context & ctx, const float * data, int n_len, int n_mel);
bool encode(whisper_context & ctx, int mel_offset, bool defer = false);
bool encode_rows(whisper_context & ctx, const std::vector<int> & rows, const std::vector<int> & seek, int audio_ctx);
bool decode(whisper_context & ctx, const Batch & batch);
template <typename BUFS> inline k::Q8Rows q8_rows(const BUFS & d, int K) {
    return k::Q8Rows{d.aq, d.ads, d.ads + (size_t) (K / 32) * d.aq_rows, d.aq_rows, d.aq16, d.wq16, d.wq16_elems};
}
bool encode_layers_q(whisper_context & ctx, int T);
struct EncBufsQ {
    int T, nb, Tpad;
    float * x; __half * q, * k, * vt, * h; float * att32; float * enc_out; __half * enc_out_h; __half * kvc_k, * kvc_v;
    k::Q8Rows A, A4;
};
bool encode_layers_q_on(whisper_context & ctx, const EncBufsQ & e, hipStream_t s);
void enqueue_rows_step_q(whisper_context & ctx, int nb);
bool decode_layers_q(whisper_context & ctx, int n, int n_kv, int kv_head, int Tc, const std::vector<int> & rows);
void enqueue_greedy_step_q(whisper_context & ctx, int Tc);
struct StepFilter { bool ban_blank, last_ts, penult_ts; int ts_floor_end, ts_initial_start; };
inline StepFilter make_step_filter(const Vocab & v, const HParams & hp, const whisper_full_params & params, const Decoder & d) {
    const auto & h = d.sequence.tokens;
    StepFilter f{};
    const bool initial = h.empty();
    f.ban_blank = params.suppress_blank && initial;
// ... 59 lines not shown
```

Baseline: 9958 x realtime.

## Fuse layernorm into residual GEMM tails and fold mel padding into frames

Adds an optional path where the residual-add GEMMs in the encoder publish their output rows with coherent stores. A per-panel ticket lets the last block apply the next layernorm directly, removing the standalone layernorm launches. It is gated by WMI_LN_TAIL. Separately, the mel front end now skips the pad kernel by reading PCM directly in mel_frames, and ping-pongs the global max word so normalize can reset the next one. This saves a launch and a pass over the padded buffer. The LN tail adds cross-block synchronization complexity and the risk of ticket-state corruption on errors, which is handled by resetting the tickets on failure.

Result: no change. 10070 x realtime (median of 3 runs) (+1.1%).

```diff
diff --git a/godot-whisper_amd/csrc/device.cpp b/godot-whisper_amd/csrc/device.cpp
--- a/godot-whisper_amd/csrc/device.cpp
+++ b/godot-whisper_amd/csrc/device.cpp
@@ -74,6 +74,7 @@
     ctx.state = st;
     return init_state_into(ctx, st, replica_state, adopt);
 }
+constexpr size_t LN_TICKET_WORDS = 64;
 static bool init_state_into(whisper_context & ctx, State * st, bool replica_state, hipStream_t adopt) {
     const HParams & hp = ctx.model.hp;
     st->device = ctx.device;
@@ -101,7 +102,7 @@
             && dalloc(d.x, T * S) && dalloc(d.embd_conv, T * S) && dalloc(d.xn, T * S)
             && dalloc(d.q, T * S) && dalloc(d.k, T * S) && dalloc(d.vt, S * d.Tpad) && dalloc(d.att, T * S)
             && dalloc(d.h, T * 4 * S) && dalloc(d.rowmax, H * T) && dalloc(d.enc_out, T * S) && dalloc(d.enc_out_h, T * S)
-            && dalloc(d.mel_max, 4);
+            && dalloc(d.mel_max, 4) && dalloc(d.ln_tickets, LN_TICKET_WORDS);
     const size_t n = hp.n_text_ctx;
     if (ctx.model.quantised) {
         const size_t rows = std::max<size_t>(T, n);
@@ -126,6 +127,7 @@
     }
     if (!ok) { WMI_ERR("%s: device allocation failed\n", __func__); return false; }
     k::fill_zero(d.vt, S * d.Tpad * sizeof(__half), d.stream);
+    k::fill_zero(d.ln_tickets, LN_TICKET_WORDS * sizeof(uint32_t), d.stream);
     k::fill_zero(d.conv1, (2 * T + 4) * S * sizeof(__half), d.stream);
     k::fill_zero(d.mel_t, (mel_rows * hp.n_mels + 1024) * sizeof(__half), d.stream);
     k::fill_zero(st->kv_self.k, Lt * n_self * S * sizeof(__half), d.stream);
@@ -166,7 +168,7 @@
     if (d.mel_ev) { (void) hipEventDestroy(d.mel_ev); d.mel_ev = nullptr; }
     dfree(d.energy); if (d.energy_host) (void) hipHostFree(d.energy_host);
     if (d.ts_host) (void) hipHostFree(d.ts_host);
-    dfree(d.pcm); dfree(d.mel); dfree(d.mel_max); dfree(d.mel_t); dfree(d.conv1); dfree(d.x); dfree(d.embd_conv);
+    dfree(d.pcm); dfree(d.mel); dfree(d.mel_max); dfree(d.ln_tickets); dfree(d.mel_t); dfree(d.conv1); dfree(d.x); dfree(d.embd_conv);
     dfree(d.xn); dfree(d.q); dfree(d.k); dfree(d.vt); dfree(d.att); dfree(d.h); dfree(d.rowmax); dfree(d.enc_out);
     dfree(d.enc_out_h); dfree(d.d_tokens); d.d_pos = nullptr; d.d_mask = nullptr; d.d_rows = nullptr; dfree(d.dx); dfree(d.dxn);
     dfree(d.dq); dfree(d.datt); dfree(d.dh); dfree(d.logits); dfree(d.xattn); dfree(d.ban_dev);
@@ -227,9 +229,18 @@
         src = stage;
     }
     d.last_pcm = src; d.last_pcm_n = n_samples;
-    k::mel_pad(src, n_samples, d.pcm, (int) n_pad, ms, (int *) d.mel_max);
-    k::mel_frames(d.pcm, n_valid, n_fft_frames, n_len, n_mel, ctx.w.mel_filters, ctx.w.mel_ranges, ctx.w.mel_taps, d.mel, (int *) d.mel_max, ms);
-    k::mel_normalize(d.mel, n_mel * n_len, (const int *) d.mel_max, ms);
+    if (k::knobs().plain_front) {
+        k::mel_pad(src, n_samples, d.pcm, (int) n_pad, ms, (int *) d.mel_max);
+        k::mel_frames(d.pcm, n_valid, n_fft_frames, n_len, n_mel, ctx.w.mel_filters, ctx.w.mel_ranges, ctx.w.mel_taps, d.mel, (int *) d.mel_max, ms);
+        k::mel_normalize(d.mel, n_mel * n_len, (const int *) d.mel_max, ms);
+    } else {
+        int * words = (int *) d.mel_max + 1;
+        if (!d.mel_words_ready) { k::mel_max_init(words, 2, ms); d.mel_words_ready = true; d.mel_par = 0; }
+        int * gmax = words + d.mel_par, * gnext = words + (d.mel_par ^ 1);
+        d.mel_par ^= 1;
+        k::mel_frames(nullptr, n_valid, n_fft_frames, n_len, n_mel, ctx.w.mel_filters, ctx.w.mel_ranges, ctx.w.mel_taps, d.mel, gmax, ms, src, n_samples);
+        k::mel_normalize(d.mel, n_mel * n_len, gmax, ms, gnext);
+    }
     st.mel.n_len = n_len; st.mel.n_len_org = n_len_org; st.mel.n_mel = n_mel;
     if (defer) { HIP_TRY(hipEventRecord(d.ph_ev[1], ms)); d.ph_mel = true; d.ph_host0 = t0; return true; }
     if (sync) HIP_TRY(hipStreamSynchronize(ms));
@@ -381,7 +392,18 @@
     return true;
 }
 
+static bool encode_launches(whisper_context & ctx, int mel_offset, bool defer);
 bool encode(whisper_context & ctx, int mel_offset, bool defer) {
+    if (encode_launches(ctx, mel_offset, defer)) return true;
+    if (ctx.state && ctx.state->dev.ln_tickets && ctx.state->dev.stream) {
+        DeviceState & d = ctx.state->dev;
+        (void) hipGetLastError();
+        k::fill_zero(d.ln_tickets, LN_TICKET_WORDS * sizeof(uint32_t), d.stream);
+        (void) hipStreamSynchronize(d.stream);
+    }
+    return false;
+}
+static bool encode_launches(whisper_context & ctx, int mel_offset, bool defer) {
     if (!compute_ready(ctx, __func__)) return false;
     State & st = *ctx.state; DeviceState & d = st.dev; const Weights & w = ctx.w; const HParams & hp = ctx.model.hp;
     const int64_t t0 = time_us();
@@ -397,6 +419,9 @@
     hipStream_t s = d.stream;
     if (st.mel.n_mel != nm || d.mel == nullptr) { WMI_ERR("%s: no mel spectrogram (n_mel %d, expected %d)\n", __func__, st.mel.n_mel, nm); return false; }
 
+    const bool ln_tail = !ctx.model.quantised && k::knobs().ln_tail && d.ln_tickets &&
+                         k::gemm_ln_tail_ok(k::EPI_CONV2, T, S, w.conv2_k) && k::gemm_ln_tail_ok(k::EPI_F32_BIAS_RESID, T, S, S) &&
+                         k::gemm_ln_tail_ok(k::EPI_F32_BIAS_RESID, T, S, 4 * S);
     const int rows_mel = 2 * T + 6;
     k::mel_slice(d.mel, st.mel.n_len, nm, mel_offset, 2 * T, d.mel_t, nm, rows_mel, s);
     {
@@ -411,14 +436,16 @@
         k::GemmArgs a{};
         a.A = d.conv1; a.lda = 2 * S; a.W = w.conv2_w; a.ldw = w.conv2_k; a.M = T; a.N = S; a.K = w.conv2_k;
         a.bias = w.conv2_b; a.C = d.x; a.ldc = S; a.resid = w.e_pe; a.ldr = S; a.aux = d.embd_conv; a.ldaux = S;
+        if (ln_tail && La > 0) a.ln = k::GemmLn{w.enc[0].ln1_g, w.enc[0].ln1_b, hp.eps, d.xn, nullptr, d.ln_tickets};
         k::gemm(k::EPI_CONV2, a, s);
     }
+    if (ln_tail && La == 0) k::layernorm(d.x, T, S, w.e_ln_g, w.e_ln_b, hp.eps, d.enc_out_h, d.enc_out, s);
     const float kq_scale = 1.0f / sqrtf((float) S / H);
     if (ctx.model.quantised) { if (!encode_layers_q(ctx, T)) return false; }
     else {
     for (int il = 0; il < La; ++il) {
         const EncLayerW & l = w.enc[il];
-        k::layernorm(d.x, T, S, l.ln1_g, l.ln1_b, hp.eps, d.xn, nullptr, s);
+        if (!ln_tail) k::layernorm(d.x, T, S, l.ln1_g, l.ln1_b, hp.eps, d.xn, nullptr, s);
         {
             k::GemmArgs a{};
             a.A = d.xn; a.lda = S; a.W = l.w_qkv; a.ldw = S; a.M = T; a.N = 3 * S; a.K = S; a.bias = l.b_qkv;
@@ -430,9 +457,10 @@
             k::GemmArgs a{};
             a.A = d.att; a.lda = S; a.W = l.w_o; a.ldw = S; a.M = T; a.N = S; a.K = S; a.bias = l.b_o;
             a.C = d.x; a.ldc = S; a.resid = d.x; a.ldr = S;
+            if (ln_tail) a.ln = k::GemmLn{l.ln2_g, l.ln2_b, hp.eps, d.xn, nullptr, d.ln_tickets};
             k::gemm(k::EPI_F32_BIAS_RESID, a, s);
         }
-        k::layernorm(d.x, T, S, l.ln2_g, l.ln2_b, hp.eps, d.xn, nullptr, s);
+        if (!ln_tail) k::layernorm(d.x, T, S, l.ln2_g, l.ln2_b, hp.eps, d.xn, nullptr, s);
         {
             k::GemmArgs a{};
             a.A = d.xn; a.lda = S; a.W = l.w_fc1; a.ldw = S; a.M = T; a.N = 4 * S; a.K = S; a.bias = l.b_fc1;
@@ -443,10 +471,12 @@
             k::GemmArgs a{};
             a.A = d.h; a.lda = 4 * S; a.W = l.w_fc2; a.ldw = 4 * S; a.M = T; a.N = S; a.K = 4 * S; a.bias = l.b_fc2;
             a.C = d.x; a.ldc = S; a.resid = d.x; a.ldr = S;
+            if (ln_tail) a.ln = il + 1 < La ? k::GemmLn{w.enc[il + 1].ln1_g, w.enc[il + 1].ln1_b, hp.eps, d.xn, nullptr, d.ln_tickets}
+                                            : k::GemmLn{w.e_ln_g, w.e_ln_b, hp.eps, d.enc_out_h, d.enc_out, d.ln_tickets};
             k::gemm(k::EPI_F32_BIAS_RESID, a, s);
         }
     }
-    k::layernorm(d.x, T, S, w.e_ln_g, w.e_ln_b, hp.eps, d.enc_out_h, d.enc_out, s);
+    if (!ln_tail) k::layernorm(d.x, T, S, w.e_ln_g, w.e_ln_b, hp.eps, d.enc_out_h, d.enc_out, s);
     {
         k::GemmArgs a{};
         a.A = d.enc_out_h; a.lda = S; a.W = w.w_ckv; a.ldw = S; a.M = T; a.N = Lt * 2 * S; a.K = S; a.bias = w.b_ckv;
diff --git a/godot-whisper_amd/csrc/gemm_epi.h b/godot-whisper_amd/csrc/gemm_epi.h
--- a/godot-whisper_amd/csrc/gemm_epi.h
+++ b/godot-whisper_amd/csrc/gemm_epi.h
@@ -8,6 +8,17 @@
 typedef _Float16 half4 __attribute__((ext_vector_type(4)));
 typedef float    floatx4 __attribute__((ext_vector_type(4)));
 
+
+typedef uint32_t u32x4_t __attribute__((ext_vector_type(4)));
+template <bool PUB>
+__device__ __forceinline__ void store_x16(void * p, const u32x4_t v) {
+    if constexpr (PUB) asm volatile("global_store_dwordx4 %0, %1, off sc1\n\ts_nop 1" :: "v"(p), "v"(v) : "memory");
+    else *(u32x4_t *) p = v;
+}
+template <bool PUB>
+__device__ __forceinline__ void store_x16(void * p, const float4 o) {
+    store_x16<PUB>(p, u32x4_t{__float_as_uint(o.x), __float_as_uint(o.y), __float_as_uint(o.z), __float_as_uint(o.w)});
+}
 
 __device__ __forceinline__ float round_f16(float x) { return __half2float(f2h(x)); }
 
@@ -150,7 +161,7 @@
     }
 }
 
-template <int EPI, int FM, int FN, bool GUARD>
+template <int EPI, int FM, int FN, bool GUARD, bool PUB = false>
 __device__ __forceinline__ void epilogue_cols(const GemmArgs & a, floatx4 (&acc)[FM][FN], const int mb, const int nb, const int n0, const int lane) {
     const int frow = lane & 15, fq = lane >> 4;
 #pragma unroll
@@ -196,7 +207,7 @@
             } else if constexpr (EPI == EPI_F32_BIAS_RESID) {
                 float4 o;
                 o.x = (v[0] + bias[0]) + rpre[i].x; o.y = (v[1] + bias[1]) + rpre[i].y; o.z = (v[2] + bias[2]) + rpre[i].z; o.w = (v[3] + bias[3]) + rpre[i].w;
-                *(float4 *) ((float *) a.C + (size_t) m * a.ldc + n) = o;
+                store_x16<PUB>((float *) a.C + (size_t) m * a.ldc + n, o);
             } else if constexpr (EPI == EPI_CONV2) {
                 float4 g, o;
                 const float2v x0 = {v[0] + bias[0], v[1] + bias[1]}, x1 = {v[2] + bias[2], v[3] + bias[3]};
@@ -206,7 +217,7 @@
                 if (cr.valid) {
                     if (a.aux) *(float4 *) ((float *) a.aux + (size_t) cr.out * a.ldaux + n) = g;
                     o.x = rpre[i].x + g.x; o.y = rpre[i].y + g.y; o.z = rpre[i].z + g.z; o.w = rpre[i].w + g.w;
-                    *(float4 *) ((float *) a.C + (size_t) cr.out * a.ldc + n) = o;
+                    store_x16<PUB>((float *) a.C + (size_t) cr.out * a.ldc + n, o);
                 }
             } else if constexpr (EPI == EPI_QKV_ENC) {
                 const int seg = __builtin_amdgcn_readfirstlane(n0 / a.S);
@@ -303,12 +314,12 @@
     return !(a.no_glds & 16) && (rpc >= a.M || (rpc & 15) == 0) && (a.ldaux2 & 7) == 0 && (a.chunk_stride_aux2 & 7) == 0;
 }
 
-template <int EPI, int FM, int FN, bool GUARD>
+template <int EPI, int FM, int FN, bool GUARD, bool PUB = false>
 __device__ __forceinline__ void epilogue_cols_wide(const GemmArgs & a, floatx4 (&acc)[FM][FN], const int mb, const int nb, const int n0, const int lane) {
     static_assert(FN % 2 == 0, "wide stores pair fragment columns");
     static_assert(EPI == EPI_F16_BIAS || EPI == EPI_F16_BIAS_GELU || EPI == EPI_Q_SCALED || EPI == EPI_F32_BIAS_RESID || EPI == EPI_CROSS_KV || EPI == EPI_QKV_ENC, "epilogue");
     if constexpr (GUARD) {
-        if (nb + 16 * FN > a.N) { epilogue_cols<EPI, FM, FN, true>(a, acc, mb, nb, n0, lane); return; }
+        if (nb + 16 * FN > a.N) { epilogue_cols<EPI, FM, FN, true, PUB>(a, acc, mb, nb, n0, lane); return; }
     }
     const int frow = lane & 15, fq = lane >> 4;
     const bool lo = frow < 8;
@@ -341,8 +352,8 @@
                 }
                 trade_rows8(P, Q, lo);
                 const int mr = mb + i * 16 + r8, n = nb + (j + hb) * 16 + fq * 4;
-                if (!GUARD || mr < a.M)     *(uint4 *) ((float *) a.C + (size_t) mr * a.ldc + n) = P;
-                if (!GUARD || mr + 8 < a.M) *(uint4 *) ((float *) a.C + (size_t) (mr + 8) * a.ldc + n) = Q;
+                if (!GUARD || mr < a.M)     store_x16<PUB>((float *) a.C + (size_t) mr * a.ldc + n, u32x4_t{P.x, P.y, P.z, P.w});
+                if (!GUARD || mr + 8 < a.M) store_x16<PUB>((float *) a.C + (size_t) (mr + 8) * a.ldc + n, u32x4_t{Q.x, Q.y, Q.z, Q.w});
             }
         }
         return;
diff --git a/godot-whisper_amd/csrc/k_dec.hip b/godot-whisper_amd/csrc/k_dec.hip
--- a/godot-whisper_amd/csrc/k_dec.hip
+++ b/godot-whisper_amd/csrc/k_dec.hip
@@ -2013,6 +2013,8 @@
     kn.debug_sync = getenv("WMI_DEBUG_SYNC") != nullptr;
     kn.pair_withhold = getenv("WMI_PAIR_WITHHOLD") ? atoi(getenv("WMI_PAIR_WITHHOLD")) : 0;
     kn.pair_spin_cap = getenv("WMI_PAIR_SPIN_CAP") ? (uint32_t) strtoul(getenv("WMI_PAIR_SPIN_CAP"), nullptr, 0) : 0u;
+    kn.plain_front = getenv("WMI_PLAIN_FRONT") != nullptr;
+    kn.ln_tail = getenv("WMI_LN_TAIL") != nullptr && !kn.plain_front;
     kn.no_front = getenv("WMI_NO_FRONT") != nullptr;
     kn.front_withhold = getenv("WMI_FRONT_WITHHOLD") ? atoi(getenv("WMI_FRONT_WITHHOLD")) : 0;
     kn.front_wpb = getenv("WMI_FRONT_WPB") ? atoi(getenv("WMI_FRONT_WPB")) : 4;
diff --git a/godot-whisper_amd/csrc/k_gemm.hip b/godot-whisper_amd/csrc/k_gemm.hip
--- a/godot-whisper_amd/csrc/k_gemm.hip
+++ b/godot-whisper_amd/csrc/k_gemm.hip
@@ -2,8 +2,10 @@
 #include "kernels.h"
 #include "wave_ops.h"
 #include "gemm_epi.h"
+#include "ln_row.h"
 
 #include <cstdlib>
+#include <cstdio>
 #include <type_traits>
 
 namespace wmi { namespace k {
@@ -18,7 +20,45 @@
     return (uint32_t) (row * 128 + ((chunk ^ (row & 7)) << 4));
 }
 
-template <int BM, int BN, int EPI, int NST = 2, int NW = 4>
+template <int MAXV>
+__device__ __forceinline__ void ln_panel(const GemmArgs & a, const int m0, const int wave, const int lane) {
+    constexpr int RB = 16 / MAXV;
+    const int S = a.N;
+    float4 gg[MAXV], bb[MAXV]; int cc[MAXV];
+#pragma unroll
+    for (int i = 0; i < MAXV; ++i) {
+        const int c = (i * 64 + lane) * 4;
+        cc[i] = c < S ? c : 0;
+        gg[i] = *(const float4 *) (a.ln.g + cc[i]); bb[i] = *(const float4 *) (a.ln.b + cc[i]);
+    }
+    const int rend = m0 + 64 < a.M ? m0 + 64 : a.M;
+    for (int r0 = m0 + wave * RB; r0 < rend; r0 += 4 * RB) {
+        floatx4 q[16];
+#pragma unroll
+        for (int rb = 0; rb < RB; ++rb) {
+            const int r = r0 + rb < rend ? r0 + rb : rend - 1;
+#pragma unroll
+            for (int i = 0; i < MAXV; ++i) {
+                const float * src = (const float *) a.C + (size_t) r * a.ldc + cc[i];
+                asm volatile("global_load_dwordx4 %0, %1, off sc1" : "=&v"(q[rb * MAXV + i]) : "v"(src) : "memory");
+            }
+        }
+        asm volatile("s_waitcnt vmcnt(0)" : "+v"(q[0]), "+v"(q[1]), "+v"(q[2]), "+v"(q[3]), "+v"(q[4]), "+v"(q[5]), "+v"(q[6]), "+v"(q[7]),
+                                            "+v"(q[8]), "+v"(q[9]), "+v"(q[10]), "+v"(q[11]), "+v"(q[12]), "+v"(q[13]), "+v"(q[14]), "+v"(q[15]) :: "memory");
+#pragma unroll
+        for (int rb = 0; rb < RB; ++rb) {
+            const int r = r0 + rb;
+            if (r < rend) {
+                float4 v[MAXV];
+#pragma unroll
+                for (int i = 0; i < MAXV; ++i) v[i] = make_float4(q[rb * MAXV + i][0], q[rb * MAXV + i][1], q[rb * MAXV + i][2], q[rb * MAXV + i][3]);
+                ln_row<MAXV>(v, gg, bb, S, a.ln.eps, lane, a.ln.out16 + (size_t) r * S, a.ln.out32 ? a.ln.out32 + (size_t) r * S : nullptr);
+            }
+        }
+    }
+}
+
+template <int BM, int BN, int EPI, int NST = 2, int NW = 4, bool LN = false>
 __global__ __launch_bounds__(NW * 64) void k_gemm(const GemmArgs a) {
     constexpr int WN_ = NW / 2;
     constexpr int FM = BM / 32, FN = BN / (WN_ * 16);
@@ -84,6 +124,7 @@
 #else
     constexpr bool SWAP = EPI != EPI_QKV_DEC;
 #endif
+    static_assert(!LN || (SWAP && BM == 64 && NW == 4 && (EPI == EPI_F32_BIAS_RESID || EPI == EPI_CONV2)), "LN tail: published stores exist in the transposed epilogues of x only");
     const bool big = a.M >= 4096;
     const bool swap = SWAP && !(EPI == EPI_QKV_ENC && (n0 >= 2 * a.S || (big && !(a.no_glds & 8)))) && !(EPI == EPI_F32_BIAS_RESID && big && !(a.no_glds & 32));
     auto compute = [&](int buf, auto sw_tag) {
@@ -171,12 +212,12 @@
     if (SWAP && swap) {
         if constexpr (WIDE_OK) {
             if (!(a.no_glds & 4)) {
-                if (interior) epilogue_cols_wide<EPI, FM, FN, false>(a, acc, mb, nb, n0, lane); else epilogue_cols_wide<EPI, FM, FN, true>(a, acc, mb, nb, n0, lane);
+                if (interior) epilogue_cols_wide<EPI, FM, FN, false, LN>(a, acc, mb, nb, n0, lane); else epilogue_cols_wide<EPI, FM, FN, true, LN>(a, acc, mb, nb, n0, lane);
             } else {
-                if (interior) epilogue_cols<EPI, FM, FN, false>(a, acc, mb, nb, n0, lane); else epilogue_cols<EPI, FM, FN, true>(a, acc, mb, nb, n0, lane);
+                if (interior) epilogue_cols<EPI, FM, FN, false, LN>(a, acc, mb, nb, n0, lane); else epilogue_cols<EPI, FM, FN, true, LN>(a, acc, mb, nb, n0, lane);
             }
         } else {
-            if (interior) epilogue_cols<EPI, FM, FN, false>(a, acc, mb, nb, n0, lane); else epilogue_cols<EPI, FM, FN, true>(a, acc, mb, nb, n0, lane);
+            if (interior) epilogue_cols<EPI, FM, FN, false, LN>(a, acc, mb, nb, n0, lane); else epilogue_cols<EPI, FM, FN, true, LN>(a, acc, mb, nb, n0, lane);
         }
     }
     else              { if (interior) epilogue_rows<EPI, FM, FN, false>(a, acc, mb, nb, lane);     else epilogue_rows<EPI, FM, FN, true>(a, acc, mb, nb, lane); }
@@ -186,25 +227,57 @@
         unsigned long long * o = a.probe + (size_t) blockIdx.x * 5;
         o[0] = pt0; o[1] = pt1; o[2] = pt2; o[3] = wall_clock64(); o[4] = hwid;
     }
-}
-
-template <int BM, int BN, int EPI, int NST, int NW = 4>
+    if constexpr (LN) {
+        asm volatile("s_waitcnt vmcnt(0)" ::: "memory");
+        __syncthreads();
+        volatile int * last = (volatile int *) smem;
+        if (tid == 0) {
+            auto * word = (__attribute__((address_space(1))) uint32_t *) (a.ln.tickets + tm);
+            const uint32_t t = __hip_atomic_fetch_add(word, 1u, __ATOMIC_RELAXED, __HIP_MEMORY_SCOPE_AGENT);
+            *last = t == (uint32_t) ntn - 1;
+            if (t == (uint32_t) ntn - 1) __hip_atomic_store(word, 0u, __ATOMIC_RELAXED, __HIP_MEMORY_SCOPE_AGENT);
+        }
+        __syncthreads();
+        if (__builtin_amdgcn_readfirstlane(*last)) {
+            const int nv = (a.N + 255) / 256;
+            if (nv <= 2)      ln_panel<2>(a, m0, wave, lane);
+            else if (nv <= 4) ln_panel<4>(a, m0, wave, lane);
+            else              ln_panel<8>(a, m0, wave, lane);
+        }
+    }
+}
+
+template <int BM, int BN, int EPI, int NST, int NW = 4, bool LN = false>
 void launch_n(const GemmArgs & a, hipStream_t st) {
     const int ntm = (a.M + BM - 1) / BM, ntn = (a.N + BN - 1) / BN;
     const size_t smem = NST * (size_t) (BM + BN) * 128;
     static std::atomic<uint64_t> lds_ok{0};
-    allow_full_lds((const void *) k_gemm<BM, BN, EPI, NST, NW>, lds_ok);
-    hipLaunchKernelGGL((k_gemm<BM, BN, EPI, NST, NW>), dim3(ntm * ntn), dim3(NW * 64), smem, st, a);
-}
-template <int BM, int BN, int EPI>
+    allow_full_lds((const void *) k_gemm<BM, BN, EPI, NST, NW, LN>, lds_ok);
+    hipLaunchKernelGGL((k_gemm<BM, BN, EPI, NST, NW, LN>), dim3(ntm * ntn), dim3(NW * 64), smem, st, a);
+}
+template <int BM, int BN, int EPI, bool LN = false>
 void launch(const GemmArgs & a, hipStream_t st) {
     const long nwg = (long) ((a.M + BM - 1) / BM) * ((a.N + BN - 1) / BN);
-    if (BM < 128 && nwg <= 400) launch_n<BM, BN, EPI, 4>(a, st);
-    else                        launch_n<BM, BN, EPI, 2>(a, st);
+    if (BM < 128 && nwg <= 400) launch_n<BM, BN, EPI, 4, 4, LN>(a, st);
+    else                        launch_n<BM, BN, EPI, 2, 4, LN>(a, st);
+}
+bool ln_tail_shape(int epi, int M, int N, int K) {
+    const long t128 = (long) ((M + 127) / 128) * ((N + 127) / 128);
+    return (epi == EPI_F32_BIAS_RESID || epi == EPI_CONV2) && M > 0 && M < 4096 && (N % 32) == 0 && N <= 2048 && !(t128 >= 320 || (t128 >= 256 && K >= 1024));
 }
 
 template <int EPI>
 void dispatch(const GemmArgs & a, hipStream_t st) {
+    if constexpr (EPI == EPI_F32_BIAS_RESID || EPI == EPI_CONV2) {
+        if (a.ln.out16) {
+            const long t64 = (long) ((a.M + 63) / 64) * ((a.N + 63) / 64);
+            if constexpr (EPI == EPI_F32_BIAS_RESID) {
+                if (a.K >= 1024 && (a.N % 128) == 0 && (a.K % BK) == 0 && t64 >= 400 && !(a.no_glds & 1)) { launch_n<64, 128, EPI, 4, 4, true>(a, st); return; }
+                if (t64 < 256) launch<64, 32, EPI, true>(a, st); else launch<64, 64, EPI, true>(a, st);
+            } else launch<64, 64, EPI, true>(a, st);
+            return;
+        }
+    }
     const long t128 = (long) ((a.M + 127) / 128) * ((a.N + 127) / 128);
     const long t64 = (long) ((a.M + 63) / 64) * ((a.N + 63) / 64);
     static const int wide = getenv("WMI_GEMM_WIDE") ? atoi(getenv("WMI_GEMM_WIDE")) : 0;
@@ -237,6 +310,8 @@
 
 static thread_local GemmLog * tl_gemm_log = nullptr;
 void gemm_log_install(GemmLog * log) { tl_gemm_log = log; }
+
+bool gemm_ln_tail_ok(int epi, int M, int N, int K) { return ln_tail_shape(epi, M, N, K); }
 
 void gemm(int epi, const GemmArgs & a_in, hipStream_t st) {
     static const bool no_glds = getenv("WMI_GEMM_NO_GLDS") != nullptr;
@@ -245,6 +320,10 @@
     static const bool qkv_swap = getenv("WMI_GEMM_QKV_SWAP") != nullptr;
     static const bool resid_swap = getenv("WMI_GEMM_RESID_SWAP") != nullptr;
     static const bool vt_narrow = getenv("WMI_GEMM_VT_NARROW") != nullptr;
+    if (a_in.ln.out16 && !(ln_tail_shape(epi, a_in.M, a_in.N, a_in.K) && a_in.ln.tickets && a_in.ln.g && a_in.ln.b && a_in.rows_per_chunk <= 0 && a_in.ldc == a_in.N)) {
+        fprintf(stderr, "[wmi] gemm: LN tail asked of a launch that does not take it (epi %d, %d x %d x %d)\n", epi, a_in.M, a_in.N, a_in.K);
+        return;
+    }
     GemmArgs a = a_in; a.no_glds = (no_glds ? 1 : 0) | (guard_all ? 2 : 0) | (narrow ? 4 : 0) | (qkv_swap ? 8 : 0) | (vt_narrow ? 16 : 0) | (resid_swap ? 32 : 0);
     if (GemmLog * lg = tl_gemm_log) {
         const size_t wgs = (size_t) ((a.M + 63) / 64) * (size_t) ((a.N + 31) / 32);
diff --git a/godot-whisper_amd/csrc/k_mel.hip b/godot-whisper_amd/csrc/k_mel.hip
--- a/godot-whisper_amd/csrc/k_mel.hip
+++ b/godot-whisper_amd/csrc/k_mel.hip
@@ -43,6 +43,10 @@
     out[i] = v;
 }
 __global__ void k_mel_pad(const float * __restrict__ pcm, int n, float * __restrict__ out, int total, int * __restrict__ gmax) { mel_pad_body(pcm, n, out, total, gmax); }
+__device__ __forceinline__ float mel_pad_at(const float * __restrict__ pcm, int n, int i) {
+    if (i < 200) { int j = 200 - i; if (j > n - 1) j = n - 1; if (j < 0) j = 0; return n > 0 ? pcm[j] : 0.0f; }
+    return i < 200 + n ? pcm[i - 200] : 0.0f;
+}
 __global__ void k_mel_pad_b(const MelBatch b) { const int c = blockIdx.y; mel_pad_body(b.pcm[c], b.n[c], b.pad[c], b.n[c] + 480400, b.gmax[c]); }
 
 __device__ inline void butterfly_stage(const float * src, float * dst, int ngroups, int N, int tid, int nthreads,
@@ -64,19 +68,20 @@
     }
 }
 
-__device__ __forceinline__ void mel_tail_body(float * __restrict__ mel, int n_len, int n_mel, int n_fft_frames, int * __restrict__ gmax) {
+__device__ __forceinline__ void mel_tail_body(float * __restrict__ mel, int n_len, int n_mel, int n_fft_frames, int * __restrict__ gmax, int blk) {
     const int w = n_len - n_fft_frames;
-    const int i = blockIdx.x * blockDim.x + threadIdx.x;
+    const int i = blk * blockDim.x + threadIdx.x;
     if (i < w * n_mel) { const int j = i / w, f = n_fft_frames + (i - j * w); mel[(size_t) j * n_len + f] = -10.0f; }
     if (i == 0 && w > 0) atomicMax(gmax, enc_ordered(-10.0f));
 }
-__global__ void k_mel_tail(float * __restrict__ mel, int n_len, int n_mel, int n_fft_frames, int * __restrict__ gmax) { mel_tail_body(mel, n_len, n_mel, n_fft_frames, gmax); }
+__global__ void k_mel_tail(float * __restrict__ mel, int n_len, int n_mel, int n_fft_frames, int * __restrict__ gmax) { mel_tail_body(mel, n_len, n_mel, n_fft_frames, gmax, blockIdx.x); }
 
 constexpr int MEL_NT = 256;
 __device__ __forceinline__ void mel_frames_body(const float * __restrict__ pad, int n_valid, int n_fft_frames,
                                                     int n_len, int n_mel, const float * __restrict__ filters,
                                                     const int32_t * __restrict__ ranges, const float * __restrict__ taps,
-                                                    float * __restrict__ mel, int * __restrict__ gmax) {
+                                                    float * __restrict__ mel, int * __restrict__ gmax,
+                                                    const float * __restrict__ pcm = nullptr, int n_pcm = 0) {
     __shared__ float xin[400];
     __shared__ __attribute__((aligned(8))) float bufA[800];
     __shared__ __attribute__((aligned(8))) float bufB[800];
@@ -93,7 +98,8 @@
         const int j0 = tid, j1 = tid + 256;
         const int j1c = j1 < 400 ? j1 : 0, jt = tid < 200 ? tid : 0, j25 = tid < 25 ? tid : 0, j50 = tid < 50 ? tid : 0, j100 = tid < 100 ? tid : 0;
         const float h0 = c_mel.hann[j0], h1 = c_mel.hann[j1c];
-        const float p0 = pad[offset + (j0 < nin ? j0 : 0)], p1 = pad[offset + (j1c < nin ? j1c : 0)];
+        const int i0 = offset + (j0 < nin ? j0 : 0), i1 = offset + (j1c < nin ? j1c : 0);
+        const float p0 = pcm ? mel_pad_at(pcm, n_pcm, i0) : pad[i0], p1 = pcm ? mel_pad_at(pcm, n_pcm, i1) : pad[i1];
         const float2 w25 = make_float2(c_mel.cosv[16 * j25], c_mel.sinv[16 * j25]), w50 = make_float2(c_mel.cosv[8 * j25], c_mel.sinv[8 * j25]);
         const float2 w100 = make_float2(c_mel.cosv[4 * j50], c_mel.sinv[4 * j50]);
         const float2 w200 = make_float2(c_mel.cosv[2 * j100], c_mel.sinv[2 * j100]);
@@ -198,6 +204,14 @@
                                                     float * __restrict__ mel, int * __restrict__ gmax) {
     mel_frames_body(pad, n_valid, n_fft_frames, n_len, n_mel, filters, ranges, taps, mel, gmax);
 }
+__global__ __launch_bounds__(MEL_NT) void k_mel_frames_pcm(const float * __restrict__ pcm, int n_pcm, int n_fft_frames,
+                                                        int n_len, int n_mel, const float * __restrict__ filters,
+                                                        const int32_t * __restrict__ ranges, const float * __restrict__ taps,
+                                                        float * __restrict__ mel, int * __restrict__ gmax) {
+    static_assert(MEL_NT == 256, "the tail's element index");
+    if ((int) blockIdx.x >= n_fft_frames) { mel_tail_body(mel, n_len, n_mel, n_fft_frames, gmax, (int) blockIdx.x - n_fft_frames); return; }
+    mel_frames_body(nullptr, n_pcm + 200, n_fft_frames, n_len, n_mel, filters, ranges, taps, mel, gmax, pcm, n_pcm);
+}
 __device__ __forceinline__ int mel_n_len(int n) { return (int) (((long long) n + 480000) / 160); }
 __device__ __forceinline__ int mel_n_fft(int n) { const int a = (n + 200) / 160 + 1, l = mel_n_len(n); return a < l ? a : l; }
 __global__ __launch_bounds__(MEL_NT) void k_mel_frames_b(const MelBatch b, int n_mel, const float * __restrict__ filters,
@@ -207,18 +221,19 @@
 }
 __global__ void k_mel_tail_b(const MelBatch b, int n_mel) {
     const int c = blockIdx.y, n = b.n[c];
-    mel_tail_body(b.mel[c], mel_n_len(n), n_mel, mel_n_fft(n), b.gmax[c]);
-}
-
-__device__ __forceinline__ void mel_normalize_body(float * __restrict__ mel, int n, const int * __restrict__ gmax) {
+    mel_tail_body(b.mel[c], mel_n_len(n), n_mel, mel_n_fft(n), b.gmax[c], blockIdx.x);
+}
+
+__device__ __forceinline__ void mel_normalize_body(float * __restrict__ mel, int n, const int * __restrict__ gmax, int * __restrict__ gmax_next = nullptr) {
     int i = blockIdx.x * blockDim.x + threadIdx.x;
+    if (i == 0 && gmax_next) *gmax_next = INT_MIN;
     if (i >= n) return;
     const double mmax = (double) dec_ordered(*gmax) - 8.0;
     float v = mel[i];
     if ((double) v < mmax) v = (float) mmax;
     mel[i] = (float) (((double) v + 4.0) / 4.0);
 }
-__global__ void k_mel_normalize(float * __restrict__ mel, int n, const int * __restrict__ gmax) { mel_normalize_body(mel, n, gmax); }
+__global__ void k_mel_normalize(float * __restrict__ mel, int n, const int * __restrict__ gmax, int * __restrict__ gmax_next) { mel_normalize_body(mel, n, gmax, gmax_next); }
 __global__ void k_mel_normalize_b(const MelBatch b, int n_mel) { const int c = blockIdx.y; mel_normalize_body(b.mel[c], n_mel * mel_n_len(b.n[c]), b.gmax[c]); }
 
 __global__ void k_mel_slice(const float * __restrict__ mel, int n_len, int n_mel, int offset, int n_frames,
@@ -391,16 +406,22 @@
 }
 
 void mel_frames(const float * pcm_pad, int n_valid, int n_fft_frames, int n_len, int n_mel, const float * filters,
-                const int32_t * ranges, const float * taps, float * mel, int * gmax, hipStream_t st) {
+                const int32_t * ranges, const float * taps, float * mel, int * gmax, hipStream_t st, const float * pcm, int n_pcm) {
     {
         int dev = 0; (void) hipGetDevice(&dev);
         const uint64_t bit = 1ull << (dev & 63);
         if (!(g_tables_mask.load(std::memory_order_acquire) & bit)) { upload_tables(); g_tables_mask.fetch_or(bit, std::memory_order_release); }
     }
-    if (n_fft_frames > 0)
+    if (n_fft_frames > 0 && !pcm)
         hipLaunchKernelGGL(k_mel_frames, dim3(n_fft_frames), dim3(MEL_NT), 0, st, pcm_pad, n_valid, n_fft_frames, n_len, n_mel,
                            filters, ranges, taps, mel, gmax);
     const int tail = (n_len - n_fft_frames) * n_mel;
+    if (pcm) {
+        const int blocks = std::max(n_fft_frames, 0) + (tail > 0 ? (tail + MEL_NT - 1) / MEL_NT : 0);
+        if (blocks > 0) hipLaunchKernelGGL(k_mel_frames_pcm, dim3(blocks), dim3(MEL_NT), 0, st, pcm, n_pcm, std::max(n_fft_frames, 0), n_len, n_mel,
+                                           filters, ranges, taps, mel, gmax);
+        return;
+    }
     if (tail > 0) hipLaunchKernelGGL(k_mel_tail, dim3((tail + 255) / 256), dim3(256), 0, st, mel, n_len, n_mel, n_fft_frames, gmax);
 }
 
@@ -427,8 +448,11 @@
     if (n_max > 0) hipLaunchKernelGGL(k_signal_energy_b, dim3((n_max + 255) / 256, nb), dim3(256), 0, st, b, hw);
 }
 
-void mel_normalize(float * mel, int n, const int * gmax, hipStream_t st) {
-    hipLaunchKernelGGL(k_mel_normalize, dim3((n + 255) / 256), dim3(256), 0, st, mel, n, gmax);
+void mel_normalize(float * mel, int n, const int * gmax, hipStream_t st, int * gmax_next) {
+    hipLaunchKernelGGL(k_mel_normalize, dim3((n + 255) / 256), dim3(256), 0, st, mel, n, gmax, gmax_next);
+}
+void mel_max_init(int * words, int n, hipStream_t st) {
+    for (int i = 0; i < n; ++i) hipLaunchKernelGGL(k_set_int, dim3(1), dim3(1), 0, st, words + i, INT_MIN);
 }
 
 void mel_slice(const float * mel, int n_len, int n_mel, int offset, int n_frames, __half * out, int ld, int rows_total,
diff --git a/godot-whisper_amd/csrc/k_norm.hip b/godot-whisper_amd/csrc/k_norm.hip
--- a/godot-whisper_amd/csrc/k_norm.hip
+++ b/godot-whisper_amd/csrc/k_norm.hip
@@ -1,6 +1,7 @@
 
 #include "kernels.h"
 #include "wave_ops.h"
+#include "ln_row.h"
 
 namespace wmi { namespace k {
 
@@ -21,43 +22,7 @@
         const int c = (i * 64 + lane) * 4, cc = c < S ? c : 0;
         v[i] = *(const float4 *) (xr + cc); gg[i] = *(const float4 *) (g + cc); bb[i] = *(const float4 *) (b + cc);
     }
-    float sum = 0.0f;
-#pragma unroll
-    for (int i = 0; i < MAXV; ++i) {
-        const int c = (i * 64 + lane) * 4;
-        if (c < S) sum += (v[i].x + v[i].y) + (v[i].z + v[i].w);
-        else v[i] = make_float4(0.f, 0.f, 0.f, 0.f);
-    }
-    _Pragma("unroll") for (int o = 32; o > 0; o >>= 1) sum += WMI_SHX(sum, o);
-    const float mean = sum / (float) S;
-    float sq = 0.0f;
-#pragma unroll
-    for (int i = 0; i < MAXV; ++i) {
-        const int c = (i * 64 + lane) * 4;
-        if (c < S) {
-            v[i].x -= mean; v[i].y -= mean; v[i].z -= mean; v[i].w -= mean;
-            sq += (v[i].x * v[i].x + v[i].y * v[i].y) + (v[i].z * v[i].z + v[i].w * v[i].w);
-        }
-    }
-    _Pragma("unroll") for (int o = 32; o > 0; o >>= 1) sq += WMI_SHX(sq, o);
-    const float scale = 1.0f / sqrtf(sq / (float) S + eps);
-#pragma unroll
-    for (int i = 0; i < MAXV; ++i) {
-        const int c = (i * 64 + lane) * 4;
-        if (c < S) {
-            float4 y;
-            y.x = __fadd_rn(__fmul_rn(v[i].x * scale, gg[i].x), bb[i].x);
-            y.y = __fadd_rn(__fmul_rn(v[i].y * scale, gg[i].y), bb[i].y);
-            y.z = __fadd_rn(__fmul_rn(v[i].z * scale, gg[i].z), bb[i].z);
-            y.w = __fadd_rn(__fmul_rn(v[i].w * scale, gg[i].w), bb[i].w);
-            if (out32) *(float4 *) (out32 + (size_t) orow * S + c) = y;
-            if (out16) {
-                __half2 h01 = __floats2half2_rn(pin_f32(y.x), pin_f32(y.y)), h23 = __floats2half2_rn(pin_f32(y.z), pin_f32(y.w));
-                uint2 pk; pk.x = *(uint32_t *) &h01; pk.y = *(uint32_t *) &h23;
-                *(uint2 *) (out16 + (size_t) orow * S + c) = pk;
-            }
-        }
-    }
+    ln_row<MAXV>(v, gg, bb, S, eps, lane, out16 ? out16 + (size_t) orow * S : nullptr, out32 ? out32 + (size_t) orow * S : nullptr);
 }
 
 }
diff --git a/godot-whisper_amd/csrc/kernels.h b/godot-whisper_amd/csrc/kernels.h
--- a/godot-whisper_amd/csrc/kernels.h
+++ b/godot-whisper_amd/csrc/kernels.h
@@ -59,8 +59,10 @@
 
 void mel_pad(const float * pcm, int n_samples, float * pcm_pad, int n_pad_total, hipStream_t st, int * gmax_reset);
 void mel_frames(const float * pcm_pad, int n_valid, int n_fft_frames, int n_len, int n_mel,
-                const float * filters, const int32_t * ranges, const float * taps, float * mel, int * gmax, hipStream_t st);
-void mel_normalize(float * mel, int n, const int * gmax, hipStream_t st);
+                const float * filters, const int32_t * ranges, const float * taps, float * mel, int * gmax, hipStream_t st,
+                const float * pcm = nullptr, int n_pcm = 0);
+void mel_normalize(float * mel, int n, const int * gmax, hipStream_t st, int * gmax_next = nullptr);
+void mel_max_init(int * words, int n, hipStream_t st);
 struct MelBatch { const float * pcm[16]; float * pad[16]; float * mel[16]; int * gmax[16]; float * energy[16]; float * bmin[16]; float * bmax[16]; int n[16]; };
 void mel_batch(const MelBatch & b, int nb, int n_mel, const float * filters, const int32_t * ranges, const float * taps, hipStream_t st);
 void signal_energy_batch(const MelBatch & b, int nb, int hw, hipStream_t st);
@@ -107,6 +109,7 @@
     EPI_CROSS_KV,
     EPI_Q_SCALED,
 };
+struct GemmLn { const float * g; const float * b; float eps; __half * out16; float * out32; uint32_t * tickets; };
 struct GemmArgs {
     const __half * A;  int lda;
     const __half * W;  int ldw;
@@ -123,8 +126,10 @@
     int64_t chunk_stride_aux2;
     int     no_glds;
     unsigned long long * probe;
+    GemmLn  ln;
 };
 void gemm(int epi, const GemmArgs & a, hipStream_t st);
+bool gemm_ln_tail_ok(int epi, int M, int N, int K);
 struct GemmLogEntry { int epi, M, N, K; size_t off; int cap; };
 struct GemmLog { unsigned long long * buf = nullptr; size_t cap_words = 0, used = 0; std::vector<GemmLogEntry> entries; };
 void gemm_log_install(GemmLog * log);
@@ -233,7 +238,7 @@
 void xback(XbackArgs a, int H, float * scratch, hipStream_t st);
 bool front_usable(int S, int rows = 1, int long_cap = 0);
 void front(const FrontArgs & a, hipStream_t st, bool long_kv = false);
-struct Knobs { bool no_mlp_pair; int sa_wpb; bool gemv1_wide_generic; bool host_draws; bool debug_sync; int pair_withhold; uint32_t pair_spin_cap; bool no_front; int front_withhold; bool no_xback; int xback_withhold; int front_wpb; };
+struct Knobs { bool no_mlp_pair; int sa_wpb; bool gemv1_wide_generic; bool host_draws; bool debug_sync; int pair_withhold; uint32_t pair_spin_cap; bool no_front; int front_withhold; bool no_xback; int xback_withhold; int front_wpb; bool plain_front; bool ln_tail; };
 const Knobs & knobs();
 void reload_knobs();
 void set_attn_one_group(bool on);
diff --git a/godot-whisper_amd/csrc/ln_row.h b/godot-whisper_amd/csrc/ln_row.h
--- /dev/null
+++ b/godot-whisper_amd/csrc/ln_row.h
@@ -0,0 +1,51 @@
+#pragma once
+#include "kernels.h"
+#include "wave_ops.h"
+
+namespace wmi { namespace k {
+
+#if defined(__HIPCC__)
+template <int MAXV>
+__device__ __forceinline__ void ln_row(float4 (&v)[MAXV], const float4 (&gg)[MAXV], const float4 (&bb)[MAXV], const int S, const float eps, const int lane,
+                                       __half * __restrict__ out16, float * __restrict__ out32) {
+    float sum = 0.0f;
+#pragma unroll
+    for (int i = 0; i < MAXV; ++i) {
+        const int c = (i * 64 + lane) * 4;
+        if (c < S) sum += (v[i].x + v[i].y) + (v[i].z + v[i].w);
+        else v[i] = make_float4(0.f, 0.f, 0.f, 0.f);
+    }
+    _Pragma("unroll") for (int o = 32; o > 0; o >>= 1) sum += WMI_SHX(sum, o);
+    const float mean = sum / (float) S;
+    float sq = 0.0f;
+#pragma unroll
+    for (int i = 0; i < MAXV; ++i) {
+        const int c = (i * 64 + lane) * 4;
+        if (c < S) {
+            v[i].x -= mean; v[i].y -= mean; v[i].z -= mean; v[i].w -= mean;
+            sq += (v[i].x * v[i].x + v[i].y * v[i].y) + (v[i].z * v[i].z + v[i].w * v[i].w);
+        }
+    }
+    _Pragma("unroll") for (int o = 32; o > 0; o >>= 1) sq += WMI_SHX(sq, o);
+    const float scale = 1.0f / sqrtf(sq / (float) S + eps);
+#pragma unroll
+    for (int i = 0; i < MAXV; ++i) {
+        const int c = (i * 64 + lane) * 4;
+        if (c < S) {
+            float4 y;
+            y.x = __fadd_rn(__fmul_rn(v[i].x * scale, gg[i].x), bb[i].x);
+            y.y = __fadd_rn(__fmul_rn(v[i].y * scale, gg[i].y), bb[i].y);
+            y.z = __fadd_rn(__fmul_rn(v[i].z * scale, gg[i].z), bb[i].z);
+            y.w = __fadd_rn(__fmul_rn(v[i].w * scale, gg[i].w), bb[i].w);
+            if (out32) *(float4 *) (out32 + c) = y;
+            if (out16) {
+                __half2 h01 = __floats2half2_rn(pin_f32(y.x), pin_f32(y.y)), h23 = __floats2half2_rn(pin_f32(y.z), pin_f32(y.w));
+                uint2 pk; pk.x = *(uint32_t *) &h01; pk.y = *(uint32_t *) &h23;
+                *(uint2 *) (out16 + c) = pk;
+            }
+        }
+    }
+}
+#endif
+
+}}
diff --git a/godot-whisper_amd/csrc/wmi.h b/godot-whisper_amd/csrc/wmi.h
--- a/godot-whisper_amd/csrc/wmi.h
+++ b/godot-whisper_amd/csrc/wmi.h
@@ -161,6 +161,7 @@
     float * pcm = nullptr;      size_t pcm_cap = 0;
     float * mel = nullptr;      size_t mel_cap = 0;
     float * mel_max = nullptr;
+    bool    mel_words_ready = false; int mel_par = 0;
     const float * last_pcm = nullptr; int last_pcm_n = 0;
     float * energy = nullptr;   size_t energy_cap = 0;
     float * energy_host = nullptr;
@@ -190,6 +191,7 @@
     __half * enc_out_h = nullptr;
     __half * kvc_k = nullptr, * kvc_v = nullptr;
     int      Tpad = 0;
+    uint32_t * ln_tickets = nullptr;
     int      conv1_max_T = 0;
     int32_t * d_tokens = nullptr, * d_pos = nullptr;
     float   * d_mask = nullptr;
```
